# ilkyyldz95/3DmedicalImageSegmentation

Measured on AMD Instinct MI355X. Metric: training volumes/sec (96^3, 4-class), higher is better.
Workload: dtype bf16; 1 GPU; UNETR(img=96^3,patch=16,hidden=768,layers=12,heads=12,classes=4) fwd+DiceCE+bwd+AdamW, batch 2/GPU, configs[1]; global_batch=2

## Files before the change

### 3dmedicalimagesegmentation_amd/_capi.py

```python
import ctypes
import os
from ctypes import c_double, c_float, c_int, c_long, c_size_t, c_void_p

_HERE = os.path.dirname(os.path.abspath(__file__))
LIB_PATH = os.environ.get("UNETR_AMD_LIB") or os.path.join(_HERE, "libunetr_hip.so")

PREC_F32 = 0
PREC_BF16 = 1
PREC_BF16X3 = 2
ABI_VERSION = 21

_ERR = {1: "invalid argument", 2: "kernel launch failed", 3: "unsupported shape/configuration",
        4: "workspace too small"}


class GemmDesc(ctypes.Structure):
    _fields_ = [
        ("M", c_int), ("N", c_int), ("K", c_int), ("batch", c_int),
        ("a_trans", c_int), ("b_trans", c_int),
        ("lda", c_long), ("ldb", c_long), ("ldc", c_long),
        ("strideA", c_long), ("strideB", c_long), ("strideC", c_long),
        ("bias", c_void_p), ("res", c_void_p),
        ("ldr", c_long), ("strideR", c_long), ("res_mod", c_int),
        ("pre", c_void_p), ("aux", c_void_p), ("ldaux", c_long),
        ("act", c_int), ("accumulate", c_int), ("alpha", c_float), ("prec", c_int), ("b_x3words", c_int),
    ]


class GemmBf16Desc(ctypes.Structure):
    _fields_ = [
        ("M", c_int), ("N", c_int), ("K", c_int), ("b_kn", c_int),
        ("lda", c_long), ("ldb", c_long), ("ldc", c_long), ("ldcb", c_long),
        ("bias", c_void_p), ("res", c_void_p), ("ldr", c_long), ("res_mod", c_int),
        ("pre", c_void_p), ("aux", c_void_p), ("ldaux", c_long),
        ("act", c_int), ("accumulate", c_int), ("alpha", c_float),
        ("tc_d", c_int), ("tc_h", c_int), ("tc_w", c_int), ("tc_cout", c_int), ("x3", c_int),
    ]


class GroupedProblem(ctypes.Structure):
    _fields_ = [("dy", c_void_p), ("x", c_void_p), ("dw", c_void_p), ("M", c_int), ("N", c_int), ("K", c_int)]


class AdamWArena(ctypes.Structure):
    _fields_ = [("param", c_void_p), ("grad", c_void_p), ("m", c_void_p), ("v", c_void_p), ("shadow_bf16", c_void_p), ("steps", c_void_p),
                ("total", c_long), ("lr", c_float), ("beta1", c_float), ("beta2", c_float), ("eps", c_float), ("weight_decay", c_float),
                ("shadow_x3", c_void_p)]


class PackProblem(ctypes.Structure):
    _fields_ = [("w", c_void_p), ("out", c_void_p), ("Cin", c_int), ("Cout", c_int), ("kind", c_int)]


class ReduceProblem(ctypes.Structure):
    _fields_ = [("part", c_void_p), ("dst", c_void_p), ("n", c_long), ("rows", c_int)]


class SplitProblem(ctypes.Structure):
    _fields_ = [("src", c_void_p), ("dst", c_void_p), ("rows", c_long), ("cols", c_long), ("second", c_int)]


class ColsumProblem(ctypes.Structure):
    _fields_ = [("x", c_void_p), ("out", c_void_p), ("ld", c_long), ("M", c_int), ("N", c_int), ("x_bf16", c_int)]


class AugDesc(ctypes.Structure):
    _fields_ = [("B", c_int), ("num_samples", c_int), ("C", c_int), ("L", c_int), ("S0", c_int), ("S1", c_int), ("S2", c_int),
                ("sampling", c_int), ("ax0", c_int), ("ax1", c_int), ("max_k", c_int), ("normalize", c_int),
                ("pos_ratio", c_double), ("flip_prob", c_double * 3), ("rot90_prob", c_double), ("shift_prob", c_double),
                ("shift_lo", c_double), ("shift_hi", c_double), ("seed", ctypes.c_uint64)]


P = c_void_p
_SIGNATURES = {
    "unetr_abi_version": [],
    "unetr_gemm": [ctypes.POINTER(GemmDesc), P, P, P, P, c_size_t, P],
    "unetr_gemm_bf16": [ctypes.POINTER(GemmBf16Desc), P, P, P, P, P, c_size_t, P],
    "unetr_gemm_bf16_ln_bwd": [ctypes.POINTER(GemmBf16Desc), P, P, P, P, P, P, P, P, P, P, P, P, P, c_size_t, P, c_size_t, P],
    "unetr_gemm_bf16_ln_fwd": [ctypes.POINTER(GemmBf16Desc), P, P, P, P, P, c_float, P, P, P, P, P, c_size_t, P],
    "unetr_cast_bf16": [P, P, c_long, P],
    "unetr_split_words": [P, P, c_long, P],
    "unetr_split_stack_bf16": [P, P, c_long, c_long, c_int, P],
    "unetr_split_stack_bf16_grouped": [ctypes.POINTER(SplitProblem), c_int, P],
    "unetr_attention_bf16_fwd": [P, P, P, P, c_int, c_int, c_int, c_int, c_float, P],
    "unetr_attention_bf16_bwd": [P, P, P, P, P, P, P, c_int, c_int, c_int, c_int, c_float, P],
    "unetr_gemm_grouped_wgrad": [ctypes.POINTER(GroupedProblem), c_int, c_int, P],
    "unetr_gemm_bf16_grouped_wgrad": [ctypes.POINTER(GroupedProblem), c_int, P],
    "unetr_gemm_bf16_grouped_wgrad_adamw": [ctypes.POINTER(GroupedProblem), c_int, ctypes.POINTER(AdamWArena), ctypes.POINTER(c_int), P],
    "unetr_adamw_ranges": [ctypes.POINTER(AdamWArena), P, c_int, c_long, P],
    "unetr_gemm_bf16_grouped_wgrad_bf16out": [ctypes.POINTER(GroupedProblem), c_int, P, P, c_long, P],
    "unetr_cast_bf16_ranges": [P, P, P, c_int, c_long, P],
    "unetr_colsum_grouped": [ctypes.POINTER(ColsumProblem), c_int, P],
    "unetr_tconv_fwd": [P, c_long, P, P, c_long, c_int, c_int, c_int, c_int, c_int, c_int, c_int, P, c_size_t, P],
    "unetr_tconv_dgrad": [P, c_long, P, P, c_long, c_int, c_int, c_int, c_int, c_int, c_int, c_int, c_int, P, c_size_t, P],
    "unetr_tconv_wgrad": [P, c_long, P, c_long, P, c_int, c_int, c_int, c_int, c_int, c_int, c_int, P, c_size_t, P],
    "unetr_tconv2_fwd": [P, c_long, P, P, c_long, c_int, c_int, c_int, c_int, c_int, c_int, c_int, P, c_size_t, P],
    "unetr_tconv2_wgrad": [P, c_long, P, c_long, P, c_int, c_int, c_int, c_int, c_int, c_int, c_int, P, c_size_t, P],
    "unetr_tconv2_dgrad": [P, c_long, P, P, c_long, c_int, c_int, c_int, c_int, c_int, c_int, c_int, c_int, P, c_size_t, P],
    "unetr_tconv2_fwd_supported": [c_long, c_int, c_int, c_long, c_long],
    "unetr_tconv2_wgrad_supported": [c_long, c_int, c_int, c_long, c_long],
    "unetr_pixel_shuffle2": [P, P, c_long, c_int, c_int, c_int, c_int, c_int, c_int, P],
    "unetr_pixel_unshuffle2_bf16": [P, c_long, P, c_int, c_int, c_int, c_int, c_int, c_int, P],
    "unetr_colsum": [P, c_long, c_int, c_int, P, c_int, P, c_size_t, P],
    "unetr_layernorm_fwd": [P, P, P, P, P, P, P, c_int, c_int, c_float, P],
    "unetr_layernorm_bwd": [P, P, P, P, P, P, P, P, P, P, c_int, c_int, P, c_size_t, P],
    "unetr_attention_fwd": [P, P, P, P, c_int, c_int, c_int, c_int, c_float, c_int, P],
    "unetr_attention_bwd": [P, P, P, P, P, P, P, c_int, c_int, c_int, c_int, c_float, c_int, P],
    "unetr_conv_pack_weight": [P, P, c_int, c_int, c_int, c_int, P],
    "unetr_conv_gemm_fwd": [P, c_long, P, P, c_long, c_int, c_int, c_int, c_int, c_int, c_int, c_int, c_int, c_int, P, c_size_t, P],
    "unetr_conv_gemm_wgrad": [P, c_long, P, c_long, P, c_int, c_int, c_int, c_int, c_int, c_int, c_int, c_int, P, c_size_t, P],
    "unetr_conv3_pack_weight": [P, P, c_int, c_int, c_int, c_int, P],
    "unetr_conv3_fwd": [P, c_long, P, P, c_long, c_int, c_int, c_int, c_int, c_int, c_int, c_int, c_int, P],
    "unetr_conv3_fwd_fused": [P, c_long, P, P, c_long, P, P, P, c_long, P, c_float, c_int, c_int, c_int, c_int, c_int, c_int, c_int, c_int, P, c_size_t, P],
    "unetr_conv3_fwd_parts": [P, c_long, P, P, c_long, P, P, P, c_long, P, ctypes.POINTER(c_int), c_int, c_int, c_int, c_int, c_int, c_int, c_int, c_int, P],
    "unetr_conv3_dgrad_stats": [P, c_long, P, P, c_long, P, c_long, P, P, ctypes.POINTER(c_int), c_int, c_int, c_int, c_int, c_int, c_int, c_int, P],
    "unetr_instnorm_apply_fin": [P, c_long, P, c_int, P, c_long, P, c_int, P, P, c_float, P, c_long, c_int, c_long, c_int, c_int, c_int, P],
    "unetr_instnorm_apply_fin_img": [P, c_long, P, c_int, P, c_int, P, P, c_int, P, P, c_float, P, c_long, c_int, c_long, c_int, c_int, c_int, P],
    "unetr_instnorm_bwd_img": [P, c_long, P, c_long, P, P, c_int, P, P, P, c_long, P, ctypes.POINTER(c_int), c_int, c_long, c_int, c_int, P, c_size_t, c_int, P],
    "unetr_instnorm_bwd_apply_fin": [P, c_long, P, c_long, P, P, c_long, P, P, c_int, c_int, P, c_long, P, c_long, c_int, c_long, c_int, c_int, c_int, P],
    "unetr_conv3_wgrad_parts": [P, c_long, P, c_long, P, c_long, P, c_size_t, ctypes.POINTER(c_long), c_int, c_int, c_int, c_int, c_int, c_int, c_int, c_int, P],
    "unetr_tconv2_wgrad_parts": [P, c_long, P, c_long, P, c_size_t, ctypes.POINTER(c_long), c_int, c_int, c_int, c_int, c_int, c_int, c_int, P],
    "unetr_reduce_rows_grouped": [ctypes.POINTER(ReduceProblem), c_int, P],
    "unetr_conv3_dgrad_fused": [P, c_long, P, P, c_long, P, P, P, c_long, c_int, c_int, c_int, c_int, c_int, c_int, c_int, P, c_size_t, P],
    "unetr_conv3_pack_grouped": [ctypes.POINTER(PackProblem), c_int, c_int, P],
    "unetr_conv3_pack_1x1": [P, P, c_int, c_int, c_int, P],
    "unetr_instnorm_stats_finalize": [P, c_int, c_int, c_long, c_int, c_float, P, P],
    "unetr_conv3_wgrad": [P, c_long, P, c_long, P, P, c_long, P, c_int, c_int, c_int, c_int, c_int, c_int, c_int, c_int, P, c_size_t, P],
    "unetr_debug_tr16": [P, P, P],
    "unetr_instnorm_stats": [P, c_long, c_int, c_long, c_int, c_float, P, P, c_size_t, c_int, P],
    "unetr_instnorm_apply": [P, c_long, P, P, c_long, P, P, c_long, c_int, c_long, c_int, c_int, c_int, P],
    "unetr_instnorm_bwd": [P, c_long, P, c_long, P, P, c_long, P, P, c_long, P, c_long, c_int, c_long, c_int, c_int, P, c_size_t, c_int, P],
    "unetr_nchw_to_nhwc": [P, P, c_long, c_int, c_int, c_long, c_int, P],
    "unetr_nhwc_to_nchw": [P, c_long, P, c_int, c_int, c_long, c_int, c_int, P],
    "unetr_patch_gather": [P, P, P, c_int, c_int, c_int, c_int, c_int, c_int, P],
    "unetr_counter_add": [P, P, c_int, P],
    "unetr_add_cast_bf16": [P, P, P, P, c_long, P],
    "unetr_copy_rows": [P, c_long, P, c_long, c_long, c_int, c_int, c_int, P],
    "unetr_outconv_fwd": [P, c_long, P, P, P, c_int, c_long, c_int, c_int, c_int, P],
    "unetr_outconv_bwd": [P, P, c_long, P, P, c_long, P, P, c_int, c_long, c_int, c_int, P, c_size_t, c_int, P],
    "unetr_outconv_in_fwd": [P, c_long, P, c_int, P, c_long, P, c_int, P, P, c_float, P, P, P, c_int, c_long, c_int, c_int, c_int, P],
    "unetr_outconv_in_bwd": [P, P, c_long, P, P, c_long, P, P, P, c_long, P, P, P, c_int, c_long, c_int, c_int, P, c_size_t, c_int, P],
    "unetr_dicece_fwd": [P, P, c_int, c_int, c_long, c_int, c_float, c_float, P, P, P, c_size_t, P],
    "unetr_dicece_bwd": [P, P, P, P, P, c_int, c_int, c_long, c_int, P],
    "unetr_sw_accumulate": [P, P, P, P, c_int, c_int, c_int, c_int, c_int, c_int, c_int, c_int, c_int, c_int, P],
    "unetr_sw_finalize": [P, P, c_int, c_int, c_long, P],
    "unetr_dice_counts": [P, P, c_int, c_int, c_long, c_int, P, P, c_size_t, P],
    "unetr_hausdorff": [P, P, c_int, c_int, c_int, c_int, c_int, c_int, c_int, c_int, c_double, c_int, P, P, c_size_t, c_int, P],
    "unetr_aug_prep": [P, P, c_int, c_int, c_int, c_int, c_int, c_int, c_float, c_float, c_float, c_float, c_float, c_int, P, P, P],
    "unetr_aug_crop": [P, P, c_int, c_int, c_int, c_int, c_int, c_int, c_int, c_int, c_int, c_int, c_int, P, P, P],
    "unetr_aug_index_count": [P, P, c_int, c_int, c_long, c_float, P, c_size_t, P],
    "unetr_aug_index_scatter": [P, P, c_int, c_int, c_long, c_float, P, c_size_t, P, P, P],
    "unetr_aug_sample": [ctypes.POINTER(AugDesc), P, c_int, P, P, P, P],
    "unetr_aug_gather": [ctypes.POINTER(AugDesc), P, c_int, P, P, P, P, c_size_t, P],
    "unetr_resample_orient": [P, c_int, P, c_int, c_int, c_int, c_int, c_int, c_int, ctypes.POINTER(c_double), c_int, c_int, c_int, P, P, P],
    "unetr_ranking_loss_fwd": [P, c_int, c_int, c_int, c_int, c_int, c_int, c_float, c_int, P, P, P, c_size_t, P],
    "unetr_ranking_loss_bwd": [P, c_int, c_int, c_int, c_int, c_int, c_int, P, P, P, P],
    "unetr_adamw": [P, P, P, P, c_long, c_float, c_float, c_float, c_float, c_float, P, P, P],
    "unetr_adamw_reduced": [P, P, c_int, c_float, P, P, c_long, c_float, c_float, c_float, c_float, c_float, P, P, P, P],
}

EXPORTED_SYMBOLS = tuple(_SIGNATURES) + ("unetr_conv3_packed_bytes", "unetr_conv3_packed_1x1_bytes", "unetr_ranking_workspace_floats",
                                            "unetr_conv3_wgrad_rows", "unetr_tconv2_wgrad_rows", "unetr_outconv_in_bwd_rows", "unetr_hausdorff_workspace_bytes",
                                            "unetr_aug_index_ws_ints", "unetr_aug_gather_ws_bytes")

_lib = None


def load():
    global _lib
    if _lib is not None:
        return _lib
    if not os.path.exists(LIB_PATH):
        raise RuntimeError(
            f"{LIB_PATH} is missing: the HIP extension is not built. Run `python -c 'import __graft_entry__ as g; "
            f"g.build()'` or `make -C {os.path.join(_HERE, 'csrc')}`. There is no CPU/PyTorch fallback.")
    lib = ctypes.CDLL(LIB_PATH)
    lib.unetr_abi_version.restype = c_int
    got = lib.unetr_abi_version()
    if got != ABI_VERSION:
        raise RuntimeError(f"{LIB_PATH} reports C-ABI version {got}, this binding was written against {ABI_VERSION}: the "
                           f"library is stale -- rebuild the extension (`make -C {os.path.join(_HERE, 'csrc')}`).")
    for name, argtypes in _SIGNATURES.items():
        fn = getattr(lib, name)
        fn.argtypes = argtypes
        fn.restype = c_int
    lib.unetr_conv3_packed_bytes.argtypes = [c_int, c_int, c_int, c_int]
    lib.unetr_conv3_packed_bytes.restype = c_size_t
    lib.unetr_conv3_packed_1x1_bytes.argtypes = [c_int, c_int, c_int]
# ... 31 lines not shown
```

### 3dmedicalimagesegmentation_amd/csrc/attention_b16.hip

```cpp
#include <cstdlib>
#include "common.hpp"
#include "../../include/unetr_hip.h"

namespace {

typedef __attribute__((address_space(3))) void lds_void_t;
typedef const __attribute__((address_space(1))) void gbl_void_t;
typedef short s16x4 __attribute__((ext_vector_type(4)));
typedef short s16x8 __attribute__((ext_vector_type(8)));
#define LDS_AS_ __attribute__((address_space(3)))

constexpr int DH = 64, ROWB = 128;
constexpr int CKEYS = 224, CT = CKEYS / 16;
constexpr int IMG = CKEYS * ROWB;
constexpr float NEG_BIG = -1.0e30f;

__device__ __forceinline__ int img_off(int row, int chunk) { return row * ROWB + ((chunk ^ (((row >> 1) & 3) << 1)) << 4); }

template <int NT>
__device__ __forceinline__ void stage_img(const uint16_t* __restrict__ src, long rs, int row0, int nrows, int rows, char* img) {
    const int tid = threadIdx.x, wave = __builtin_amdgcn_readfirstlane(tid >> 6);
    const int pieces = rows * 8;
    for (int base = 0; base < pieces; base += NT) {
        const int id = base + tid;
// ... 18 lines not shown

__device__ __forceinline__ void prod_T(f32x4 (&out)[4], f32x4 x0, f32x4 x1, const char* img, int R0) {
    const int lane = threadIdx.x & 63, c = lane & 15, g = lane >> 4, q = c >> 2, p = c & 3;
    float xv[8] = {x0[0], x0[1], x0[2], x0[3], x1[0], x1[1], x1[2], x1[3]};
    const u32x4 b = PrecBF16::pack(xv);
    const int r0 = R0 + 4 * g + q, r1 = r0 + 16;
#pragma unroll
    for (int dt = 0; dt < 4; ++dt) {
        const int ch = dt * 2 + (p >> 1);
        s16x4 lo = __builtin_amdgcn_ds_read_tr16_b64_v4i16((LDS_AS_ s16x4*)(img + img_off(r0, ch) + (p & 1) * 8));
        s16x4 hi = __builtin_amdgcn_ds_read_tr16_b64_v4i16((LDS_AS_ s16x4*)(img + img_off(r1, ch) + (p & 1) * 8));
        s16x8 t = {lo[0], lo[1], lo[2], lo[3], hi[0], hi[1], hi[2], hi[3]};
        PrecBF16::mma(out[dt], __builtin_bit_cast(u32x4, t), b);
    }
}

template <class F>
__device__ __forceinline__ void prod_rows_full(const char* img, const u32x4 (&vec)[2], F&& each) {
    const int lane = threadIdx.x & 63, c = lane & 15, g = lane >> 4;
    constexpr int DPT = 5;
    const char* p0 = img + img_off(c, g);
    const char* p1 = img + img_off(c, 4 + g);
    u32x4 r0[DPT], r1[DPT];
#pragma unroll
    for (int t = 0; t < DPT; ++t) { r0[t] = *(const u32x4*)(p0 + t * 16 * ROWB); r1[t] = *(const u32x4*)(p1 + t * 16 * ROWB); }
    __builtin_amdgcn_sched_barrier(0);
#pragma unroll
    for (int t = 0; t < CT; ++t) {
        f32x4 acc = {0.f, 0.f, 0.f, 0.f};
        PrecBF16::mma(acc, r0[t % DPT], vec[0]);
        PrecBF16::mma(acc, r1[t % DPT], vec[1]);
        if (t + DPT < CT) { r0[t % DPT] = *(const u32x4*)(p0 + (t + DPT) * 16 * ROWB); r1[t % DPT] = *(const u32x4*)(p1 + (t + DPT) * 16 * ROWB); }
        each(t, acc);
        __builtin_amdgcn_sched_barrier(0);
    }
}
template <class F>
__device__ __forceinline__ void prod_T_full(f32x4 (&out)[4], const char* img, F&& x) {
    const int lane = threadIdx.x & 63, c = lane & 15, g = lane >> 4, q = c >> 2, p = c & 3;
    constexpr int NS = (CT / 2) * 4, DPT = 6;
    const char* b0[2];
    const int r0 = 4 * g + q;
    auto addr = [&](int st, int hi) { const int t2 = st >> 2, dt = st & 3; return img + img_off(32 * t2 + r0 + 16 * hi, dt * 2 + (p >> 1)) + (p & 1) * 8; };
    (void)b0;
    s16x4 lo[DPT], hi[DPT];
#pragma unroll
    for (int st = 0; st < DPT; ++st) {
        lo[st] = __builtin_amdgcn_ds_read_tr16_b64_v4i16((LDS_AS_ s16x4*)addr(st, 0));
        hi[st] = __builtin_amdgcn_ds_read_tr16_b64_v4i16((LDS_AS_ s16x4*)addr(st, 1));
    }
    __builtin_amdgcn_sched_barrier(0);
    u32x4 b = {0u, 0u, 0u, 0u};
#pragma unroll
    for (int st = 0; st < NS; ++st) {
        const int t2 = st >> 2, dt = st & 3;
        if (dt == 0) {
            f32x4 x0, x1;
            x(t2, x0, x1);
            float xv[8] = {x0[0], x0[1], x0[2], x0[3], x1[0], x1[1], x1[2], x1[3]};
            b = PrecBF16::pack(xv);
        }
        s16x8 t = {lo[st % DPT][0], lo[st % DPT][1], lo[st % DPT][2], lo[st % DPT][3], hi[st % DPT][0], hi[st % DPT][1], hi[st % DPT][2], hi[st % DPT][3]};
        PrecBF16::mma(out[dt], __builtin_bit_cast(u32x4, t), b);
        if (st + DPT < NS) {
            lo[st % DPT] = __builtin_amdgcn_ds_read_tr16_b64_v4i16((LDS_AS_ s16x4*)addr(st + DPT, 0));
            hi[st % DPT] = __builtin_amdgcn_ds_read_tr16_b64_v4i16((LDS_AS_ s16x4*)addr(st + DPT, 1));
        }
        __builtin_amdgcn_sched_barrier(0);
    }
}

__device__ __forceinline__ void load_vec(const uint16_t* __restrict__ row, u32x4 (&f)[2]) {
    const int g = (threadIdx.x & 63) >> 4;
    f[0] = *(const u32x4*)(row + g * 8);
    f[1] = *(const u32x4*)(row + (4 + g) * 8);
}

__device__ __forceinline__ float grp_max(float v) { v = fmaxf(v, __shfl_xor(v, 16, 64)); return fmaxf(v, __shfl_xor(v, 32, 64)); }
__device__ __forceinline__ float grp_sum(float v) { v += __shfl_xor(v, 16, 64); return v + __shfl_xor(v, 32, 64); }

template <int NW>
__global__ void __launch_bounds__(64 * NW)
attn16_fwd_kernel(const uint16_t* __restrict__ qkv, float* __restrict__ out, uint16_t* __restrict__ outb, float* __restrict__ lse,
                  int L, int heads, float scale) {
    constexpr int NT = 64 * NW;
    extern __shared__ __attribute__((aligned(1024))) char lds[];
    char* kimg = lds;
    char* vimg = lds + IMG;
    const int lane = threadIdx.x & 63, wave = __builtin_amdgcn_readfirstlane(threadIdx.x >> 6), c = lane & 15, g = lane >> 4;
    const int head = blockIdx.y, b = blockIdx.z, Hd = heads * DH;
    const long rs = 3L * Hd;
    const uint16_t* qb = qkv + (long)b * L * rs + head * DH;
    const uint16_t* kb_ = qb + Hd;
    const uint16_t* vb = qb + 2 * Hd;
    const int q = blockIdx.x * (16 * NW) + wave * 16 + c, qc = min(q, L - 1);
    u32x4 qf[2];
    load_vec(qb + (long)qc * rs, qf);
    f32x4 o[4];
#pragma unroll
    for (int dt = 0; dt < 4; ++dt) o[dt] = (f32x4){0.f, 0.f, 0.f, 0.f};
    float m = NEG_BIG, l = 0.f;
    for (int k0 = 0; k0 < L; k0 += CKEYS) {
        const int nkeys = min(CKEYS, L - k0), rows = (nkeys + 31) & ~31, nt = rows >> 4;
        if (k0) __syncthreads();
        stage_img<NT>(kb_, rs, k0, L, rows, kimg);
        stage_img<NT>(vb, rs, k0, L, rows, vimg);
        asm volatile("s_waitcnt vmcnt(0)" ::: "memory");
        __syncthreads();
        f32x4 s[CT];
        float tmax = NEG_BIG;
        const bool full = nt == CT;
        if (full) {
            prod_rows_full(kimg, qf, [&](int t, f32x4 acc) {
#pragma unroll
                for (int r = 0; r < 4; ++r) {
                    const int key = t * 16 + 4 * g + r;
                    acc[r] = key < nkeys ? acc[r] * scale : NEG_BIG;
                    tmax = fmaxf(tmax, acc[r]);
                }
                s[t] = acc;
            });
        } else
#pragma unroll
        for (int t = 0; t < CT; ++t) {
            if (t < nt) {
                s[t] = prod_rows(kimg, t, qf);
#pragma unroll
                for (int r = 0; r < 4; ++r) {
                    const int key = t * 16 + 4 * g + r;
                    s[t][r] = key < nkeys ? s[t][r] * scale : NEG_BIG;
                    tmax = fmaxf(tmax, s[t][r]);
                }
            } else {
                s[t] = (f32x4){NEG_BIG, NEG_BIG, NEG_BIG, NEG_BIG};
            }
        }
        tmax = grp_max(tmax);
        const float mn = fmaxf(m, tmax), alpha = __expf(m - mn);
        float ps = 0.f;
#pragma unroll
        for (int t = 0; t < CT; ++t)
#pragma unroll
            for (int r = 0; r < 4; ++r) { s[t][r] = __expf(s[t][r] - mn); ps += s[t][r]; }
        ps = grp_sum(ps);
        l = l * alpha + ps;
        m = mn;
#pragma unroll
        for (int dt = 0; dt < 4; ++dt) o[dt] *= alpha;
        if (full) {
            prod_T_full(o, vimg, [&](int t2, f32x4& x0, f32x4& x1) { x0 = s[2 * t2]; x1 = s[2 * t2 + 1]; });
        } else {
#pragma unroll
            for (int t2 = 0; t2 < CT / 2; ++t2)
                if (2 * t2 < nt) prod_T(o, s[2 * t2], s[2 * t2 + 1], vimg, 32 * t2);
        }
    }
    if (q < L) {
        const float inv = 1.f / l;
        if (out) {
            float* op = out + ((long)b * L + q) * Hd + head * DH + 4 * g;
#pragma unroll
            for (int dt = 0; dt < 4; ++dt) *(f32x4*)(op + dt * 16) = o[dt] * inv;
        }
        if (outb) {
            uint16_t* ob = outb + ((long)b * L + q) * Hd + head * DH + 4 * g;
#pragma unroll
            for (int dt = 0; dt < 4; ++dt) *(bf16x4*)(ob + dt * 16) = __builtin_convertvector(o[dt] * inv, bf16x4);
        }
// ... 117 lines not shown
        stage_img<NT>(qb, rs, q0, L, rows, qimg);
        stage_img<NT>(dob, (long)Hd, q0, L, rows, doimg);
        for (int i = threadIdx.x; i < rows; i += NT) {
            const int qq = q0 + i;
            lse_t[i] = qq < L ? lse[((long)b * heads + head) * L + qq] : 1.0e30f;
        }
        for (int i = threadIdx.x; i < rows; i += NT) {
            const int qq = min(q0 + i, L - 1);
            float part[4];
#pragma unroll
            for (int gg = 0; gg < 4; ++gg) {
                part[gg] = 0.f;
#pragma unroll
                for (int kb = 0; kb < 2; ++kb) {
                    const bf16x8 a = __builtin_bit_cast(bf16x8, *(const u32x4*)(ob_ + (long)qq * Hd + (kb * 4 + gg) * 8));
                    const bf16x8 d = __builtin_bit_cast(bf16x8, *(const u32x4*)(dob + (long)qq * Hd + (kb * 4 + gg) * 8));
#pragma unroll
                    for (int e = 0; e < 8; ++e) part[gg] += (float)a[e] * (float)d[e];
                }
            }
            del_t[i] = q0 + i < L ? (part[0] + part[1]) + (part[2] + part[3]) : 0.f;
        }
        asm volatile("s_waitcnt vmcnt(0)" ::: "memory");
        __syncthreads();
        if (nt == CT) {
            f32x4 pf[CT], dsf[CT];
            prod_rows_full(qimg, kf, [&](int t, f32x4 acc) {
                const f32x4 l4 = *(const f32x4*)(lse_t + t * 16 + 4 * g);
#pragma unroll
                for (int r = 0; r < 4; ++r) acc[r] = __expf(acc[r] * scale - l4[r]);
                pf[t] = acc;
            });
            prod_rows_full(doimg, vf, [&](int t, f32x4 dp) {
                const f32x4 d4 = *(const f32x4*)(del_t + t * 16 + 4 * g);
#pragma unroll
                for (int r = 0; r < 4; ++r) dsf[t][r] = pf[t][r] * (dp[r] - d4[r]);
            });
            prod_T_full(dv, doimg, [&](int t2, f32x4& x0, f32x4& x1) { x0 = pf[2 * t2]; x1 = pf[2 * t2 + 1]; });
            prod_T_full(dk, qimg, [&](int t2, f32x4& x0, f32x4& x1) { x0 = dsf[2 * t2]; x1 = dsf[2 * t2 + 1]; });
        } else
#pragma unroll
        for (int t2 = 0; t2 < CT / 2; ++t2) {
            if (2 * t2 >= nt) break;
            f32x4 p[2], ds[2];
#pragma unroll
            for (int h = 0; h < 2; ++h) {
                const int t = 2 * t2 + h;
                const f32x4 s = prod_rows(qimg, t, kf);
                const f32x4 dp = prod_rows(doimg, t, vf);
                const f32x4 l4 = *(const f32x4*)(lse_t + t * 16 + 4 * g), d4 = *(const f32x4*)(del_t + t * 16 + 4 * g);
#pragma unroll
                for (int r = 0; r < 4; ++r) {
                    const float pv = __expf(s[r] * scale - l4[r]);
                    p[h][r] = pv;
                    ds[h][r] = pv * (dp[r] - d4[r]);
                }
            }
            prod_T(dv, p[0], p[1], doimg, 32 * t2);
            prod_T(dk, ds[0], ds[1], qimg, 32 * t2);
        }
    }
    if (key < L) {
        if (dqkv) {
            float* kp = dqkv + ((long)b * L + key) * rs + Hd + head * DH + 4 * g;
#pragma unroll
            for (int dt = 0; dt < 4; ++dt) {
                *(f32x4*)(kp + dt * 16) = dk[dt] * scale;
                *(f32x4*)(kp + Hd + dt * 16) = dv[dt];
            }
        }
        uint16_t* kb2 = dqkvb + ((long)b * L + key) * rs + Hd + head * DH + 4 * g;
#pragma unroll
        for (int dt = 0; dt < 4; ++dt) {
            *(bf16x4*)(kb2 + dt * 16) = __builtin_convertvector(dk[dt] * scale, bf16x4);
            *(bf16x4*)(kb2 + Hd + dt * 16) = __builtin_convertvector(dv[dt], bf16x4);
        }
    }
}

template <int NW>
__global__ void __launch_bounds__(64 * NW)
attn16_bwd_kernel(const uint16_t* __restrict__ qkv, const uint16_t* __restrict__ outb, const uint16_t* __restrict__ doutb,
                  const float* __restrict__ lse, float* __restrict__ delta, float* __restrict__ dqkv, uint16_t* __restrict__ dqkvb,
                  int L, int heads, float scale, int nqb) {
    extern __shared__ __attribute__((aligned(1024))) char lds[];
    const int xb = __builtin_amdgcn_readfirstlane(blockIdx.x);
    if (xb < nqb) attn16_bwd_dq_body<NW>(lds, xb, qkv, outb, doutb, lse, delta, dqkv, dqkvb, L, heads, scale);
    else attn16_bwd_dkv_body<NW>(lds, xb - nqb, qkv, outb, doutb, lse, dqkv, dqkvb, L, heads, scale);
}

template <class K, class... A>
void launch_dyn(K kern, dim3 grid, int nt, size_t lds, hipStream_t st, A... args) {
    if (lds > 64 * 1024) (void)hipFuncSetAttribute((const void*)kern, hipFuncAttributeMaxDynamicSharedMemorySize, (int)lds);
    hipLaunchKernelGGL(kern, grid, dim3(nt), lds, st, args...);
}

inline int pick_nw(int B, int L, int heads) { return ((long)cdiv(L, 32) * heads * B <= 512) ? 2 : 4; }
inline int pick_nw_fwd(int B, int L, int heads) {
    if (const char* e = getenv("UNETR_ATTN_NW")) { const int v = atoi(e); if (v == 2 || v == 4 || v == 8) return v; }
    const int nw = pick_nw(B, L, heads);
    return (nw == 4 && (long)cdiv(L, 64) * heads * B > 1024) ? 8 : nw;
}

}

extern "C" int unetr_attention_bf16_fwd(const void* qkv, float* out, void* out_bf16, float* lse, int B, int L, int heads, int dh,
                                        float scale, void* stream) {
    if (!qkv || (!out && !out_bf16) || !lse || B <= 0 || L <= 0 || heads <= 0 || B > 65535 || heads > 65535) return UNETR_ERR_ARG;
    if (dh != DH || ((uintptr_t)qkv & 15) || (out && ((uintptr_t)out & 15)) || (out_bf16 && ((uintptr_t)out_bf16 & 7))) return UNETR_ERR_UNSUPPORTED;
    hipStream_t st = (hipStream_t)stream;
    const size_t lds = 2 * IMG;
    const int nw = pick_nw_fwd(B, L, heads);
    if (nw == 2)
        launch_dyn(attn16_fwd_kernel<2>, dim3(cdiv(L, 32), heads, B), 128, lds, st, (const uint16_t*)qkv, out, (uint16_t*)out_bf16, lse, L, heads, scale);
    else if (nw == 4)
        launch_dyn(attn16_fwd_kernel<4>, dim3(cdiv(L, 64), heads, B), 256, lds, st, (const uint16_t*)qkv, out, (uint16_t*)out_bf16, lse, L, heads, scale);
    else
        launch_dyn(attn16_fwd_kernel<8>, dim3(cdiv(L, 128), heads, B), 512, lds, st, (const uint16_t*)qkv, out, (uint16_t*)out_bf16, lse, L, heads, scale);
    return unetr_check_launch();
}

extern "C" int unetr_attention_bf16_bwd(const void* qkv, const void* out_bf16, const void* dout_bf16, const float* lse, float* dqkv,
                                        void* dqkv_bf16, float* delta, int B, int L, int heads, int dh, float scale, void* stream) {
    if (!qkv || !out_bf16 || !dout_bf16 || !lse || !dqkv_bf16 || !delta || B <= 0 || L <= 0 || heads <= 0 || B > 65535 || heads > 65535)
        return UNETR_ERR_ARG;
    if (dh != DH || ((uintptr_t)qkv & 15) || ((uintptr_t)out_bf16 & 15) || ((uintptr_t)dout_bf16 & 15) || ((uintptr_t)dqkv_bf16 & 7) ||
        (dqkv && ((uintptr_t)dqkv & 15)))
        return UNETR_ERR_UNSUPPORTED;
    hipStream_t st = (hipStream_t)stream;
    const uint16_t* q = (const uint16_t*)qkv;
    const uint16_t* o = (const uint16_t*)out_bf16;
    const uint16_t* d = (const uint16_t*)dout_bf16;
    uint16_t* gq = (uint16_t*)dqkv_bf16;
    const size_t lk = 2 * IMG + 2 * CKEYS * sizeof(float);
    if (pick_nw(B, L, heads) == 2) {
        const int nqb = cdiv(L, 32);
        launch_dyn(attn16_bwd_kernel<2>, dim3(2 * nqb, heads, B), 128, lk, st, q, o, d, lse, delta, dqkv, gq, L, heads, scale, nqb);
    } else {
        const int nqb = cdiv(L, 64);
        launch_dyn(attn16_bwd_kernel<4>, dim3(2 * nqb, heads, B), 256, lk, st, q, o, d, lse, delta, dqkv, gq, L, heads, scale, nqb);
    }
    return unetr_check_launch();
}
```

### 3dmedicalimagesegmentation_amd/csrc/common.hpp

```cpp
#pragma once
#include "../../include/unetr_hip.h"
#include <hip/hip_runtime.h>
#include <stdint.h>

typedef float f32x2 __attribute__((ext_vector_type(2)));
typedef float f32x4 __attribute__((ext_vector_type(4)));
typedef float f32x8 __attribute__((ext_vector_type(8)));
typedef __bf16 bf16x8 __attribute__((ext_vector_type(8)));
typedef __bf16 bf16x4 __attribute__((ext_vector_type(4)));
typedef uint32_t u32x4 __attribute__((ext_vector_type(4)));

#define UNETR_OK 0
#define UNETR_ERR_ARG 1
#define UNETR_ERR_LAUNCH 2
#define UNETR_ERR_UNSUPPORTED 3
#define UNETR_ERR_WORKSPACE 4

#define UNETR_PREC_F32 0
#define UNETR_PREC_BF16 1
#define UNETR_PREC_BF16X3 2

static inline int unetr_check_launch() {
    hipError_t e = hipGetLastError();
    return e == hipSuccess ? UNETR_OK : UNETR_ERR_LAUNCH;
}

struct PrecF32 {
    static constexpr int CH = 4;
    static __device__ __forceinline__ u32x4 pack(const float* v) {
        f32x4 t = {v[0], v[1], v[2], v[3]};
        return __builtin_bit_cast(u32x4, t);
    }
    static __device__ __forceinline__ u32x4 from_raw(u32x4 r) { return r; }
    static __device__ __forceinline__ void mma(f32x4& acc, u32x4 a, u32x4 b) {
        f32x4 af = __builtin_bit_cast(f32x4, a), bf = __builtin_bit_cast(f32x4, b);
        acc = __builtin_amdgcn_mfma_f32_16x16x4f32(af[0], bf[0], acc, 0, 0, 0);
        acc = __builtin_amdgcn_mfma_f32_16x16x4f32(af[1], bf[1], acc, 0, 0, 0);
        acc = __builtin_amdgcn_mfma_f32_16x16x4f32(af[2], bf[2], acc, 0, 0, 0);
        acc = __builtin_amdgcn_mfma_f32_16x16x4f32(af[3], bf[3], acc, 0, 0, 0);
    }
};

struct PrecBF16 {
    static constexpr int CH = 8;
    static __device__ __forceinline__ u32x4 pack(const float* v) {
        f32x8 t = {v[0], v[1], v[2], v[3], v[4], v[5], v[6], v[7]};
        bf16x8 b = __builtin_convertvector(t, bf16x8);
        return __builtin_bit_cast(u32x4, b);
    }
    static __device__ __forceinline__ u32x4 from_raw(u32x4 r) { return r; }
    static __device__ __forceinline__ void mma(f32x4& acc, u32x4 a, u32x4 b) {
        acc = __builtin_amdgcn_mfma_f32_16x16x32_bf16(__builtin_bit_cast(bf16x8, a), __builtin_bit_cast(bf16x8, b),
                                                      acc, 0, 0, 0);
    }
};

struct PrecBF16x3 {
    static constexpr int CH = 4;
    static __device__ __forceinline__ uint32_t split(float a) {
        const __bf16 h = (__bf16)a;
#ifdef UNETR_X3_DROP_LO
        return (uint32_t)__builtin_bit_cast(uint16_t, h);
#endif
        const __bf16 l = (__bf16)(a - (float)h);
        return (uint32_t)__builtin_bit_cast(uint16_t, h) | ((uint32_t)__builtin_bit_cast(uint16_t, l) << 16);
    }
    static __device__ __forceinline__ u32x4 pack(const float* v) { return (u32x4){split(v[0]), split(v[1]), split(v[2]), split(v[3])}; }
    static __device__ __forceinline__ u32x4 from_raw(u32x4 r) {
        const f32x4 f = __builtin_bit_cast(f32x4, r);
        return (u32x4){split(f[0]), split(f[1]), split(f[2]), split(f[3])};
    }
    static __device__ __forceinline__ void mma(f32x4& acc, u32x4 a, u32x4 b) {
        u32x4 ah, al;
#pragma unroll
        for (int e = 0; e < 4; ++e) {
            ah[e] = __builtin_amdgcn_perm(a[e], a[e], 0x01000100u);
            al[e] = __builtin_amdgcn_perm(a[e], a[e], 0x03020302u);
        }
        acc = __builtin_amdgcn_mfma_f32_16x16x32_bf16(__builtin_bit_cast(bf16x8, ah), __builtin_bit_cast(bf16x8, b), acc, 0, 0, 0);
        acc = __builtin_amdgcn_mfma_f32_16x16x32_bf16(__builtin_bit_cast(bf16x8, al), __builtin_bit_cast(bf16x8, b), acc, 0, 0, 0);
    }
};
typedef float f32x2_ __attribute__((ext_vector_type(2)));
typedef __bf16 bf16x2_ __attribute__((ext_vector_type(2)));
__device__ __forceinline__ float x3_rem(uint32_t r) {
#ifdef UNETR_X3_DROP_LO
// ... 66 lines not shown
    const float pe = p * c.decay;
    const float me = fmaf(c.b1, m, (1.f - c.b1) * g);
    const float ve = fmaf(c.b2, v, ((1.f - c.b2) * g) * g);
    const float denom = fmaf(sqrtf(ve), c.inv_sqrt_bc2, c.eps);
    p = fmaf(-c.step_size, me / denom, pe);
    m = me;
    v = ve;
}

__device__ __forceinline__ float gelu_exact(float x) { return 0.5f * x * (1.0f + erff(x * 0.70710678118654752440f)); }
__device__ __forceinline__ float gelu_grad(float x) {
    return 0.5f * (1.0f + erff(x * 0.70710678118654752440f)) + x * 0.39894228040143267794f * expf(-0.5f * x * x);
}

__device__ __forceinline__ float erf_poly_tail(float t , float e ) {
    const float k = __builtin_amdgcn_rcpf(1.0f + 0.3275911f * t);
    float p = 1.061405429f;
    p = fmaf(p, k, -1.453152027f); p = fmaf(p, k, 1.421413741f); p = fmaf(p, k, -0.284496736f); p = fmaf(p, k, 0.254829592f);
    return 1.0f - p * k * e;
}
__device__ __forceinline__ float gelu_fast(float x) {
    const float t = fabsf(x) * 0.70710678118654752440f;
    const float e = __expf(-t * t);
    const float er = copysignf(erf_poly_tail(t, e), x);
    return 0.5f * x * (1.0f + er);
}
__device__ __forceinline__ float gelu_grad_fast(float x) {
    const float t = fabsf(x) * 0.70710678118654752440f;
    const float e = __expf(-t * t);
    const float er = copysignf(erf_poly_tail(t, e), x);
    return 0.5f * (1.0f + er) + x * 0.39894228040143267794f * e;
}

static inline int cdiv(long a, long b) { return (int)((a + b - 1) / b); }

template <class T> struct Io;
template <> struct Io<float> {
    static constexpr int B16 = 0;
    static constexpr int W = 4;
    static __device__ __forceinline__ void ldw(const float* p, float (&v)[4]) { const f32x4 t = *(const f32x4*)p; v[0] = t[0]; v[1] = t[1]; v[2] = t[2]; v[3] = t[3]; }
    static __device__ __forceinline__ void stw(float* p, const float (&v)[4]) { *(f32x4*)p = (f32x4){v[0], v[1], v[2], v[3]}; }
    static __device__ __forceinline__ u32x4 ldraw(const float* p) { return *(const u32x4*)p; }
    static __device__ __forceinline__ void unpack(u32x4 r, float (&v)[4]) {
#pragma unroll
        for (int e = 0; e < 4; ++e) { const uint32_t t = r[e]; v[e] = __builtin_bit_cast(float, t); }
    }
    static __device__ __forceinline__ f32x4 ld4(const float* p) { return *(const f32x4*)p; }
    static __device__ __forceinline__ void st4(float* p, f32x4 v) { *(f32x4*)p = v; }
    static __device__ __forceinline__ float ld1(const float* p) { return *p; }
    static __device__ __forceinline__ void st1(float* p, float v) { *p = v; }
};
template <> struct Io<uint16_t> {
    static constexpr int B16 = 1;
    static constexpr int W = 8;
    static __device__ __forceinline__ void ldw(const uint16_t* p, float (&v)[8]) {
        const f32x8 t = __builtin_convertvector(*(const bf16x8*)p, f32x8);
#pragma unroll
        for (int e = 0; e < 8; ++e) v[e] = t[e];
    }
    static __device__ __forceinline__ void stw(uint16_t* p, const float (&v)[8]) {
        const f32x8 t = {v[0], v[1], v[2], v[3], v[4], v[5], v[6], v[7]};
        *(bf16x8*)p = __builtin_convertvector(t, bf16x8);
    }
    static __device__ __forceinline__ u32x4 ldraw(const uint16_t* p) { return *(const u32x4*)p; }
    static __device__ __forceinline__ void unpack(u32x4 r, float (&v)[8]) {
#pragma unroll
        for (int e = 0; e < 4; ++e) {
            v[2 * e] = __builtin_bit_cast(float, r[e] << 16);
            v[2 * e + 1] = __builtin_bit_cast(float, r[e] & 0xffff0000u);
        }
    }
    static __device__ __forceinline__ f32x4 ld4(const uint16_t* p) { return __builtin_convertvector(*(const bf16x4*)p, f32x4); }
    static __device__ __forceinline__ void st4(uint16_t* p, f32x4 v) { *(bf16x4*)p = __builtin_convertvector(v, bf16x4); }
    static __device__ __forceinline__ float ld1(const uint16_t* p) { return __builtin_bit_cast(float, (uint32_t)*p << 16); }
    static __device__ __forceinline__ void st1(uint16_t* p, float v) { __bf16 h = (__bf16)v; *p = __builtin_bit_cast(uint16_t, h); }
};
template <class P> struct ActOf { typedef float type; };
template <> struct ActOf<PrecBF16> { typedef uint16_t type; };
template <class P>
__device__ __forceinline__ u32x4 act_chunk(const typename ActOf<P>::type* p, bool ok) {
    const u32x4 w = *(const u32x4*)p;
    return ok ? P::from_raw(w) : (u32x4){0u, 0u, 0u, 0u};
}
int unetr_layernorm_bwd_partials(const float* dy, int splits, long slab, const float* x, const float* gamma, const float* mean,
                                 const float* rstd, float* dx, void* dx_bf16, const float* dres, float* dgamma,
                                 float* dbeta, int M, int H, float* ws, size_t ws_bytes, void* stream);

int unetr_layernorm_fwd_partials(const float* partials, int splits, long slab, const float* bias, const float* res, long ldr, int res_mod,
                                 float* xout, const float* gamma, const float* beta, float* y, void* y_bf16, float* mean, float* rstd,
                                 int M, int H, float eps, void* stream);

int unetr_gemm_x3_dma(const unetr_gemm_bf16_desc* d, const float* A, const float* B, int b_words, float* C, float* ws, size_t ws_bytes, void* stream,
                      int* psp = nullptr);

int unetr_instnorm_stats_finalize2(const float* part, const float* part_b, int nchunk, int B, long V, int C, float eps,
                                   float* stats, float* stats_b, void* stream);

#define ACT_DISPATCH(act16, ...) do { if (act16) { typedef uint16_t AT; __VA_ARGS__; } else { typedef float AT; __VA_ARGS__; } } while (0)
```

### 3dmedicalimagesegmentation_amd/csrc/gemm_bf16.hip

```cpp
#include <type_traits>
#include "gemm_kernel.hpp"

namespace {

typedef __attribute__((address_space(3))) void lds_void_t;
typedef const __attribute__((address_space(1))) void gbl_void_t;
typedef short s16x4 __attribute__((ext_vector_type(4)));
typedef short s16x8 __attribute__((ext_vector_type(8)));
#define LDS_AS_ __attribute__((address_space(3)))

struct EpBf {
    int vec_ok;
    float* C; long ldc;
    uint16_t* Cb; long ldcb;
    const float* bias;
    const float* res; long ldr; int res_mod;
    float* pre;
    const float* aux; long ldaux;
    int act, accumulate; float alpha;
    int tc_d, tc_h, tc_w, tc_cout;
    __device__ __forceinline__ long tc_off(int m, int n) const {
        const int tap = n / tc_cout, co = n - tap * tc_cout;
        const int x = m % tc_w; int t = m / tc_w; const int y = t % tc_h; t /= tc_h; const int z = t % tc_d; const int b = t / tc_d;
        const long ov = (((long)b * 2 * tc_d + 2 * z + (tap >> 2)) * 2 * tc_h + 2 * y + ((tap >> 1) & 1)) * 2 * tc_w + 2 * x + (tap & 1);
// ... 760 lines not shown
    if (M <= 0 || N <= 0 || K <= 0) return UNETR_ERR_ARG;
    if (K % 64 || d->lda % 8 || d->ldb % 8 || ((uintptr_t)A & 15) || ((uintptr_t)B & 15)) return UNETR_ERR_UNSUPPORTED;
    if (d->b_kn && (N % 8 || N < 8)) return UNETR_ERR_UNSUPPORTED;
    if (d->act == 2 && !d->aux) return UNETR_ERR_ARG;
    if (d->accumulate && !C) return UNETR_ERR_ARG;
    hipStream_t st = (hipStream_t)stream;
    auto al16 = [](const void* p) { return ((uintptr_t)p & 15) == 0; };
    const int vec_ok = (N % 4 == 0) && (!C || (d->ldc % 4 == 0 && al16(C))) && (!Cb || (d->ldcb % 4 == 0 && ((uintptr_t)Cb & 7) == 0)) &&
                       (!d->bias || al16(d->bias)) && (!d->res || (d->ldr % 4 == 0 && al16(d->res))) && (!d->pre || al16(d->pre)) &&
                       (!d->aux || (d->ldaux % 4 == 0 && al16(d->aux))) && al16(ws);
    if (d->tc_cout > 0 && (C || !Cb || d->pre || d->accumulate || d->tc_cout % 4 || N != 8 * d->tc_cout || d->tc_d <= 0 || d->tc_h <= 0 ||
                           d->tc_w <= 0 || M % (d->tc_d * d->tc_h * d->tc_w))) return UNETR_ERR_UNSUPPORTED;
    EpBf ep{vec_ok, C, d->ldc, (uint16_t*)Cb, d->ldcb, d->bias, d->res, d->ldr, d->res_mod > 0 ? d->res_mod : M,
            d->pre, d->aux, d->ldaux, d->act, d->accumulate, d->alpha, d->tc_d, d->tc_h, d->tc_w, d->tc_cout > 0 ? d->tc_cout : 0};
    const uint16_t* a = (const uint16_t*)A;
    const uint16_t* b = (const uint16_t*)B;
    const int env_cfg = getenv("UNETR_GEMM_CFG") ? atoi(getenv("UNETR_GEMM_CFG")) : 0;
    const bool few128 = K <= 512 && (long)cdiv(M, 128) * cdiv(N, 128) < 128;
    const bool big = env_cfg == 128 || (env_cfg == 0 && M >= 1024 && N >= 128 && !few128);
    if (!d->b_kn && d->tc_cout <= 0 && (env_cfg == 256 || (env_cfg == 0 && M >= 1024))) {
        const int wn = env_cfg == 256 ? (getenv("UNETR_GEMM_BIG_WN") ? big_tile_width(M, N, K) : 4) : big_tile_width(M, N, K);
        if (wn) return launch_bf16_big(M, N, K, a, d->lda, b, d->ldb, ep, st, wn);
    }
#define BF16_GO(WM_, WN_, BKN_, NS_) return launch_bf16<WM_, WN_, 2, 2, BKN_, NS_>(M, N, K, a, d->lda, b, d->ldb, ep, ws, ws_bytes, st, psp)
    int cfg = env_cfg;
    if (!big && (cfg == 0 || cfg == 64)) {
        cfg = 6464;
        if (env_cfg == 0 && K <= 1024 && N <= 1024) cfg = d->b_kn ? 3264 : 6432;
        if (env_cfg == 0 && K <= 1024 && d->b_kn && N > 1024 && N % 64 == 0) cfg = 3264;
        if (env_cfg == 0 && M > 512) {
            if (!d->b_kn) {
                if (N >= 3072 || (N >= 2304 && M >= 960)) cfg = 6496;
                else if (K >= 2048 && N <= 1024) cfg = 6432;
            } else if (N % 128 == 0) {
                if ((K >= 2048 && N <= 1024) || (K <= 1024 && N > 1024)) cfg = 64128;
            }
        }
    }
    if (!d->b_kn) {
        if (big) BF16_GO(4, 4, false, 2);
        if (cfg == 6432) BF16_GO(2, 1, false, 4);
        if (cfg == 3264) BF16_GO(1, 2, false, 4);
        if (cfg == 64128) BF16_GO(2, 4, false, 3);
        if (cfg == 6496) BF16_GO(2, 3, false, 3);
        BF16_GO(2, 2, false, 4);
    }
    if (big) BF16_GO(4, 4, true, 2);
    if (cfg == 3264) BF16_GO(1, 2, true, 4);
    if (cfg == 64128) BF16_GO(2, 4, true, 3);
    BF16_GO(2, 2, true, 4);
#undef BF16_GO
}

int unetr_gemm_x3_dma(const unetr_gemm_bf16_desc* d, const float* A, const float* B, int b_words, float* C, float* ws, size_t ws_bytes, void* stream,
                      int* psp) {
    const int M = d->M, N = d->N, K = d->K;
    if (M <= 0 || N <= 0 || K <= 0) return UNETR_ERR_ARG;
    if (K % 32 || d->lda % 4 || d->ldb % 4 || ((uintptr_t)A & 15) || ((uintptr_t)B & 15) || N % 4) return UNETR_ERR_UNSUPPORTED;
    if (d->b_kn && N < 64) return UNETR_ERR_UNSUPPORTED;
    auto al16 = [](const void* p) { return ((uintptr_t)p & 15) == 0; };
    const int vec_ok = (d->ldc % 4 == 0 && al16(C)) && (!d->bias || al16(d->bias)) && (!d->res || (d->ldr % 4 == 0 && al16(d->res))) &&
                       (!d->pre || al16(d->pre)) && (!d->aux || (d->ldaux % 4 == 0 && al16(d->aux))) && al16(ws);
    if (!vec_ok) return UNETR_ERR_UNSUPPORTED;
    EpBf ep{1, C, d->ldc, nullptr, 0, d->bias, d->res, d->ldr, d->res_mod > 0 ? d->res_mod : M, d->pre, d->aux, d->ldaux, d->act,
            d->accumulate, d->alpha, 0, 0, 0, 0};
    hipStream_t st = (hipStream_t)stream;
#define X3_GO(WM_, WN_, BKN_, NS_) do { if (b_words) return launch_bf16<WM_, WN_, 2, 2, BKN_, NS_, 2>(M, N, K, A, d->lda, B, d->ldb, ep, ws, ws_bytes, st, psp); \
                                        return launch_bf16<WM_, WN_, 2, 2, BKN_, NS_, 1>(M, N, K, A, d->lda, B, d->ldb, ep, ws, ws_bytes, st, psp); } while (0)
    if (M >= 1024 && N >= 128) { if (d->b_kn) X3_GO(4, 4, true, 2); X3_GO(4, 4, false, 2); }
    if (!d->b_kn) {
        if (K <= 1024 && N <= 1024) X3_GO(2, 1, false, 4);
        X3_GO(2, 2, false, 4);
    }
    if (K <= 1024 && N % 64 == 0) X3_GO(1, 2, true, 4);
    X3_GO(2, 2, true, 4);
#undef X3_GO
}

extern "C" int unetr_gemm_bf16(const unetr_gemm_bf16_desc* d, const void* A, const void* B, float* C, void* Cb,
                               float* ws, size_t ws_bytes, void* stream) {
    return gemm_bf16_impl(d, A, B, C, Cb, ws, ws_bytes, stream, nullptr);
}

extern "C" int unetr_gemm_bf16_ln_bwd(const unetr_gemm_bf16_desc* d, const void* A, const void* B, float* C,
                                      const float* x, const float* gamma, const float* mean, const float* rstd,
                                      float* dx, void* dx_bf16, const float* dres, float* dgamma, float* dbeta,
                                      float* ln_ws, size_t ln_ws_bytes, float* ws, size_t ws_bytes, void* stream) {
    if (!d || !C) return UNETR_ERR_ARG;
    if (d->bias || d->res || d->pre || d->act || d->accumulate || d->alpha != 1.f || d->ldc != d->N) return UNETR_ERR_UNSUPPORTED;
    int splits = 1;
    if (int e = gemm_bf16_impl(d, A, B, C, nullptr, ws, ws_bytes, stream, &splits)) return e;
    const float* dy = splits > 1 ? ws : C;
    return unetr_layernorm_bwd_partials(dy, splits, (long)d->M * d->N, x, gamma, mean, rstd, dx, dx_bf16, dres, dgamma, dbeta,
                                        d->M, d->N, ln_ws, ln_ws_bytes, stream);
}

extern "C" int unetr_gemm_bf16_ln_fwd(const unetr_gemm_bf16_desc* d, const void* A, const void* B, float* C,
                                      const float* gamma, const float* beta, float eps, float* y, void* y_bf16, float* mean, float* rstd,
                                      float* ws, size_t ws_bytes, void* stream) {
    if (!d || !C) return UNETR_ERR_ARG;
    if (d->pre || d->act || d->accumulate || d->alpha != 1.f || d->ldc != d->N) return UNETR_ERR_UNSUPPORTED;
    int splits = 1;
    if (int e = gemm_bf16_impl(d, A, B, C, nullptr, ws, ws_bytes, stream, &splits)) return e;
    if (splits > 1)
        return unetr_layernorm_fwd_partials(ws, splits, (long)d->M * d->N, d->bias, d->res, d->ldr, d->res_mod > 0 ? d->res_mod : d->M,
                                            C, gamma, beta, y, y_bf16, mean, rstd, d->M, d->N, eps, stream);
    return unetr_layernorm_fwd(C, gamma, beta, y, y_bf16, mean, rstd, d->M, d->N, eps, stream);
}

extern "C" int unetr_cast_bf16(const float* src, void* dst, long n, void* stream) {
    if (!src || !dst || n < 0) return UNETR_ERR_ARG;
    if (n == 0) return UNETR_OK;
    hipStream_t st = (hipStream_t)stream;
    const bool al = (((uintptr_t)src & 15) | ((uintptr_t)dst & 15)) == 0;
    const long n8 = al ? n / 8 : 0;
    if (n8) hipLaunchKernelGGL(cast_bf16_kernel, dim3((unsigned)std::min<long>(cdiv(n8, 256), 4096)), dim3(256), 0, st, src, (uint16_t*)dst, n8);
    if (n8 * 8 < n) hipLaunchKernelGGL(cast_bf16_tail_kernel, dim3(cdiv(n - n8 * 8, 256)), dim3(256), 0, st, src, (uint16_t*)dst, n8 * 8, n);
    return unetr_check_launch();
}

__global__ void __launch_bounds__(256) split_words_kernel(const float* __restrict__ src, uint32_t* __restrict__ dst, long n4) {
    for (long i = blockIdx.x * 256L + threadIdx.x; i < n4; i += (long)gridDim.x * 256) ((u32x4*)dst)[i] = x3_words(((const u32x4*)src)[i]);
}

extern "C" int unetr_split_words(const float* src, void* dst, long n, void* stream) {
    if (!src || !dst || n <= 0) return UNETR_ERR_ARG;
    if ((n & 3) || (((uintptr_t)src | (uintptr_t)dst) & 15)) return UNETR_ERR_UNSUPPORTED;
    hipLaunchKernelGGL(split_words_kernel, dim3((unsigned)std::min<long>(cdiv(n / 4, 256), 8192)), dim3(256), 0, (hipStream_t)stream, src, (uint32_t*)dst, n / 4);
    return unetr_check_launch();
}

extern "C" int unetr_split_stack_bf16(const float* src, void* dst, long rows, long cols, int second, void* stream) {
    if (!src || !dst || rows <= 0 || cols <= 0) return UNETR_ERR_ARG;
    const long n = rows * cols;
    if ((n & 7) || (((uintptr_t)src | (uintptr_t)dst) & 15)) return UNETR_ERR_UNSUPPORTED;
    hipLaunchKernelGGL(split_stack_kernel, dim3((unsigned)std::min<long>(cdiv(n / 8, 256), 4096)), dim3(256), 0, (hipStream_t)stream, src, (uint16_t*)dst,
                       n / 8, n, second);
    return unetr_check_launch();
}

extern "C" int unetr_split_stack_bf16_grouped(const unetr_split_problem* probs, int n, void* stream) {
    if (!probs || n <= 0) return UNETR_ERR_ARG;
    for (int base = 0; base < n; base += SS_MAX) {
        SsArgs a;
        a.n = std::min(SS_MAX, n - base);
        int blocks = 0;
        for (int i = 0; i < a.n; ++i) {
            const unetr_split_problem& q = probs[base + i];
            const long ne = q.rows * q.cols;
            if (!q.src || !q.dst || q.rows <= 0 || q.cols <= 0) return UNETR_ERR_ARG;
            if ((ne & 7) || (((uintptr_t)q.src | (uintptr_t)q.dst) & 15)) return UNETR_ERR_UNSUPPORTED;
            const int nb = (int)std::min<long>(cdiv(ne / 8, 256), 1024);
            a.p[i] = SsProblem{q.src, (uint16_t*)q.dst, ne / 8, q.second, blocks, nb};
            blocks += nb;
        }
        hipLaunchKernelGGL(split_stack_grouped_kernel, dim3(blocks), dim3(256), 0, (hipStream_t)stream, a);
    }
    return unetr_check_launch();
}

__global__ void __launch_bounds__(256) cast_bf16_ranges_kernel(const float* __restrict__ src, uint16_t* __restrict__ dst,
                                                               const long* __restrict__ table, int nr) {
    int lo_r = 0, hi_r = nr - 1;
    const long blk = blockIdx.x;
    while (lo_r < hi_r) {
        const int mid = (lo_r + hi_r + 1) >> 1;
        if (table[3 * mid + 2] <= blk) lo_r = mid; else hi_r = mid - 1;
    }
    const long beg = table[3 * lo_r] + (blk - table[3 * lo_r + 2]) * 8192, end = min(table[3 * lo_r + 1], beg + 8192);
    for (long i = beg / 8 + threadIdx.x; i < end / 8; i += 256) {
        const f32x4 a = ((const f32x4*)src)[2 * i], b = ((const f32x4*)src)[2 * i + 1];
        float v[8] = {a[0], a[1], a[2], a[3], b[0], b[1], b[2], b[3]};
        ((u32x4*)dst)[i] = PrecBF16::pack(v);
    }
}

extern "C" int unetr_cast_bf16_ranges(const float* src_arena, void* dst_arena, const long* table_dev, int n_ranges, long n_blocks, void* stream) {
    if (!src_arena || !dst_arena || !table_dev || n_ranges <= 0 || n_blocks <= 0 || n_blocks > 0x7fffffffL) return UNETR_ERR_ARG;
    if (((uintptr_t)src_arena & 31) || ((uintptr_t)dst_arena & 15)) return UNETR_ERR_UNSUPPORTED;
    hipLaunchKernelGGL(cast_bf16_ranges_kernel, dim3((unsigned)n_blocks), dim3(256), 0, (hipStream_t)stream, src_arena, (uint16_t*)dst_arena,
                       table_dev, n_ranges);
    return unetr_check_launch();
}

extern "C" int unetr_add_cast_bf16(const float* a, const float* b, float* out, void* out_bf16, long n, void* stream) {
    if (!a || !b || !out || n <= 0) return UNETR_ERR_ARG;
    if ((n & 3) || (((uintptr_t)a | (uintptr_t)b | (uintptr_t)out) & 15) || ((uintptr_t)out_bf16 & 7)) return UNETR_ERR_UNSUPPORTED;
    hipLaunchKernelGGL(add_cast_bf16_kernel, dim3((unsigned)std::min<long>(cdiv(n / 4, 256), 2048)), dim3(256), 0, (hipStream_t)stream, a, b, out,
                       (uint16_t*)out_bf16, n / 4);
    return unetr_check_launch();
// ... 54 lines not shown
```

### 3dmedicalimagesegmentation_amd/csrc/norm_misc.hip

```cpp
#include <algorithm>
#include <cstdlib>
#include "common.hpp"
#include "../../include/unetr_hip.h"

namespace {

constexpr int LN_MAXV_MAX = 8;

struct LnFwdSrc { int splits; long slab; const float* bias; const float* res; long ldr; int res_mod; float* xout; };

template <int LN_MAXV>
__global__ void __launch_bounds__(256)
layernorm_fwd_kernel(const float* __restrict__ x, const float* __restrict__ gamma, const float* __restrict__ beta,
                     float* __restrict__ y, uint16_t* __restrict__ yb, float* __restrict__ mean, float* __restrict__ rstd,
                     int M, int H, float eps, LnFwdSrc src) {
    const int lane = threadIdx.x & 63, row = blockIdx.x * 4 + (threadIdx.x >> 6);
    if (row >= M) return;
    const int nv = H >> 2;
    const f32x4* xr = (const f32x4*)(x + (long)row * H);
    f32x4 v[LN_MAXV], gam[LN_MAXV], bet[LN_MAXV];
    float s = 0.f;
#pragma unroll
    for (int j = 0; j < LN_MAXV; ++j) {
        const int i = min(lane + 64 * j, nv - 1);
        gam[j] = ((const f32x4*)gamma)[i];
        bet[j] = ((const f32x4*)beta)[i];
    }
    if (src.splits > 1) {
        f32x4 sl[LN_MAXV][4], bi[LN_MAXV], re[LN_MAXV];
#pragma unroll
        for (int j = 0; j < LN_MAXV; ++j) {
            const int i = min(lane + 64 * j, nv - 1);
#pragma unroll
            for (int sp = 0; sp < 4; ++sp) sl[j][sp] = ((const f32x4*)(x + (sp < src.splits ? sp : 0) * src.slab + (long)row * H))[i];
            bi[j] = src.bias ? ((const f32x4*)src.bias)[i] : (f32x4){0.f, 0.f, 0.f, 0.f};
            re[j] = src.res ? ((const f32x4*)(src.res + (long)(row % src.res_mod) * src.ldr))[i] : (f32x4){0.f, 0.f, 0.f, 0.f};
        }
#pragma unroll
        for (int j = 0; j < LN_MAXV; ++j) {
            const int i = lane + 64 * j;
            f32x4 t = {0.f, 0.f, 0.f, 0.f};
            if (i < nv) {
#pragma unroll
                for (int sp = 0; sp < 4; ++sp)
                    if (sp < src.splits) t += sl[j][sp];
                for (int sp = 4; sp < src.splits; ++sp) t += ((const f32x4*)(x + sp * src.slab + (long)row * H))[i];
                if (src.bias) t += bi[j];
                if (src.res) t += re[j];
                ((f32x4*)(src.xout + (long)row * H))[i] = t;
            }
            v[j] = t;
        }
    } else {
#pragma unroll
        for (int j = 0; j < LN_MAXV; ++j) {
            const int i = lane + 64 * j;
            v[j] = i < nv ? xr[i] : (f32x4){0.f, 0.f, 0.f, 0.f};
        }
    }
#pragma unroll
    for (int j = 0; j < LN_MAXV; ++j) s += v[j][0] + v[j][1] + v[j][2] + v[j][3];
    const float mu = wave_sum(s) / (float)H;
    float q = 0.f;
#pragma unroll
    for (int j = 0; j < LN_MAXV; ++j) {
        int i = lane + 64 * j;
        if (i < nv) {
#pragma unroll
            for (int e = 0; e < 4; ++e) { float d = v[j][e] - mu; q += d * d; }
        }
    }
    const float rs = rsqrtf(wave_sum(q) / (float)H + eps);
    if (lane == 0) { mean[row] = mu; rstd[row] = rs; }
    f32x4* yr = (f32x4*)(y + (long)row * H);
#pragma unroll
    for (int j = 0; j < LN_MAXV; ++j) {
        int i = lane + 64 * j;
        if (i < nv) {
            const f32x4 g = gam[j], b = bet[j];
            f32x4 o;
#pragma unroll
            for (int e = 0; e < 4; ++e) o[e] = (v[j][e] - mu) * rs * g[e] + b[e];
            if (y) yr[i] = o;
            if (yb) ((bf16x4*)(yb + (long)row * H))[i] = __builtin_convertvector(o, bf16x4);
        }
    }
}

constexpr int LN_RPB = 4;
template <int LN_MAXV>
__global__ void __launch_bounds__(256)
layernorm_bwd_kernel(const float* __restrict__ dy, int splits, long slab, const float* __restrict__ x, const float* __restrict__ gamma,
                     const float* __restrict__ mean, const float* __restrict__ rstd, float* __restrict__ dx,
                     uint16_t* __restrict__ dxb, const float* __restrict__ dres, float* __restrict__ part, int M, int H) {
    extern __shared__ __attribute__((aligned(16))) float lds[];
    const int lane = threadIdx.x & 63, wave = threadIdx.x >> 6;
    const int nv = H >> 2;
    f32x4 dg[LN_MAXV], db[LN_MAXV];
#pragma unroll
    for (int j = 0; j < LN_MAXV; ++j) { dg[j] = (f32x4){0.f, 0.f, 0.f, 0.f}; db[j] = dg[j]; }
    for (int rr = wave; rr < LN_RPB; rr += 4) {
        const int row = blockIdx.x * LN_RPB + rr;
        if (row >= M) break;
        const float mu = mean[row], rs = rstd[row];
        const f32x4* xr = (const f32x4*)(x + (long)row * H);
        const f32x4* dyr = (const f32x4*)(dy + (long)row * H);
        f32x4 xh[LN_MAXV], g[LN_MAXV];
        float s1 = 0.f, s2 = 0.f;
        f32x4 xv_[LN_MAXV], gm_[LN_MAXV], sl_[LN_MAXV][4], rs_[LN_MAXV];
#pragma unroll
        for (int j = 0; j < LN_MAXV; ++j) {
            const int i = min(lane + 64 * j, nv - 1);
            xv_[j] = xr[i];
            gm_[j] = ((const f32x4*)gamma)[i];
#pragma unroll
            for (int sp = 0; sp < 4; ++sp) sl_[j][sp] = ((const f32x4*)(dy + (sp < splits ? sp : 0) * slab + (long)row * H))[i];
            rs_[j] = dres ? ((const f32x4*)(dres + (long)row * H))[i] : (f32x4){0.f, 0.f, 0.f, 0.f};
        }
#pragma unroll
        for (int j = 0; j < LN_MAXV; ++j) {
            int i = lane + 64 * j;
            if (i < nv) {
                f32x4 xv = xv_[j], dv = {0.f, 0.f, 0.f, 0.f}, gm = gm_[j];
                if (splits <= 1) dv = sl_[j][0];
                else {
#pragma unroll
                    for (int sp = 0; sp < 4; ++sp)
                        if (sp < splits) dv += sl_[j][sp];
                    for (int sp = 4; sp < splits; ++sp) dv += ((const f32x4*)(dy + sp * slab + (long)row * H))[i];
                }
#pragma unroll
                for (int e = 0; e < 4; ++e) {
                    float h = (xv[e] - mu) * rs;
                    xh[j][e] = h;
                    g[j][e] = dv[e] * gm[e];
                    s1 += g[j][e];
                    s2 += g[j][e] * h;
                    dg[j][e] += dv[e] * h;
                    db[j][e] += dv[e];
                }
            } else { xh[j] = (f32x4){0.f, 0.f, 0.f, 0.f}; g[j] = xh[j]; }
        }
        const float c1 = wave_sum(s1) / (float)H, c2 = wave_sum(s2) / (float)H;
        f32x4* dxr = (f32x4*)(dx + (long)row * H);
#pragma unroll
        for (int j = 0; j < LN_MAXV; ++j) {
            int i = lane + 64 * j;
            if (i < nv) {
                f32x4 o;
#pragma unroll
                for (int e = 0; e < 4; ++e) o[e] = rs * (g[j][e] - c1 - xh[j][e] * c2);
                if (dres) o += rs_[j];
                dxr[i] = o;
                if (dxb) ((bf16x4*)(dxb + (long)row * H))[i] = __builtin_convertvector(o, bf16x4);
            }
        }
    }
    f32x4* l4 = (f32x4*)lds;
#pragma unroll
    for (int j = 0; j < LN_MAXV; ++j) {
        int i = lane + 64 * j;
        if (i < nv) { l4[(wave * 2 + 0) * nv + i] = dg[j]; l4[(wave * 2 + 1) * nv + i] = db[j]; }
    }
    __syncthreads();
    for (int i = threadIdx.x; i < 2 * nv; i += 256) {
        int which = i / nv, c = i - which * nv;
        f32x4 s = l4[(0 * 2 + which) * nv + c];
        s += l4[(1 * 2 + which) * nv + c];
        s += l4[(2 * 2 + which) * nv + c];
        s += l4[(3 * 2 + which) * nv + c];
        ((f32x4*)part)[((long)blockIdx.x * 2 + which) * nv + c] = s;
    }
}

__global__ void __launch_bounds__(256)
ln_finalize_kernel(const float* __restrict__ part, int nblk, int H, float* __restrict__ dgamma, float* __restrict__ dbeta) {
    __shared__ float sm[4][64];
// ... 1307 lines not shown
__global__ void outconv_final_kernel(const float* __restrict__ part, int R, int N, int n0, float* __restrict__ out0, float* __restrict__ out1) {
    const int n = blockIdx.x * blockDim.x + threadIdx.x;
    if (n >= N) return;
    float s = 0.f;
    for (int r = 0; r < R; ++r) s += part[(long)r * N + n];
    if (n < n0) out0[n] = s; else out1[n - n0] = s;
}

template <bool GB16>
__global__ void __launch_bounds__(256)
adamw_kernel(float* __restrict__ p, const void* __restrict__ gsrc, float gscale, float* __restrict__ m, float* __restrict__ v,
             long n4, long n, float lr, float b1, float b2, float eps, float wd, const float* __restrict__ step_dev,
             uint16_t* __restrict__ shadow, uint32_t* __restrict__ words) {
    const AdamWCoef c = adamw_coef(lr, b1, b2, eps, wd, *step_dev);
    auto grad1 = [&](long i) -> float {
        if (GB16) { uint32_t u = (uint32_t)((const uint16_t*)gsrc)[i] << 16; return __builtin_bit_cast(float, u) * gscale; }
        return ((const float*)gsrc)[i] * gscale;
    };
    for (long i = (long)blockIdx.x * blockDim.x + threadIdx.x; i < n4; i += (long)gridDim.x * blockDim.x) {
        f32x4 pv = __builtin_nontemporal_load((f32x4*)p + i), mv = __builtin_nontemporal_load((f32x4*)m + i), vv = __builtin_nontemporal_load((f32x4*)v + i), gv;
        if (GB16) gv = __builtin_convertvector(__builtin_nontemporal_load((const bf16x4*)gsrc + i), f32x4) * gscale;
        else gv = __builtin_nontemporal_load((const f32x4*)gsrc + i) * gscale;
#pragma unroll
        for (int e = 0; e < 4; ++e) {
            float pe = pv[e], me = mv[e], ve = vv[e];
            adamw_elem(pe, me, ve, gv[e], c);
            pv[e] = pe; mv[e] = me; vv[e] = ve;
        }
        __builtin_nontemporal_store(pv, (f32x4*)p + i); __builtin_nontemporal_store(mv, (f32x4*)m + i); __builtin_nontemporal_store(vv, (f32x4*)v + i);
        if (shadow) ((bf16x4*)shadow)[i] = __builtin_convertvector(pv, bf16x4);
        if (words) ((u32x4*)words)[i] = x3_words(__builtin_bit_cast(u32x4, pv));
    }
    if (blockIdx.x == 0 && threadIdx.x < (n - n4 * 4)) {
        long i = n4 * 4 + threadIdx.x;
        float pe = p[i], me = m[i], ve = v[i];
        adamw_elem(pe, me, ve, grad1(i), c);
        p[i] = pe; m[i] = me; v[i] = ve;
        if (shadow) { __bf16 h = (__bf16)p[i]; shadow[i] = __builtin_bit_cast(uint16_t, h); }
        if (words) { const u32x4 w4 = x3_words((u32x4){__builtin_bit_cast(uint32_t, p[i]), 0u, 0u, 0u}); words[i] = w4[0]; }
    }
}

constexpr int AR_BLOCK = 4096;
__global__ void __launch_bounds__(256)
adamw_ranges_kernel(float* __restrict__ p, const float* __restrict__ g, float* __restrict__ m, float* __restrict__ v,
                    uint16_t* __restrict__ shadow, const float* __restrict__ steps, const long* __restrict__ table, int nr,
                    float lr, float b1, float b2, float eps, float wd, uint32_t* __restrict__ words) {
    int lo_r = 0, hi_r = nr - 1;
    const long blk = blockIdx.x;
    while (lo_r < hi_r) {
        const int mid = (lo_r + hi_r + 1) >> 1;
        if (table[4 * mid + 3] <= blk) lo_r = mid; else hi_r = mid - 1;
    }
    const long lo = table[4 * lo_r], hi = table[4 * lo_r + 1];
    const AdamWCoef c = adamw_coef(lr, b1, b2, eps, wd, steps[table[4 * lo_r + 2]]);
    const long beg = lo + (blk - table[4 * lo_r + 3]) * AR_BLOCK, end = min(hi, beg + AR_BLOCK);
    for (long i = beg / 4 + threadIdx.x; i < end / 4; i += 256) {
        f32x4 pv = __builtin_nontemporal_load((f32x4*)p + i), mv = __builtin_nontemporal_load((f32x4*)m + i), vv = __builtin_nontemporal_load((f32x4*)v + i);
        const f32x4 gv = __builtin_nontemporal_load((const f32x4*)g + i);
#pragma unroll
        for (int e = 0; e < 4; ++e) {
            float pe = pv[e], me = mv[e], ve = vv[e];
            adamw_elem(pe, me, ve, gv[e], c);
            pv[e] = pe; mv[e] = me; vv[e] = ve;
        }
        __builtin_nontemporal_store(pv, (f32x4*)p + i); __builtin_nontemporal_store(mv, (f32x4*)m + i); __builtin_nontemporal_store(vv, (f32x4*)v + i);
        if (shadow) ((bf16x4*)shadow)[i] = __builtin_convertvector(pv, bf16x4);
        if (words) ((u32x4*)words)[i] = x3_words(__builtin_bit_cast(u32x4, pv));
    }
}

inline void in_chunks(long V, int B, long step, long blocks, long& vpb, int& nchunk) {
    vpb = std::max<long>(step, ((V * B + blocks - 1) / blocks + step - 1) / step * step);
    nchunk = (int)((V + vpb - 1) / vpb);
}

inline int grid_for(long total, int per_block = 256, int cap = 8192) {
    long b = (total + per_block - 1) / per_block;
    return (int)std::max<long>(1, std::min<long>(b, cap));
}

}

extern "C" int unetr_layernorm_fwd(const float* x, const float* gamma, const float* beta, float* y, void* y_bf16,
                                   float* mean, float* rstd, int M, int H, float eps, void* stream) {
    if (!x || !gamma || !beta || (!y && !y_bf16) || !mean || !rstd || M <= 0) return UNETR_ERR_ARG;
    if ((H & 3) || H > LN_MAXV_MAX * 256) return UNETR_ERR_UNSUPPORTED;
    const LnFwdSrc src{1, 0, nullptr, nullptr, 0, 1, nullptr};
#define LN_FWD(V_) hipLaunchKernelGGL(layernorm_fwd_kernel<V_>, dim3(cdiv(M, 4)), dim3(256), 0, (hipStream_t)stream, x, gamma, beta, y, \
                                      (uint16_t*)y_bf16, mean, rstd, M, H, eps, src)
    if (H <= 768) LN_FWD(3); else if (H <= 1024) LN_FWD(4); else LN_FWD(8);
#undef LN_FWD
    return unetr_check_launch();
}

int unetr_layernorm_fwd_partials(const float* partials, int splits, long slab, const float* bias, const float* res, long ldr, int res_mod,
                                 float* xout, const float* gamma, const float* beta, float* y, void* y_bf16, float* mean, float* rstd,
                                 int M, int H, float eps, void* stream) {
    if (!partials || splits < 2 || !xout || !gamma || !beta || (!y && !y_bf16) || !mean || !rstd || M <= 0) return UNETR_ERR_ARG;
    if ((H & 3) || H > LN_MAXV_MAX * 256 || (res && (ldr & 3))) return UNETR_ERR_UNSUPPORTED;
    const LnFwdSrc src{splits, slab, bias, res, ldr, res_mod > 0 ? res_mod : M, xout};
    const float* x = partials;
#define LN_FWD(V_) hipLaunchKernelGGL(layernorm_fwd_kernel<V_>, dim3(cdiv(M, 4)), dim3(256), 0, (hipStream_t)stream, x, gamma, beta, y, \
                                      (uint16_t*)y_bf16, mean, rstd, M, H, eps, src)
    if (H <= 768) LN_FWD(3); else if (H <= 1024) LN_FWD(4); else LN_FWD(8);
#undef LN_FWD
    return unetr_check_launch();
}

int unetr_layernorm_bwd_partials(const float* dy, int splits, long slab, const float* x, const float* gamma, const float* mean,
                                 const float* rstd, float* dx, void* dx_bf16, const float* dres, float* dgamma,
                                 float* dbeta, int M, int H, float* ws, size_t ws_bytes, void* stream) {
    if (!dy || !x || !gamma || !mean || !rstd || !dx || ((dgamma == nullptr) != (dbeta == nullptr)) || M <= 0) return UNETR_ERR_ARG;
    if ((H & 3) || H > LN_MAXV_MAX * 256) return UNETR_ERR_UNSUPPORTED;
    int nblk = cdiv(M, LN_RPB);
    if ((size_t)nblk * 2 * H * sizeof(float) > ws_bytes || !ws) return UNETR_ERR_WORKSPACE;
    hipStream_t st = (hipStream_t)stream;
#define LN_BWD(V_) hipLaunchKernelGGL(layernorm_bwd_kernel<V_>, dim3(nblk), dim3(256), 4 * 2 * H * sizeof(float), st, dy, splits, slab, x, gamma, mean, \
                                      rstd, dx, (uint16_t*)dx_bf16, dres, ws, M, H)
    if (H <= 768) LN_BWD(3); else if (H <= 1024) LN_BWD(4); else LN_BWD(8);
    if (dgamma) hipLaunchKernelGGL(ln_finalize_kernel, dim3(cdiv(2 * H, 64)), dim3(256), 0, st, ws, nblk, H, dgamma, dbeta);
    return unetr_check_launch();
}

extern "C" int unetr_layernorm_bwd(const float* dy, const float* x, const float* gamma, const float* mean,
                                   const float* rstd, float* dx, void* dx_bf16, const float* dres, float* dgamma,
                                   float* dbeta, int M, int H, float* ws, size_t ws_bytes, void* stream) {
    return unetr_layernorm_bwd_partials(dy, 1, 0, x, gamma, mean, rstd, dx, dx_bf16, dres, dgamma, dbeta, M, H, ws, ws_bytes, stream);
}

extern "C" int unetr_colsum(const float* x, long ld, int M, int N, float* out, int accumulate,
                            float* ws, size_t ws_bytes, void* stream) {
    if (!x || !out || M <= 0 || N <= 0) return UNETR_ERR_ARG;
    int RB = std::max(1, std::min(cdiv(M, 64), 256));
    if (!ws || (size_t)RB * N * sizeof(float) > ws_bytes) return UNETR_ERR_WORKSPACE;
    hipStream_t st = (hipStream_t)stream;
    hipLaunchKernelGGL(colsum_kernel, dim3(cdiv(N, 64), RB), dim3(256), 0, st, x, ld, M, N, ws, RB);
    hipLaunchKernelGGL(colsum_final_kernel, dim3(cdiv(N, 256)), dim3(256), 0, st, ws, RB, N, out, accumulate);
    return unetr_check_launch();
}

extern "C" int unetr_colsum_grouped(const unetr_colsum_problem* probs, int n, void* stream) {
    if (!probs || n <= 0) return UNETR_ERR_ARG;
    for (int base = 0; base < n; base += CS_MAX) {
        ColsumArgs a;
        a.n = std::min(CS_MAX, n - base);
        int blocks = 0;
        for (int i = 0; i < a.n; ++i) {
            const unetr_colsum_problem& q = probs[base + i];
            if (!q.x || !q.out || q.M <= 0 || q.N <= 0) return UNETR_ERR_ARG;
            int vec = q.N % 4 == 0 && q.ld % 4 == 0 && (((uintptr_t)q.x | (uintptr_t)q.out) & 15) == 0;
            if (q.x_bf16) {
                if (q.N % 8 || q.ld % 8 || ((uintptr_t)q.x & 15)) return UNETR_ERR_UNSUPPORTED;
                vec = 2;
            }
            a.p[i] = ColsumProblem{(const float*)q.x, q.out, q.ld, q.M, q.N, blocks, vec};
            blocks += cdiv(q.N, 64);
        }
        hipLaunchKernelGGL(colsum_grouped_kernel, dim3(blocks), dim3(256), 0, (hipStream_t)stream, a);
    }
    return unetr_check_launch();
}

static int in_check(int C, long ld, int act16 = 0) {
    const int W = act16 ? 8 : 4;
    if ((C % W) || C > 1024 || (ld % W) || (256 % (C / W)) != 0) return UNETR_ERR_UNSUPPORTED;
    return UNETR_OK;
}

extern "C" int unetr_reduce_rows_grouped(const unetr_reduce_problem* probs, int n, void* stream) {
    if (!probs || n <= 0) return UNETR_ERR_ARG;
    hipStream_t st = (hipStream_t)stream;
    for (int base = 0; base < n; base += RR_MAX) {
        RrArgs a;
        a.n = std::min(RR_MAX, n - base);
        int blocks = 0;
        for (int i = 0; i < a.n; ++i) {
            const unetr_reduce_problem& q = probs[base + i];
            if (!q.part || !q.dst || q.rows <= 0 || q.n <= 0) return UNETR_ERR_ARG;
            const int vec = (q.n % 4 == 0 && (((uintptr_t)q.part | (uintptr_t)q.dst) & 15) == 0) ? 1 : 0;
            const int nb = (int)std::min<long>(vec ? (q.n + 127) / 128 : (q.n + 31) / 32, 8192);
            a.p[i] = RrProblem{q.part, q.dst, q.n, q.rows, blocks, nb, vec};
            blocks += nb;
        }
        hipLaunchKernelGGL(reduce_rows_grouped_kernel, dim3(blocks), dim3(256), 0, st, a);
    }
    return unetr_check_launch();
}

extern "C" int unetr_instnorm_stats(const void* x, long ld, int B, long V, int C, float eps, float* stats,
                                    float* ws, size_t ws_bytes, int act16, void* stream) {
    if (!x || !stats || B <= 0 || V <= 0) return UNETR_ERR_ARG;
    if (int e = in_check(C, ld, act16)) return e;
    int nchunk = cdiv(V, IN_VPB);
    if (!ws || (size_t)B * nchunk * 2 * C * sizeof(float) > ws_bytes) return UNETR_ERR_WORKSPACE;
    hipStream_t st = (hipStream_t)stream;
    const int cvn = C / (act16 ? 8 : 4), nphase = 256 / cvn;
    ACT_DISPATCH(act16, hipLaunchKernelGGL(in_stats_kernel<AT>, dim3(nchunk, B), dim3(256), (size_t)2 * nphase * C * 4, st, (const AT*)x, ld, V, C, ws));
    hipLaunchKernelGGL(in_stats_final_kernel, dim3(B * C), dim3(64), 0, st, ws, nchunk, V, C, eps, stats, B);
    return unetr_check_launch();
}

__global__ void __launch_bounds__(256)
in_stats_final_block_kernel(const float* __restrict__ part, int nchunk, long V, int C, float eps, float* __restrict__ stats,
                            const float* __restrict__ part_b, float* __restrict__ stats_b) {
    if (blockIdx.y) { part = part_b; stats = stats_b; }
    __shared__ double sm[2][4];
    const int i = blockIdx.x, b = i / C, c = i - b * C, lane = threadIdx.x & 63, wave = threadIdx.x >> 6;
    double s = 0.0, q = 0.0;
    int k = threadIdx.x;
    for (; k + 3 * 256 < nchunk; k += 4 * 256) {
// ... 370 lines not shown
```

### 3dmedicalimagesegmentation_amd/functional.py

```python
import ctypes
import os
import weakref

import torch

from . import _capi
from ._capi import GemmDesc, GemmBf16Desc, call, call_rc

LN_EPS = 1e-5
IN_EPS = 1e-5

_WS = {}
_WS_BYTES = int(os.environ.get("UNETR_AMD_WS_MB", "256")) << 20
_WS_SHARED = {}


def share_workspace(stream):
    _WS_SHARED.setdefault(stream.device.index, set()).add(stream.cuda_stream)


def workspace(device):
    sid = torch.cuda.current_stream(device).cuda_stream
    idx = device.index if device.index is not None else torch.cuda.current_device()
    if sid == 0 or sid in _WS_SHARED.get(idx, ()):
# ... 228 lines not shown
        raise RuntimeError("3dmedicalimagesegmentation_amd: the HIP backend needs tensors on a ROCm device "
                           "(got a CPU tensor); there is no CPU fallback.")
    if t.dtype != torch.float32 and not (act and t.dtype == torch.bfloat16):
        raise RuntimeError(f"3dmedicalimagesegmentation_amd: fp32 storage expected, got {t.dtype}")
    if t.device.index != torch.cuda.current_device():
        raise RuntimeError(f"3dmedicalimagesegmentation_amd: tensor lives on {t.device} but the current device is "
                           f"cuda:{torch.cuda.current_device()}; call torch.cuda.set_device({t.device.index}) (one process per GPU)")


def _rows(t):
    c = t.shape[-1]
    if t.stride(-1) == 1 and t.dim() >= 2:
        ld = t.stride(-2)
        al = 16 // t.element_size()
        ok = ld >= c and (ld % al == 0 or (ld == c and t.dtype == torch.float32)) and t.data_ptr() % 16 == 0
        exp = ld
        for d in range(t.dim() - 2, -1, -1):
            if t.shape[d] != 1 and t.stride(d) != exp:
                ok = False
                break
            exp *= t.shape[d]
        if ok:
            return t, ld
    t = t.contiguous()
    return t, c


def gemm(A, B, C, M, N, K, *, lda, ldb, ldc, prec, a_trans=False, b_trans=False, bias=None, res=None, ldr=0,
         res_mod=0, pre=None, aux=None, ldaux=0, act=0, accumulate=False, alpha=1.0, b_words=None):
    d = GemmDesc()
    d.b_x3words = 0
    if (b_words is not None and prec == _capi.PREC_BF16X3 and not a_trans and M >= 32 and K % 32 == 0 and N % 4 == 0 and lda % 4 == 0
            and ldb % 4 == 0 and ldc % 4 == 0 and (not b_trans or N >= 64)):
        B = b_words
        d.b_x3words = 1
    d.M, d.N, d.K, d.batch = M, N, K, 1
    d.a_trans, d.b_trans = int(a_trans), int(b_trans)
    d.lda, d.ldb, d.ldc = lda, ldb, ldc
    d.strideA = d.strideB = d.strideC = d.strideR = 0
    d.bias = bias.data_ptr() if bias is not None else None
    d.res = res.data_ptr() if res is not None else None
    d.ldr, d.res_mod = ldr, res_mod
    d.pre = pre.data_ptr() if pre is not None else None
    d.aux = aux.data_ptr() if aux is not None else None
    d.ldaux = ldaux
    d.act, d.accumulate, d.alpha, d.prec = act, int(accumulate), alpha, prec
    ws = workspace(C.device)
    call("unetr_gemm", ctypes.byref(d), A.data_ptr(), B.data_ptr(), C.data_ptr(), ws.data_ptr(), ws.numel() * 4, _stream())


def cast_bf16(src, out=None):
    src = src.contiguous()
    if out is None:
        out = torch.empty(src.shape, dtype=torch.bfloat16, device=src.device)
    call("unetr_cast_bf16", src.data_ptr(), out.data_ptr(), src.numel(), _stream())
    return out


def gemm_bf16(A, B, M, N, K, *, b_kn=False, C=None, Cb=None, lda=None, ldb=None, bias=None, res=None, ldr=0, res_mod=0,
              pre=None, aux=None, ldaux=0, act=0, accumulate=False, alpha=1.0, ldcb=None, tc=None):
    assert A.dtype == torch.bfloat16 and B.dtype == torch.bfloat16
    d = GemmBf16Desc()
    d.M, d.N, d.K, d.b_kn = M, N, K, int(b_kn)
    d.lda = lda if lda is not None else K
    d.ldb = ldb if ldb is not None else (N if b_kn else K)
    d.ldc = d.ldcb = N
    if ldcb is not None:
        d.ldcb = ldcb
    if tc is not None:
        d.tc_d, d.tc_h, d.tc_w, d.tc_cout = tc
    d.bias = bias.data_ptr() if bias is not None else None
    d.res = res.data_ptr() if res is not None else None
    d.ldr, d.res_mod = ldr, res_mod
    d.pre = pre.data_ptr() if pre is not None else None
    d.aux = aux.data_ptr() if aux is not None else None
    d.ldaux = ldaux
    d.act, d.accumulate, d.alpha = act, int(accumulate), alpha
    ws = workspace(A.device)
    call("unetr_gemm_bf16", ctypes.byref(d), A.data_ptr(), B.data_ptr(), C.data_ptr() if C is not None else None,
         Cb.data_ptr() if Cb is not None else None, ws.data_ptr(), ws.numel() * 4, _stream())


_SHADOW = {}
_WEIGHT_EPOCH = [0]


def mark_flat_maintained(params, state=None):
    if state is None and params:
        state = _GRAD_SINK.get(params[0].data_ptr())
    if state is not None and not state.unmaintained:
        return
    for w in params:
        ent = _SHADOW.get(id(w))
        if ent is not None and ent[4]() is w and ent[5] == w.data_ptr():
            ent[1], ent[3] = w._version, True
    if state is not None:
        state.unmaintained = 0


def invalidate_weight_shadows():
    _WEIGHT_EPOCH[0] += 1
    for ent in _SHADOW.values():
        ent[1] = -1
    for ent in _SHADOW_X3.values():
        ent[1] = -1
    for ent in _PACKS.values():
        ent[1] = -1


def begin_forward(state=None):
    if not torch.cuda.is_current_stream_capturing():
        _WEIGHT_EPOCH[0] += 1
    if state is not None:
        state.reset_deferred()
        state.fuse = None


_SHADOW_X3 = {}


def x3_words_enabled():
    return os.environ.get("UNETR_AMD_X3_WORDS", "1") != "0"


def _split_words(src, dst, n):
    call("unetr_split_words", src.data_ptr(), dst.data_ptr(), n, _stream())


def weight_x3(w):
    if not x3_words_enabled():
        return None
    st = _GRAD_SINK.get(w.data_ptr())
    flat = getattr(st, "flat", None) if st is not None else None
    if flat is None:
        return None
    if flat.get("shadow_x3") is None:
        if torch.cuda.is_current_stream_capturing():
            return None
        arena = torch.empty(flat["total"], dtype=torch.int32, device=w.device)
        _split_words(flat["param"], arena, flat["total"])
        flat["shadow_x3"] = arena
        for p, o in zip(flat["params"], flat["offsets"]):
            _SHADOW_X3[id(p)] = [arena[o:o + p.numel()].view_as(p), p._version, weakref.ref(p), p.data_ptr(), (p.numel() + 7) // 8 * 8]
    ent = _SHADOW_X3.get(id(w))
    if ent is None or ent[2]() is not w or ent[3] != w.data_ptr() or ent[0].device != w.device:
        return None
    if ent[1] != w._version:
        _split_words(w, ent[0], ent[4])
        ent[1] = w._version
    return ent[0]


def refresh_x3_shadow(flat, written=False):
    arena = flat.get("shadow_x3") if flat is not None else None
    if arena is None:
        return
    if not written:
        _split_words(flat["param"], arena, flat["total"])
    for p in flat["params"]:
        ent = _SHADOW_X3.get(id(p))
        if ent is not None and ent[2]() is p and ent[3] == p.data_ptr():
            ent[1] = p._version


def register_weight_shadow(w, shadow):
    _SHADOW[id(w)] = [shadow, w._version, _WEIGHT_EPOCH[0], True, weakref.ref(w), w.data_ptr()]


def weight_bf16(w):
    ent = _SHADOW.get(id(w))
    if ent is None or ent[4]() is not w or ent[0].shape != w.shape or ent[0].device != w.device:
        ent = [torch.empty(w.shape, dtype=torch.bfloat16, device=w.device), -1, -1, False, weakref.ref(w), 0]
        _SHADOW[id(w)] = ent
    fresh = ent[1] == w._version and ent[5] == w.data_ptr() and (
        ent[3] or (ent[2] == _WEIGHT_EPOCH[0] and not torch.cuda.is_current_stream_capturing()))
    if not fresh:
        cast_bf16(w.detach(), out=ent[0])
        ent[1], ent[2], ent[5], ent[3] = w._version, _WEIGHT_EPOCH[0], w.data_ptr(), False
        st = _GRAD_SINK.get(w.data_ptr())
        if st is not None:
            st.unmaintained += 1
    return ent[0]


_PACKS = {}


def conv_pack_get(w, kind, prec):
    key = (id(w), kind, prec)
    ent = _PACKS.get(key)
    cout, cin = w.shape[0], w.shape[1]
    if ent is None or ent[4]() is not w or ent[0].device != w.device:
        lib = _capi.load()
        if kind == 4:
            nbytes = w.numel() * 2
        else:
            nbytes = lib.unetr_conv3_packed_bytes(cin, cout, kind, prec) if kind <= 1 else (
                lib.unetr_conv3_packed_1x1_bytes(cin, cout, prec) if kind == 2 else lib.unetr_conv3_packed_1x1_bytes(cout, cin, prec))
        ent = [torch.empty(nbytes, dtype=torch.uint8, device=w.device), -1, -1, False, weakref.ref(w), 0]
        _PACKS[key] = ent
    fresh = ent[1] == w._version and ent[5] == w.data_ptr() and (
        ent[3] or (ent[2] == _WEIGHT_EPOCH[0] and not torch.cuda.is_current_stream_capturing()))
    if not fresh:
        _pack_launch([(w, ent[0], cin, cout, kind)], prec)
        ent[1], ent[2], ent[5], ent[3] = w._version, _WEIGHT_EPOCH[0], w.data_ptr(), False
    return ent[0]


def _pack_launch(items, prec):
    arr = (_capi.PackProblem * len(items))()
    for i, (w, buf, cin, cout, kind) in enumerate(items):
        arr[i].w, arr[i].out, arr[i].Cin, arr[i].Cout, arr[i].kind = w.data_ptr(), buf.data_ptr(), cin, cout, kind
    call("unetr_conv3_pack_grouped", arr, len(items), prec, _stream())


def refresh_conv_packs():
    by_prec = {}
    for key, ent in list(_PACKS.items()):
        w = ent[4]()
        if w is None:
            del _PACKS[key]
            continue
        if not w.is_cuda or ent[1] != w._version or ent[5] != w.data_ptr():
            continue
        by_prec.setdefault(key[2], []).append((w, ent[0], w.shape[1], w.shape[0], key[1]))
        ent[3] = True
    for prec, items in by_prec.items():
        _pack_launch(items, prec)


def shadow_ptr_for_update(w):
    ent = _SHADOW.get(id(w))
    if ent is None or ent[4]() is not w or ent[1] != w._version or ent[5] != w.data_ptr():
        return None
    ent[3] = True
    return ent[0].data_ptr()


def _bf16_path(prec, *kdims):
    return prec == _capi.PREC_BF16 and all(k % 64 == 0 for k in kdims)


def _twin(t):
    if t.dtype == torch.bfloat16:
        return t
    tw = getattr(t, "_unetr_bf16", None)
    if tw is not None and tw[0].numel() == t.numel() and tw[1] == t._version and t.is_contiguous():
        return tw[0].view(t.shape)
    return cast_bf16(t)


def _attach_twin(t, tb):
    t._unetr_bf16 = (tb, t._version)


def carry_twin(src, dst):
    tw = getattr(src, "_unetr_bf16", None)
    if tw is not None and tw[1] == src._version:
        dst._unetr_bf16 = (tw[0], dst._version)
    if hasattr(src, "_unetr_ln"):
        dst._unetr_ln = src._unetr_ln
    return dst


def add_cast(a, b, want_bf16=True):
    a, b = a.contiguous(), b.contiguous()
    out = torch.empty_like(a)
    ok16 = want_bf16 and a.numel() % 4 == 0
    ob = torch.empty(a.shape, dtype=torch.bfloat16, device=a.device) if ok16 else None
    if a.numel() % 4 or a.dtype != torch.float32 or b.dtype != torch.float32:
        raise RuntimeError("add_cast needs fp32 tensors with a multiple of 4 elements")
    call("unetr_add_cast_bf16", a.data_ptr(), b.data_ptr(), out.data_ptr(), _p(ob), a.numel(), _stream())
    if ob is not None:
        _attach_twin(out, ob)
    return out


class TapFn(torch.autograd.Function):

    @staticmethod
    def forward(ctx, x, want_bf16):
        ctx.want_bf16 = bool(want_bf16)
        a, b = x.view_as(x), x.view_as(x)
        carry_twin(x, a)
        carry_twin(x, b)
        return a, b

    @staticmethod
    def backward(ctx, ga, gb):
        if ga is None or gb is None:
            return (ga if gb is None else gb), None
        _require_gpu(ga)
        return add_cast(ga, gb, ctx.want_bf16), None


def linear_fwd(x, w, bias, prec, res=None, res_mod=0, act=0, pre=None):
    M, K = x.shape
    N = w.shape[0]
    y = torch.empty(M, N, dtype=torch.float32, device=x.device)
    gemm(x, w, y, M, N, K, lda=K, ldb=K, ldc=N, prec=prec, bias=bias, res=res, ldr=N, res_mod=res_mod, act=act, pre=pre,
         b_words=weight_x3(w) if prec == _capi.PREC_BF16X3 else None)
    return y


def linear_dgrad(dy, w, prec, aux=None):
    M, N = dy.shape
    K = w.shape[1]
    dx = torch.empty(M, K, dtype=torch.float32, device=dy.device)
    gemm(dy, w, dx, M, K, N, lda=N, ldb=K, ldc=K, prec=prec, b_trans=True, aux=aux, ldaux=K, act=2 if aux is not None else 0,
         b_words=weight_x3(w) if prec == _capi.PREC_BF16X3 else None)
    return dx


def linear_wgrad(dy, x, prec, out=None):
    M, N = dy.shape
    K = x.shape[1]
    dw = out if out is not None else torch.empty(N, K, dtype=torch.float32, device=dy.device)
    gemm(dy, x, dw, N, K, M, lda=N, ldb=K, ldc=K, prec=prec, a_trans=True, b_trans=True)
    return dw


def colsum(x, M, N, ld, out=None):
    if out is None:
        out = torch.empty(N, dtype=torch.float32, device=x.device)
    ws = workspace(x.device)
    call("unetr_colsum", x.data_ptr(), ld, M, N, out.data_ptr(), 0, ws.data_ptr(), ws.numel() * 4, _stream())
    return out


def _p(t):
    return t.data_ptr() if t is not None else None


def bf16_like(t):
    return torch.empty(t.shape, dtype=torch.bfloat16, device=t.device)


def layernorm_fwd(x, w, b, bf16_out=None, want_fp32=True):
    M, H = x.shape
    y = torch.empty_like(x) if want_fp32 else None
    mean = torch.empty(M, dtype=torch.float32, device=x.device)
    rstd = torch.empty(M, dtype=torch.float32, device=x.device)
    call("unetr_layernorm_fwd", x.data_ptr(), w.data_ptr(), b.data_ptr(), _p(y), _p(bf16_out), mean.data_ptr(),
         rstd.data_ptr(), M, H, LN_EPS, _stream())
    return y, mean, rstd


def layernorm_bwd(dy, x, w, mean, rstd, dres=None, out_w=None, out_b=None, dx_bf16=None):
    M, H = x.shape
    dx = torch.empty_like(x)
    dw = out_w if out_w is not None else torch.empty(H, dtype=torch.float32, device=x.device)
    db = out_b if out_b is not None else torch.empty(H, dtype=torch.float32, device=x.device)
    ws = workspace(x.device)
    call("unetr_layernorm_bwd", dy.data_ptr(), x.data_ptr(), w.data_ptr(), mean.data_ptr(), rstd.data_ptr(), dx.data_ptr(),
         _p(dx_bf16), dres.data_ptr() if dres is not None else None, dw.data_ptr(), db.data_ptr(), M, H, ws.data_ptr(), ws.numel() * 4, _stream())
    return dx, dw, db


def layernorm_bwd_params(dy, x, w, b, mean, rstd, dres=None, dx_bf16=None):
    ow, ob = _gout(w), _gout(b)
    if ow is None or ob is None:
        dx, dw, db = layernorm_bwd(dy, x, w, mean, rstd, dres=dres, out_w=ow, out_b=ob, dx_bf16=dx_bf16)
        return dx, _ret(w, dw), _ret(b, db)
    M, H = x.shape
    nblk = (M + 3) // 4
    part = torch.empty(nblk * 2 * H, dtype=torch.float32, device=x.device)
    dx = torch.empty_like(x)
    call("unetr_layernorm_bwd", dy.data_ptr(), x.data_ptr(), w.data_ptr(), mean.data_ptr(), rstd.data_ptr(), dx.data_ptr(),
         _p(dx_bf16), _p(dres), None, None, M, H, part.data_ptr(), part.numel() * 4, _stream())
    st = _GRAD_SINK[w.data_ptr()]
    st.defer["colsum"].append((part, ow, nblk, H, 2 * H))
    st.defer["colsum"].append((part[H:], ob, nblk, H, 2 * H))
    _arm_flush(st)
    return dx, _ret(w, ow, deferred=True), _ret(b, ob, deferred=True)


def x3_ride_ok(M, N, K):
    return M >= 32 and K % 32 == 0 and N % 4 == 0 and N >= 64 and os.environ.get("UNETR_X3_GEMM_DMA", "1") != "0"


def gemm_bf16_ln_fwd(A, B, M, N, K, C, gamma, beta, y_bf16, bias=None, res=None, ldr=0, y=None, b_words=None):
    x3 = A.dtype == torch.float32
    assert x3 or (A.dtype == torch.bfloat16 and B.dtype == torch.bfloat16)
    d = GemmBf16Desc()
    d.x3 = (2 if b_words is not None else 1) if x3 else 0
    if b_words is not None:
        B = b_words
    d.M, d.N, d.K, d.b_kn = M, N, K, 0
    d.lda, d.ldb, d.ldc, d.ldcb = K, K, N, N
    d.bias = bias.data_ptr() if bias is not None else None
    d.res = res.data_ptr() if res is not None else None
    d.ldr, d.alpha = ldr, 1.0
    mean = torch.empty(M, dtype=torch.float32, device=C.device)
    rstd = torch.empty(M, dtype=torch.float32, device=C.device)
    ws = workspace(C.device)
    call("unetr_gemm_bf16_ln_fwd", ctypes.byref(d), A.data_ptr(), B.data_ptr(), C.data_ptr(), gamma.data_ptr(), beta.data_ptr(), LN_EPS,
         _p(y), _p(y_bf16), mean.data_ptr(), rstd.data_ptr(), ws.data_ptr(), ws.numel() * 4, _stream())
    return mean, rstd


def ln_ride_enabled():
    return os.environ.get("UNETR_AMD_LN_RIDE", "1") == "1"


def _stash_ln(x, gamma, beta, xn, mean, rstd):
    x._unetr_ln = (xn, mean, rstd, gamma.data_ptr(), gamma._version, beta.data_ptr(), beta._version, x._version)


def _stashed_ln(x, gamma, beta):
    st = getattr(x, "_unetr_ln", None)
    if st is None or st[3:] != (gamma.data_ptr(), gamma._version, beta.data_ptr(), beta._version, x._version) or st[0].shape != x.shape:
        return None
    return st[0], st[1], st[2]


def gemm_ln_bwd_params(A, Bw, M, N, K, x, w, b, mean, rstd, dres=None, dx_bf16=None, b_words=None):
    x3 = A.dtype == torch.float32
    assert x3 or (A.dtype == torch.bfloat16 and Bw.dtype == torch.bfloat16)
    d = GemmBf16Desc()
    d.x3 = (2 if b_words is not None else 1) if x3 else 0
    if b_words is not None:
        Bw = b_words
    d.M, d.N, d.K, d.b_kn = M, N, K, 1
    d.lda, d.ldb, d.ldc, d.ldcb = K, N, N, N
    d.alpha = 1.0
    scratch = torch.empty(M, N, dtype=torch.float32, device=x.device)
    dx = torch.empty_like(x)
    ws = workspace(x.device)
    ow, ob = _gout(w), _gout(b)
    nblk = (M + 3) // 4
    if ow is None or ob is None:
        dw = ow if ow is not None else torch.empty(N, dtype=torch.float32, device=x.device)
        db = ob if ob is not None else torch.empty(N, dtype=torch.float32, device=x.device)
        lnws = torch.empty(nblk * 2 * N, dtype=torch.float32, device=x.device)
        call("unetr_gemm_bf16_ln_bwd", ctypes.byref(d), A.data_ptr(), Bw.data_ptr(), scratch.data_ptr(), x.data_ptr(), w.data_ptr(),
             mean.data_ptr(), rstd.data_ptr(), dx.data_ptr(), _p(dx_bf16), _p(dres), dw.data_ptr(), db.data_ptr(),
             lnws.data_ptr(), lnws.numel() * 4, ws.data_ptr(), ws.numel() * 4, _stream())
        return dx, _ret(w, dw), _ret(b, db)
    part = torch.empty(nblk * 2 * N, dtype=torch.float32, device=x.device)
    call("unetr_gemm_bf16_ln_bwd", ctypes.byref(d), A.data_ptr(), Bw.data_ptr(), scratch.data_ptr(), x.data_ptr(), w.data_ptr(),
         mean.data_ptr(), rstd.data_ptr(), dx.data_ptr(), _p(dx_bf16), _p(dres), None, None,
         part.data_ptr(), part.numel() * 4, ws.data_ptr(), ws.numel() * 4, _stream())
    st = _GRAD_SINK[w.data_ptr()]
    st.defer["colsum"].append((part, ow, nblk, N, 2 * N))
    st.defer["colsum"].append((part[N:], ob, nblk, N, 2 * N))
    _arm_flush(st)
    return dx, _ret(w, ow, deferred=True), _ret(b, ob, deferred=True)


def attention_fwd(qkv, B, L, heads, dh, prec, out_bf16=None):
    out = torch.empty(B * L, heads * dh, dtype=torch.float32, device=qkv.device)
    lse = torch.empty(B, heads, L, dtype=torch.float32, device=qkv.device)
    call("unetr_attention_fwd", qkv.data_ptr(), out.data_ptr(), _p(out_bf16), lse.data_ptr(), B, L, heads, dh, float(dh) ** -0.5, prec, _stream())
    return out, lse


def attention_bwd(qkv, out, dout, lse, B, L, heads, dh, prec, dqkv_bf16=None):
    dqkv = torch.empty_like(qkv)
    delta = torch.empty_like(lse)
    call("unetr_attention_bwd", qkv.data_ptr(), out.data_ptr(), dout.data_ptr(), lse.data_ptr(), dqkv.data_ptr(), _p(dqkv_bf16),
         delta.data_ptr(),
         B, L, heads, dh, float(dh) ** -0.5, prec, _stream())
    return dqkv


def attention_bf16_fwd(qkvb, B, L, heads, dh, out_bf16, out=None):
    lse = torch.empty(B, heads, L, dtype=torch.float32, device=qkvb.device)
    call("unetr_attention_bf16_fwd", qkvb.data_ptr(), _p(out), out_bf16.data_ptr(), lse.data_ptr(), B, L, heads, dh, float(dh) ** -0.5, _stream())
    return lse


def attention_bf16_bwd(qkvb, outb, doutb, lse, B, L, heads, dh, dqkv=None):
    dqkvb = torch.empty_like(qkvb)
    delta = torch.empty_like(lse)
    call("unetr_attention_bf16_bwd", qkvb.data_ptr(), outb.data_ptr(), doutb.data_ptr(), lse.data_ptr(), _p(dqkv), dqkvb.data_ptr(),
         delta.data_ptr(), B, L, heads, dh, float(dh) ** -0.5, _stream())
    return dqkvb


def conv3(x, ldx, w, dims, prec, mode=0, out=None, ldo=None, accumulate=False):
    B, D, H, W = dims
    cout_w, cin_w = w.shape[0], w.shape[1]
    cin, cout = (cin_w, cout_w) if mode == 0 else (cout_w, cin_w)
    if cout % 16 != 0:
        return conv_fwd(x, ldx, conv_pack(w, mode), dims, cin, cout, 3, prec, out=out, ldo=ldo, accumulate=accumulate)
    wp = conv_pack_get(w, mode, prec)
    if out is None:
        out = torch.empty(B, D, H, W, cout, dtype=act_dtype(prec), device=x.device)
        ldo = cout
    call("unetr_conv3_fwd", x.data_ptr(), ldx, wp.data_ptr(), out.data_ptr(), ldo, int(accumulate), B, D, H, W, cin, cout, prec, _stream())
    return out


def conv3_fused(x, ldx, w, w3, dims, prec):
    B, D, H, W = dims
    cout, cin = w.shape[0], w.shape[1]
    if cout % 16 != 0:
        return None
    dev = x.device
    wp = conv_pack_get(w, 0, prec)
    adt = act_dtype(prec)
    x_f32 = int(prec == _capi.PREC_BF16 and x.dtype == torch.float32)
    c = torch.empty(B, D, H, W, cout, dtype=adt, device=dev)
    st = torch.empty(B, cout, 2, dtype=torch.float32, device=dev)
    wp3 = c3 = st3 = None
    if w3 is not None:
        wp3 = conv_pack_get(w3, 2, prec)
        c3 = torch.empty(B, D, H, W, cout, dtype=adt, device=dev)
        st3 = torch.empty(B, cout, 2, dtype=torch.float32, device=dev)
    ws = workspace(dev)
    rc = call_rc("unetr_conv3_fwd_fused", x.data_ptr(), ldx, wp.data_ptr(), c.data_ptr(), cout, st.data_ptr(), _p(wp3), _p(c3), cout,
                 _p(st3), IN_EPS, B, D, H, W, cin, cout, prec, x_f32, ws.data_ptr(), ws.numel() * 4, _stream())
    if rc != 0:
        return None
    return c, st, c3, st3


CONV3_MAX_ROWS = 1024


def in_fuse_level():
    return int(os.environ.get("UNETR_AMD_IN_FUSE", "3"))


def conv3_parts(x, ldx, w, w3, dims, prec, store3=True):
    B, D, H, W = dims
    cout, cin = w.shape[0], w.shape[1]
    if cout % 16 != 0 or cout > 128:
        return None
    dev = x.device
    wp = conv_pack_get(w, 0, prec)
    adt = act_dtype(prec)
    x_f32 = int(prec == _capi.PREC_BF16 and x.dtype == torch.float32)
    c = torch.empty(B, D, H, W, cout, dtype=adt, device=dev)
    part = torch.empty(B, CONV3_MAX_ROWS, 2, cout, dtype=torch.float32, device=dev)
    wp3 = c3 = part3 = None
    if w3 is not None:
        wp3 = conv_pack_get(w3, 2, prec)
        c3 = torch.empty(B, D, H, W, cout, dtype=adt, device=dev) if store3 else None
        part3 = torch.empty(B, CONV3_MAX_ROWS, 2, cout, dtype=torch.float32, device=dev)
    rows = ctypes.c_int(0)
    rc = call_rc("unetr_conv3_fwd_parts", x.data_ptr(), ldx, wp.data_ptr(), c.data_ptr(), cout, part.data_ptr(), _p(wp3), _p(c3), cout,
                 _p(part3), ctypes.byref(rows), B, D, H, W, cin, cout, prec, x_f32, _stream())
    if rc != 0:
        return None
    return c, part, c3, part3, rows.value


def instnorm_apply_fin(x, part, rows, B, V, C, lrelu, x2=None, part_b=None, rows_b=0, out=None, ldo=None):
    y = torch.empty_like(x) if out is None else out
    sa = torch.empty(B, C, 2, dtype=torch.float32, device=x.device)
    sb = torch.empty(B, C, 2, dtype=torch.float32, device=x.device) if x2 is not None else None
    rc = call_rc("unetr_instnorm_apply_fin", x.data_ptr(), C, part.data_ptr(), rows, _p(x2), C, _p(part_b), rows_b, sa.data_ptr(), _p(sb),
                 IN_EPS, y.data_ptr(), C if out is None else ldo, B, V, C, int(lrelu), _a16(x), _stream())
    if rc != 0:
        return None
    return y, sa, sb


# ... 261 lines not shown
        rows = _capi.load().unetr_tconv2_wgrad_rows(B, D, H, W, cin, cout)
        n = cin * cout * 8
        if rows > 0:
            part = torch.empty(rows * n, dtype=torch.float32, device=x.device)
            got = ctypes.c_long(0)
            if call_rc("unetr_tconv2_wgrad_parts", x.data_ptr(), ldx, dy.data_ptr(), lddy, part.data_ptr(), part.numel() * 4, ctypes.byref(got),
                       B, D, H, W, cin, cout, prec, _stream()) == 0:
                st.defer["reduce"].append((part, gw, n, got.value))
                _arm_flush(st)
                return dx, _ret(w, gw, deferred=True)
    dw = tconv_wgrad(x, ldx, dy, lddy, dims, cin, cout, prec, out=gw)
    return dx, _ret(w, dw)


def tconv_dgrad(dy, lddy, w, dims, cin, cout, prec):
    B, D, H, W = dims
    dx = torch.empty(B, D, H, W, cin, dtype=act_dtype(prec), device=dy.device)
    ws = workspace(dy.device)
    args = (dy.data_ptr(), lddy, w.data_ptr(), dx.data_ptr(), cin, 0, B, D, H, W, cin, cout, prec, ws.data_ptr(), ws.numel() * 4, _stream())
    if call_rc("unetr_tconv2_dgrad", *args) != 0:
        if prec == _capi.PREC_BF16:
            d32 = dy.float().contiguous() if lddy == cout else dy[..., :cout].float().contiguous()
            x32 = torch.empty(B, D, H, W, cin, dtype=torch.float32, device=dy.device)
            call("unetr_tconv_dgrad", d32.data_ptr(), cout, w.data_ptr(), x32.data_ptr(), cin, 0, B, D, H, W, cin, cout, prec,
                 ws.data_ptr(), ws.numel() * 4, _stream())
            dx.copy_(x32)
        else:
            call("unetr_tconv_dgrad", *args)
    return dx


def tconv_wgrad(x, ldx, dy, lddy, dims, cin, cout, prec, out=None):
    B, D, H, W = dims
    dw = out if out is not None else torch.empty(cin, cout, 2, 2, 2, dtype=torch.float32, device=x.device)
    ws = workspace(x.device)
    args = (x.data_ptr(), ldx, dy.data_ptr(), lddy, dw.data_ptr(), B, D, H, W, cin, cout, prec, ws.data_ptr(), ws.numel() * 4, _stream())
    if call_rc("unetr_tconv2_wgrad", *args) != 0:
        if prec == _capi.PREC_BF16:
            x32 = x.float().contiguous() if ldx == cin else x[..., :cin].float().contiguous()
            d32 = dy.float().contiguous() if lddy == cout else dy[..., :cout].float().contiguous()
            call("unetr_tconv_wgrad", x32.data_ptr(), cin, d32.data_ptr(), cout, dw.data_ptr(), B, D, H, W, cin, cout, prec,
                 ws.data_ptr(), ws.numel() * 4, _stream())
        else:
            call("unetr_tconv_wgrad", *args)
    return dw


class PatchEmbedFn(torch.autograd.Function):

    @staticmethod
    def forward(ctx, x_in, w, b, pos, patch, prec):
        _require_gpu(x_in)
        x_in = x_in.contiguous()
        B, C, D, H, W = x_in.shape
        L = (D // patch) * (H // patch) * (W // patch)
        pd = C * patch ** 3
        hid = w.shape[0]
        ctx.pb = None
        if _bf16_path(prec, pd) and (B * L) % 8 == 0 and hid % 8 == 0:
            z = torch.empty(B * L, hid, dtype=torch.float32, device=x_in.device)
            ctx.pb = torch.empty(B * L, pd, dtype=torch.bfloat16, device=x_in.device)
            patches = x_in.new_empty(0)
            call("unetr_patch_gather", x_in.data_ptr(), None, ctx.pb.data_ptr(), B, C, D, H, W, patch, _stream())
            gemm_bf16(ctx.pb, weight_bf16(w), B * L, hid, pd, C=z, bias=b, res=pos, ldr=hid, res_mod=L)
        else:
            patches = torch.empty(B * L, pd, dtype=torch.float32, device=x_in.device)
            call("unetr_patch_gather", x_in.data_ptr(), patches.data_ptr(), None, B, C, D, H, W, patch, _stream())
            z = linear_fwd(patches, w, b, prec, res=pos, res_mod=L)
        ctx.save_for_backward(patches, w, b, pos)
        ctx.meta = (B, L, hid, prec)
        return z

    @staticmethod
    def backward(ctx, dz):
        patches, w, b, pos = ctx.saved_tensors
        B, L, hid, prec = ctx.meta
        dz = dz.contiguous()
        dw = wgrad_or_defer(dz, patches, prec, w, _twin(dz) if ctx.pb is not None else None, ctx.pb)
        db = colsum_or_defer(dz, B * L, hid, hid, b)
        dpos = colsum_or_defer(dz, B, L * hid, L * hid, pos, view_shape=(1, L, hid))
        return None, dw, db, dpos, None, None


def _tblock_forward(x, n1w, n1b, wqkv, wp, bp, n2w, n2b, w1, b1, w2, b2, B, L, heads, prec, train, next_ln=None, emit_twin=False):
    hid = x.shape[1]
    dh = hid // heads
    M, mlp = x.shape[0], w1.shape[0]
    if _bf16_path(prec, hid, mlp) and M % 8 == 0:
        f32 = dict(dtype=torch.float32, device=x.device)
        y1 = y2 = a = x.new_empty(0)
        b16att = dh == 64
        qkv = torch.empty(M, 3 * hid, dtype=torch.bfloat16 if b16att else torch.float32, device=x.device)
        pre = _stashed_ln(x, n1w, n1b)
        if pre is not None:
            y1b, m1, r1 = pre
        else:
            y1b = bf16_like(x)
            _, m1, r1 = layernorm_fwd(x, n1w, n1b, bf16_out=y1b, want_fp32=False)
        gemm_bf16(y1b, weight_bf16(wqkv), M, 3 * hid, hid, C=None if b16att else qkv, Cb=qkv if b16att else None)
        attb = bf16_like(x)
        if b16att:
            att = x.new_empty(0)
            lse = attention_bf16_fwd(qkv, B, L, heads, dh, attb)
        else:
            att, lse = attention_fwd(qkv, B, L, heads, dh, prec, out_bf16=attb)
        x1 = torch.empty(M, hid, **f32)
        gemm_bf16(attb, weight_bf16(wp), M, hid, hid, C=x1, bias=bp, res=x, ldr=hid)
        u = torch.empty(M, mlp, **f32) if train else None
        ab = torch.empty(M, mlp, dtype=torch.bfloat16, device=x.device)
        y2b = bf16_like(x)
        _, m2, r2 = layernorm_fwd(x1, n2w, n2b, bf16_out=y2b, want_fp32=False)
        gemm_bf16(y2b, weight_bf16(w1), M, mlp, hid, Cb=ab, bias=b1, act=1, pre=u)
        if not train:
            u = m1 = r1 = m2 = r2 = y1b = y2b = x.new_empty(0)
        x2 = torch.empty(M, hid, **f32)
        if next_ln is not None and not emit_twin:
            xn = bf16_like(x)
            mn, rn = gemm_bf16_ln_fwd(ab, weight_bf16(w2), M, hid, mlp, x2, next_ln[0], next_ln[1], xn, bias=b2, res=x1, ldr=hid)
            _stash_ln(x2, next_ln[0], next_ln[1], xn, mn, rn)
        else:
            x2b = bf16_like(x) if emit_twin else None
            gemm_bf16(ab, weight_bf16(w2), M, hid, mlp, C=x2, Cb=x2b, bias=b2, res=x1, ldr=hid)
            if x2b is not None:
                _attach_twin(x2, x2b)
        twins = (y1b, attb, y2b, ab)
    else:
        twins = None
        x3ride = prec == _capi.PREC_BF16X3 and ln_ride_enabled() and x3_ride_ok(M, hid, mlp)
        pre = _stashed_ln(x, n1w, n1b) if x3ride else None
        y1, m1, r1 = pre if pre is not None else layernorm_fwd(x, n1w, n1b)
        qkv = linear_fwd(y1, wqkv, None, prec)
        att, lse = attention_fwd(qkv, B, L, heads, dh, prec)
        x1 = linear_fwd(att, wp, bp, prec, res=x)
        y2, m2, r2 = layernorm_fwd(x1, n2w, n2b)
        u = torch.empty(M, mlp, dtype=torch.float32, device=x.device)
        a = linear_fwd(y2, w1, b1, prec, act=1, pre=u)
        if x3ride and next_ln is not None:
            x2 = torch.empty(M, hid, dtype=torch.float32, device=x.device)
            xn = torch.empty_like(x2)
            mn, rn = gemm_bf16_ln_fwd(a, w2, M, hid, mlp, x2, next_ln[0], next_ln[1], None, bias=b2, res=x1, ldr=hid, y=xn, b_words=weight_x3(w2))
            _stash_ln(x2, next_ln[0], next_ln[1], xn, mn, rn)
        else:
            x2 = linear_fwd(a, w2, b2, prec, res=x1)
    return x2, (y1, m1, r1, qkv, att, lse, x1, y2, m2, r2, u, a), twins


class TransformerBlockFn(torch.autograd.Function):

    @staticmethod
    def forward(ctx, x, n1w, n1b, wqkv, wp, bp, n2w, n2b, w1, b1, w2, b2, B, L, heads, prec, ckpt=False, next_n1w=None, next_n1b=None,
                emit_twin=False):
        _require_gpu(x)
        xc = x.contiguous()
        if xc is not x and hasattr(x, "_unetr_ln"):
            xc._unetr_ln = x._unetr_ln
        x = xc
        train = any(ctx.needs_input_grad[:12])
        x2, acts, twins = _tblock_forward(x, n1w, n1b, wqkv, wp, bp, n2w, n2b, w1, b1, w2, b2, B, L, heads, prec,
                                          train and not ckpt, None if next_n1w is None else (next_n1w, next_n1b), bool(emit_twin))
        ctx.ckpt = bool(ckpt) and train
        if ctx.ckpt:
            acts, twins = (), None
        ctx.twins = twins
        ctx.save_for_backward(x, n1w, wqkv, wp, n2w, w1, w2, n1b, bp, n2b, b1, b2, *acts)
        ctx.meta = (B, L, heads, x.shape[1] // heads, prec)
        return x2

    @staticmethod
    def backward(ctx, dx2):
        x, n1w, wqkv, wp, n2w, w1, w2, n1b, bp, n2b, b1, b2, *acts = ctx.saved_tensors
        B, L, heads, dh, prec = ctx.meta
        twins = ctx.twins
        if ctx.ckpt:
            _, acts, twins = _tblock_forward(x, n1w, n1b, wqkv, wp, bp, n2w, n2b, w1, b1, w2, b2, B, L, heads, prec, True)
        y1, m1, r1, qkv, att, lse, x1, y2, m2, r2, u, a = acts
        M, hid = x.shape
        dx2 = dx2.contiguous()
        mlp = w1.shape[0]
        fast = _bf16_path(prec, hid, mlp) and M % 8 == 0
        f32 = dict(dtype=torch.float32, device=x.device)
        y1b = attb = y2b = ab = dx2b = dub = None
        if fast:
            if twins is not None:
                y1b, attb, y2b, ab = twins
            dx2b = _twin(dx2)
            du, dub = None, torch.empty(M, mlp, dtype=torch.bfloat16, device=x.device)
            gemm_bf16(dx2b, weight_bf16(w2), M, mlp, hid, b_kn=True, Cb=dub, act=2, aux=u, ldaux=mlp)
        else:
            du = linear_dgrad(dx2, w2, prec, aux=u)
        dw2 = wgrad_or_defer(dx2, a, prec, w2, dx2b, ab)
        db2 = colsum_or_defer(dx2, M, hid, hid, b2)
        dw1 = wgrad_or_defer(du, y2, prec, w1, dub, y2b)
        db1 = colsum_or_defer(dub if fast else du, M, mlp, mlp, b1)
        if fast:
            dx1b = bf16_like(x)
            dx1, dn2w, dn2b = gemm_ln_bwd_params(dub, weight_bf16(w1), M, hid, mlp, x1, n2w, n2b, m2, r2, dres=dx2, dx_bf16=dx1b)
        else:
            dx1b = None
            if prec == _capi.PREC_BF16X3 and ln_ride_enabled() and x3_ride_ok(M, hid, mlp):
                dx1, dn2w, dn2b = gemm_ln_bwd_params(du, w1, M, hid, mlp, x1, n2w, n2b, m2, r2, dres=dx2, b_words=weight_x3(w1))
            else:
                dy2 = linear_dgrad(du, w1, prec)
                dx1, dn2w, dn2b = layernorm_bwd_params(dy2, x1, n2w, n2b, m2, r2, dres=dx2, dx_bf16=dx1b)
        b16att = fast and qkv.dtype == torch.bfloat16
        if b16att:
            dattb = bf16_like(x)
            gemm_bf16(dx1b, weight_bf16(wp), M, hid, hid, b_kn=True, Cb=dattb)
        elif fast:
            datt = torch.empty(M, hid, **f32)
            gemm_bf16(dx1b, weight_bf16(wp), M, hid, hid, b_kn=True, C=datt)
        else:
            datt = linear_dgrad(dx1, wp, prec)
        dwp = wgrad_or_defer(dx1, att, prec, wp, dx1b, attb)
        dbp = colsum_or_defer(dx1, M, hid, hid, bp)
        if b16att:
            dqkv = None
            dqkvb = attention_bf16_bwd(qkv, attb, dattb, lse, B, L, heads, dh)
        else:
            dqkvb = torch.empty(M, 3 * hid, dtype=torch.bfloat16, device=x.device) if fast else None
            dqkv = attention_bwd(qkv, att, datt, lse, B, L, heads, dh, prec, dqkv_bf16=dqkvb)
        dwqkv = wgrad_or_defer(dqkv, y1, prec, wqkv, dqkvb, y1b)
        if fast:
            dxb = bf16_like(x)
            dx, dn1w, dn1b = gemm_ln_bwd_params(dqkvb, weight_bf16(wqkv), M, hid, 3 * hid, x, n1w, n1b, m1, r1, dres=dx1, dx_bf16=dxb)
        else:
            dxb = None
            if prec == _capi.PREC_BF16X3 and ln_ride_enabled() and x3_ride_ok(M, hid, 3 * hid):
                dx, dn1w, dn1b = gemm_ln_bwd_params(dqkv, wqkv, M, hid, 3 * hid, x, n1w, n1b, m1, r1, dres=dx1, b_words=weight_x3(wqkv))
            else:
                dy1 = linear_dgrad(dqkv, wqkv, prec)
                dx, dn1w, dn1b = layernorm_bwd_params(dy1, x, n1w, n1b, m1, r1, dres=dx1, dx_bf16=dxb)
        if fast:
            _attach_twin(dx, dxb)
        return (dx, dn1w, dn1b, dwqkv, dwp, dbp, dn2w, dn2b, dw1, db1, dw2, db2, None, None, None, None, None, None, None, None)


class LayerNormFn(torch.autograd.Function):
    @staticmethod
    def forward(ctx, x, w, b, twin=False):
        _require_gpu(x)
        x = x.contiguous()
        yb = bf16_like(x) if twin else None
        y, mean, rstd = layernorm_fwd(x, w, b, bf16_out=yb)
        if yb is not None:
            _attach_twin(y, yb)
        ctx.save_for_backward(x, w, mean, rstd, b)
        ctx.twin = bool(twin)
        return y

    @staticmethod
    def backward(ctx, dy):
        x, w, mean, rstd, b = ctx.saved_tensors
        dxb = bf16_like(x) if ctx.twin else None
        dx, dw, db = layernorm_bwd_params(dy.contiguous(), x, w, b, mean, rstd, dx_bf16=dxb)
        if dxb is not None:
            _attach_twin(dx, dxb)
        return dx, dw, db, None


def skip_half(dims, C, prec, device):
    cat = torch.empty(*dims, 2 * C, dtype=act_dtype(prec), device=device)
    return cat, cat[..., C:]


def cat_of_skip(skip, C):
    B, D, H, W, c = skip.shape
    want = (D * H * W * 2 * C, H * W * 2 * C, W * 2 * C, 2 * C, 1)
    if c != C or tuple(skip.stride()) != want or skip.storage_offset() != C or skip.untyped_storage().nbytes() != B * want[0] * skip.element_size():
        raise RuntimeError("skip_in_cat=True needs the second half of a buffer made by functional.skip_half")
    return skip.as_strided((B, D, H, W, 2 * C), want, 0)


def _resblock_fwd(x, ldx, dims, cin, cout, w1, w2, w3, prec, to_cat=False, head=None):
    B, D, H, W = dims
    V = D * H * W
    if in_fuse_level() & 1:
        r = _resblock_fwd_fin(x, ldx, dims, cout, w1, w2, w3, prec, to_cat, head if out_fuse_enabled() else None)
        if r is not None:
            return r if head is not None else r[:2]
    f1 = conv3_fused(x, ldx, w1, w3, dims, prec)
    if f1 is not None:
        c1, s1, c3, s3 = f1
    else:
        f1 = conv3_fused(x, ldx, w1, None, dims, prec)
        if f1 is not None:
            c1, s1 = f1[0], f1[1]
        else:
            c1 = conv3(x, ldx, w1, dims, prec)
            s1 = instnorm_stats(c1, cout, B, V, cout)
        x32 = x if x.dtype == torch.float32 else x.float()
        c3 = torch.empty(B, D, H, W, cout, dtype=torch.float32, device=x.device)
        gemm(x32, w3, c3, B * V, cout, cin, lda=x32.stride(-2), ldb=cin, ldc=cout, prec=prec)
        c3 = _as_act(c3, prec)
        s3 = instnorm_stats(c3, cout, B, V, cout)
    a1 = instnorm_apply(c1, s1, B, V, cout, True)
    f2 = conv3_fused(a1, cout, w2, None, dims, prec)
    if f2 is not None:
        c2, s2 = f2[0], f2[1]
    else:
        c2 = conv3(a1, cout, w2, dims, prec)
        s2 = instnorm_stats(c2, cout, B, V, cout)
    if to_cat:
        _, half = skip_half(dims, cout, prec, x.device)
        out = instnorm_apply(c2, s2, B, V, cout, True, x2=c3, sb=s3, out=half, ldo=2 * cout)
    else:
        out = instnorm_apply(c2, s2, B, V, cout, True, x2=c3, sb=s3)
    if head is not None:
        return out, (c1, s1, a1, c2, s2, c3, s3), False
    return out, (c1, s1, a1, c2, s2, c3, s3)


def _materialize_c3(x, w3, dims, cin, cout, prec):
    B, D, H, W = dims
    V = D * H * W
    c3f = torch.empty(B * V, cout, dtype=torch.float32, device=x.device)
    gemm(x.reshape(B * V, cin), w3, c3f, B * V, cout, cin, lda=cin, ldb=cin, ldc=cout, prec=prec)
    return _as_act(c3f.view(B, D, H, W, cout), prec)


def _resblock_fwd_fin(x, ldx, dims, cout, w1, w2, w3, prec, to_cat, head=None):
    B, D, H, W = dims
    V = D * H * W
    cin = w1.shape[1]
    img = (x.dtype == torch.float32 and cin <= 4 and ldx == cin and not x.requires_grad and w3.is_contiguous()
           and cout % 8 == 0 and 64 % max(1, cout // 8) == 0)
    f1 = conv3_parts(x, ldx, w1, w3, dims, prec, store3=not img)
    if f1 is None and img:
        img = False
        f1 = conv3_parts(x, ldx, w1, w3, dims, prec)
    if f1 is None:
        return None
    c1, p1, c3, p3, rows1 = f1
    r1 = instnorm_apply_fin(c1, p1, rows1, B, V, cout, True)
    if r1 is None:
        return None
    a1, s1, _ = r1
    f2 = conv3_parts(a1, cout, w2, None, dims, prec)
    if f2 is None:
        return None
    c2, p2, _, _, rows2 = f2
# ... 294 lines not shown
```

### 3dmedicalimagesegmentation_amd/unetr.py

```python
import os
from typing import Tuple, Union

import torch
import torch.nn as nn

try:
    from . import _capi
    from . import functional as Fn
except ImportError:
    import importlib
    import sys
    _here = os.path.dirname(os.path.abspath(__file__))
    if os.path.dirname(_here) not in sys.path:
        sys.path.insert(0, os.path.dirname(_here))
    _pkg = importlib.import_module(os.path.basename(_here))
    _capi, Fn = _pkg._capi, _pkg.functional

_PRECISIONS = {"fp32": _capi.PREC_F32, "bf16": _capi.PREC_BF16, "bf16x3": _capi.PREC_BF16X3}


def default_precision() -> str:
    return os.environ.get("UNETR_AMD_PRECISION", "fp32")


# ... 194 lines not shown
        with torch.no_grad():
            for p, o in zip(params, offs):
                v = flat_p[o:o + p.numel()].view_as(p)
                v.copy_(p)
                p.data = v
                p.grad = None
                views.append((p, flat_g[o:o + p.numel()].view_as(p)))
        old = getattr(self, "_arena_state", None)
        if old is not None:
            old.clear()
        self._arena_state = Fn.register_grad_sinks(views, Fn.ArenaState())
        shadow = Fn.cast_bf16(flat_p)
        for p, o in zip(params, offs):
            Fn.register_weight_shadow(p, shadow[o:o + p.numel()].view_as(p))
        self._flat = dict(param=flat_p, grad=flat_g, offsets=offs, params=params, total=n, shadow=shadow,
                          state=self._arena_state)
        self._arena_state.flat = self._flat
        return self._flat

    backward_stage_starts = (8, 4, 1)

    def _pass_of_block(self, j):
        return 1 + sum(1 for s in self.backward_stage_starts if s > j)

    def stage_ranges(self):
        flat = getattr(self, "_flat", None)
        if flat is None:
            raise RuntimeError("stage_ranges() needs use_flat_buffers()")
        index = {id(p): i for i, p in enumerate(flat["params"])}
        offs = flat["offsets"]
        first = lambda m: offs[index[id(next(m.parameters()))]]
        conv = first(self.encoder1)
        bounds = [conv] + [first(self.vit.blocks[s]) for s in sorted(self.backward_stage_starts, reverse=True)] + [0]
        return [(conv, flat["total"])] + [(lo, hi) for hi, lo in zip(bounds[:-1], bounds[1:])]

    def _prec(self) -> int:
        try:
            return _PRECISIONS[self.precision]
        except KeyError:
            raise ValueError(f"precision must be one of {sorted(_PRECISIONS)}, got {self.precision!r}")

    def proj_feat(self, x, hidden_size, feat_size):
        x = x.view(x.size(0), feat_size[0], feat_size[1], feat_size[2], hidden_size)
        x = x.permute(0, 4, 1, 2, 3).contiguous()
        return x

    def _tokens_cl(self, tok, B):
        g = self.feat_size
        return Fn.carry_twin(tok, tok.view(B, g[0], g[1], g[2], self.hidden_size))

    def _res_w(self, blk):
        return blk.conv1.conv.weight, blk.conv2.conv.weight, blk.conv3.conv.weight

    def _encode(self, x_in, prec, stages=None):
        B = x_in.shape[0]
        if tuple(x_in.shape[1:]) != (self.in_channels, *self.img_size):
            raise ValueError(f"expected input [B,{self.in_channels},{self.img_size}], got {tuple(x_in.shape)}")
        pe = self.vit.patch_embedding
        lin = pe.patch_embeddings[1]
        L = pe.position_embeddings.shape[1]
        Fn._require_gpu(x_in)

        def cut(t, k):
            if stages is None:
                return t
            leaf = Fn.carry_twin(t, t.detach().requires_grad_(True))
            stages[k].append((t, leaf))
            return leaf

        ckpt = self.encoder_checkpointing and torch.is_grad_enabled()
        x = Fn.PatchEmbedFn.apply(x_in, lin.weight, lin.bias, pe.position_embeddings, self.patch_size[0], prec)
        hidden_states_out = []
        nblk = len(self.vit.blocks)
        starts = set(self.backward_stage_starts)
        b16 = Fn._bf16_path(prec, self.hidden_size, self.vit.blocks[0].mlp.linear1.weight.shape[0])
        taps = (3, 6, 9)
        for i, blk in enumerate(self.vit.blocks):
            nxt = self.vit.blocks[i + 1].norm1 if i + 1 < nblk and Fn.ln_ride_enabled() else None
            x = Fn.TransformerBlockFn.apply(
                x, blk.norm1.weight, blk.norm1.bias, blk.attn.qkv.weight, blk.attn.out_proj.weight, blk.attn.out_proj.bias,
                blk.norm2.weight, blk.norm2.bias, blk.mlp.linear1.weight, blk.mlp.linear1.bias, blk.mlp.linear2.weight,
                blk.mlp.linear2.bias, B, L, self.num_heads, prec, ckpt,
                None if nxt is None else nxt.weight.detach(), None if nxt is None else nxt.bias.detach(),
                i in taps)
            k = self._pass_of_block(i) - 1
            if i in taps:
                xa, xb = Fn.TapFn.apply(x, b16)
                hidden_states_out.append(cut(xb, k))
                x = cut(xa, k) if (i + 1) in starts else xa
            else:
                if (i + 1) in starts:
                    x = cut(x, k)
                hidden_states_out.append(x)
        x = Fn.LayerNormFn.apply(x, self.vit.norm.weight, self.vit.norm.bias,
                                 Fn._bf16_path(prec, self.hidden_size, self.vit.blocks[0].mlp.linear1.weight.shape[0]))
        x = cut(x, 0)
        enc1 = Fn.ResBlockFn.apply(Fn.to_channels_last(x_in), *self._res_w(self.encoder1.layer), prec, True)
        enc = []
        for tap, blk in ((3, self.encoder2), (6, self.encoder3), (9, self.encoder4)):
            t = Fn.TconvFn.apply(self._tokens_cl(hidden_states_out[tap], B), blk.transp_conv_init.conv.weight, prec, len(blk.blocks) == 0)
            for k, sub in enumerate(blk.blocks):
                t = Fn.TconvFn.apply(t, sub.conv.weight, prec, k == len(blk.blocks) - 1)
            enc.append(t)
        return x, enc1, enc[0], enc[1], enc[2]

    def _decode(self, x_in, x, enc1, enc2, enc3, enc4, prec):
        B = x_in.shape[0]
        dec4 = self._tokens_cl(x, B)
        d = self.decoder5
        dec3 = Fn.UpBlockFn.apply(dec4, enc4, d.transp_conv.conv.weight, *self._res_w(d.conv_block), prec, True)
        d = self.decoder4
        dec2 = Fn.UpBlockFn.apply(dec3, enc3, d.transp_conv.conv.weight, *self._res_w(d.conv_block), prec, True)
        d = self.decoder3
        dec1 = Fn.UpBlockFn.apply(dec2, enc2, d.transp_conv.conv.weight, *self._res_w(d.conv_block), prec, True)
        d = self.decoder2
        logits = Fn.UpBlockFn.apply(dec1, enc1, d.transp_conv.conv.weight, *self._res_w(d.conv_block), prec, True,
                                    self.out.conv.conv.weight, self.out.conv.conv.bias)
        return Fn.ToNCDHWFn.apply(enc4), logits

    def forward(self, x_in, freeze_encoder=False):
        prec = self._prec()
        Fn._require_gpu(x_in)
        Fn.begin_forward(getattr(self, "_arena_state", None))
        if freeze_encoder:
            with torch.no_grad():
                x, enc1, enc2, enc3, enc4 = self._encode(x_in, prec)
        else:
            x, enc1, enc2, enc3, enc4 = self._encode(x_in, prec)
        return self._decode(x_in, x, enc1, enc2, enc3, enc4, prec)

    def forward_staged(self, x_in):
        prec = self._prec()
        Fn._require_gpu(x_in)
        Fn.begin_forward(getattr(self, "_arena_state", None))
        stages = [[] for _ in range(len(self.backward_stage_starts) + 1)]
        x, enc1, enc2, enc3, enc4 = self._encode(x_in, prec, stages)
        enc4_out, logits = self._decode(x_in, x, enc1, enc2, enc3, enc4, prec)
        return enc4_out, logits, stages

    @staticmethod
    def backward_staged(loss, stages, after_stage=None):
        loss.backward()
        if after_stage is not None:
            after_stage(0)
        for k, st in enumerate(stages, 1):
            roots = [r for r, leaf in st if leaf.grad is not None]
            grads = [leaf.grad for r, leaf in st if leaf.grad is not None]
            if roots:
                torch.autograd.backward(roots, grads)
            if after_stage is not None:
                after_stage(k)


class UNETRLogits(UNETR):

    def forward(self, x_in):
        return super().forward(x_in)[1]
```

### include/unetr_hip.h

```cpp
#ifndef UNETR_HIP_H
#define UNETR_HIP_H
#include <stddef.h>
#ifdef __cplusplus
extern "C" {
#endif

#define UNETR_ABI_VERSION 21
int unetr_abi_version(void);

typedef struct {
    int M, N, K, batch;
    int a_trans, b_trans;
    long lda, ldb, ldc;
    long strideA, strideB, strideC;
    const float* bias;
    const float* res;
    long ldr, strideR;
    int res_mod;
    float* pre;
    const float* aux;
    long ldaux;
    int act;
    int accumulate;
    float alpha;
    int prec;
    int b_x3words;
} unetr_gemm_desc;
int unetr_gemm(const unetr_gemm_desc* d, const float* A, const float* B, float* C,
               float* ws, size_t ws_bytes, void* stream);
int unetr_split_words(const float* src, void* dst, long n, void* stream);

typedef struct {
    int M, N, K, b_kn;
    long lda, ldb, ldc, ldcb;
    const float* bias;
    const float* res;
    long ldr;
    int res_mod;
    float* pre;
    const float* aux;
    long ldaux;
    int act;
    int accumulate;
    float alpha;
    int tc_d, tc_h, tc_w, tc_cout;
    int x3;
} unetr_gemm_bf16_desc;
int unetr_gemm_bf16(const unetr_gemm_bf16_desc* d, const void* A, const void* B, float* C, void* Cb,
                    float* ws, size_t ws_bytes, void* stream);
int unetr_cast_bf16(const float* src, void* dst, long n, void* stream);
int unetr_split_stack_bf16(const float* src, void* dst, long rows, long cols, int second, void* stream);
typedef struct { const float* src; void* dst; long rows, cols; int second; } unetr_split_problem;
int unetr_split_stack_bf16_grouped(const unetr_split_problem* probs, int n, void* stream);
int unetr_add_cast_bf16(const float* a, const float* b, float* out, void* out_bf16, long n, void* stream);

typedef struct { const float* dy; const float* x; float* dw; int M, N, K; } unetr_grouped_problem;
int unetr_gemm_grouped_wgrad(const unetr_grouped_problem* probs, int n, int prec, void* stream);
int unetr_gemm_bf16_grouped_wgrad(const unetr_grouped_problem* probs, int n, void* stream);
typedef struct { const void* x; float* out; long ld; int M, N, x_bf16; } unetr_colsum_problem;
int unetr_colsum_grouped(const unetr_colsum_problem* probs, int n, void* stream);

int unetr_tconv_fwd(const float* x, long ldx, const float* w, float* y, long ldy,
                    int B, int D, int H, int W, int Cin, int Cout, int prec,
                    float* ws, size_t ws_bytes, void* stream);
int unetr_tconv_dgrad(const float* dy, long ldy, const float* w, float* dx, long ldx, int accumulate,
                      int B, int D, int H, int W, int Cin, int Cout, int prec,
                      float* ws, size_t ws_bytes, void* stream);
int unetr_tconv_wgrad(const float* x, long ldx, const float* dy, long ldy, float* dw,
                      int B, int D, int H, int W, int Cin, int Cout, int prec,
                      float* ws, size_t ws_bytes, void* stream);
int unetr_tconv2_fwd(const void* x, long ldx, const float* w, void* y, long ldy,
                     int B, int D, int H, int W, int Cin, int Cout, int prec,
                     float* ws, size_t ws_bytes, void* stream);
int unetr_tconv2_wgrad(const void* x, long ldx, const void* dy, long ldy, float* dw,
                       int B, int D, int H, int W, int Cin, int Cout, int prec,
                       float* ws, size_t ws_bytes, void* stream);
int unetr_tconv2_dgrad(const void* dy, long ldy, const float* w, void* dx, long ldx, int accumulate,
                       int B, int D, int H, int W, int Cin, int Cout, int prec,
                       float* ws, size_t ws_bytes, void* stream);
long unetr_tconv2_wgrad_rows(int B, int D, int H, int W, int Cin, int Cout);
int unetr_tconv2_wgrad_parts(const void* x, long ldx, const void* dy, long ldy, float* part, size_t part_bytes, long* rows_out,
                             int B, int D, int H, int W, int Cin, int Cout, int prec, void* stream);
int unetr_tconv2_fwd_supported(long M, int Cin, int Cout, long ldx, long ldy);
int unetr_tconv2_wgrad_supported(long M, int Cin, int Cout, long ldx, long lddy);


int unetr_attention_bf16_fwd(const void* qkv, float* out, void* out_bf16, float* lse, int B, int L, int heads, int dh,
                             float scale, void* stream);
int unetr_attention_bf16_bwd(const void* qkv, const void* out_bf16, const void* dout_bf16, const float* lse, float* dqkv,
                             void* dqkv_bf16, float* delta, int B, int L, int heads, int dh, float scale, void* stream);

int unetr_pixel_shuffle2(const float* t, void* y, long ldy, int B, int D, int H, int W, int Cout, int act16, void* stream);
int unetr_pixel_unshuffle2_bf16(const void* dy, long lddy, void* g_bf16, int B, int D, int H, int W, int Cout, int act16, void* stream);

int unetr_colsum(const float* x, long ld, int M, int N, float* out, int accumulate,
                 float* ws, size_t ws_bytes, void* stream);

int unetr_layernorm_fwd(const float* x, const float* gamma, const float* beta, float* y,
                        void* y_bf16 ,
                        float* mean, float* rstd, int M, int H, float eps, void* stream);
int unetr_layernorm_bwd(const float* dy, const float* x, const float* gamma, const float* mean,
                        const float* rstd, float* dx, void* dx_bf16 ,
                        const float* dres , float* dgamma, float* dbeta,
                        int M, int H, float* ws, size_t ws_bytes, void* stream);

int unetr_gemm_bf16_ln_bwd(const unetr_gemm_bf16_desc* d, const void* A, const void* B, float* C,
                           const float* x, const float* gamma, const float* mean, const float* rstd,
                           float* dx, void* dx_bf16, const float* dres, float* dgamma, float* dbeta,
                           float* ln_ws, size_t ln_ws_bytes, float* ws, size_t ws_bytes, void* stream);

int unetr_gemm_bf16_ln_fwd(const unetr_gemm_bf16_desc* d, const void* A, const void* B, float* C,
                           const float* gamma, const float* beta, float eps, float* y, void* y_bf16, float* mean, float* rstd,
                           float* ws, size_t ws_bytes, void* stream);

int unetr_attention_fwd(const float* qkv, float* out, void* out_bf16 , float* lse,
                        int B, int L, int heads, int dh, float scale, int prec, void* stream);
int unetr_attention_bwd(const float* qkv, const float* out, const float* dout, const float* lse,
                        float* dqkv, void* dqkv_bf16 , float* delta,
                        int B, int L, int heads, int dh, float scale, int prec, void* stream);

int unetr_conv_pack_weight(const float* w, float* wpack, int Cin, int Cout, int KS, int mode, void* stream);
int unetr_conv_gemm_fwd(const float* x, long ldx, const float* wpack, float* y, long ldy, int accumulate,
                        int B, int D, int H, int W, int Cin, int Cout, int KS, int prec,
                        float* ws, size_t ws_bytes, void* stream);
int unetr_conv_gemm_wgrad(const float* x, long ldx, const float* dy, long ldy, float* dw,
                          int B, int D, int H, int W, int Cin, int Cout, int KS, int prec,
                          float* ws, size_t ws_bytes, void* stream);

size_t unetr_conv3_packed_bytes(int Cin, int Cout, int mode, int prec);
int unetr_conv3_pack_weight(const float* w, void* wpack, int Cin, int Cout, int mode, int prec, void* stream);
int unetr_conv3_fwd(const void* x, long ldx, const void* wpack, void* y, long ldy, int accumulate,
                    int B, int D, int H, int W, int Cin, int Cout, int prec, void* stream);
int unetr_conv3_fwd_fused(const void* x, long ldx, const void* wpack, void* y, long ldy, float* stats,
                          const void* w3pack, void* y3, long ldy3, float* stats3, float eps,
                          int B, int D, int H, int W, int Cin, int Cout, int prec,
                          int x_f32 ,
                          float* ws, size_t ws_bytes, void* stream);
#define UNETR_CONV3_MAX_ROWS 1024
int unetr_conv3_fwd_parts(const void* x, long ldx, const void* wpack, void* y, long ldy, float* part,
                          const void* w3pack, void* y3, long ldy3, float* part3, int* rows_out,
                          int B, int D, int H, int W, int Cin, int Cout, int prec, int x_f32, void* stream);
int unetr_conv3_dgrad_stats(const void* dy, long lddy, const void* wpack_dgrad, void* dx, long lddx,
                            const void* xn, long ldxn, const float* stats, float* part, int* rows_out,
                            int B, int D, int H, int W, int Cin, int Cout, int prec, void* stream);
size_t unetr_conv3_packed_1x1_bytes(int Cin, int Cout, int prec);
int unetr_conv3_pack_1x1(const float* w3 , void* w3pack, int Cin, int Cout, int prec, void* stream);
int unetr_conv3_dgrad_fused(const void* dc1, long ld1, const void* wpack_dgrad, const void* dc3, long ld3, const float* w3,
                            const void* w3pack_t ,
                            void* dx, long lddx, int B, int D, int H, int W, int Cin, int Cout, int prec,
                            float* ws, size_t ws_bytes, void* stream);
typedef struct { const float* w; void* out; int Cin, Cout, kind; } unetr_pack_problem;
int unetr_conv3_pack_grouped(const unetr_pack_problem* probs, int n, int prec, void* stream);
int unetr_instnorm_stats_finalize(const float* part, int nchunk, int B, long V, int C, float eps, float* stats, void* stream);
int unetr_conv3_wgrad(const void* x, long ldx, const void* dy, long ldy, float* dw,
                      const void* dy3, long ldy3, float* dw3,
                      int B, int D, int H, int W, int Cin, int Cout, int prec, int x_f32 ,
                      float* ws, size_t ws_bytes, void* stream);
long unetr_conv3_wgrad_rows(int B, int D, int H, int W, int Cin, int Cout, int prec, int x_f32, int has3);
int unetr_conv3_wgrad_parts(const void* x, long ldx, const void* dy, long ldy, const void* dy3, long ldy3,
                            float* part, size_t part_bytes, long* rows_out, int B, int D, int H, int W, int Cin, int Cout, int prec,
                            int x_f32, void* stream);
typedef struct { const float* part; float* dst; long n; int rows; } unetr_reduce_problem;
int unetr_reduce_rows_grouped(const unetr_reduce_problem* probs, int n, void* stream);
int unetr_debug_tr16(const void* in_u16_64x64, void* out_u16_64x4, void* stream);

int unetr_instnorm_stats(const void* x, long ld, int B, long V, int C, float eps, float* stats,
                         float* ws, size_t ws_bytes, int act16, void* stream);
int unetr_instnorm_apply(const void* x, long ldx, const float* sa, const void* x2, long ldx2, const float* sb,
                         void* y, long ldy, int B, long V, int C, int lrelu, int act16, void* stream);
int unetr_instnorm_apply_fin(const void* x, long ldx, const float* part_a, int rows_a, const void* x2, long ldx2,
                             const float* part_b, int rows_b, float* stats_a, float* stats_b, float eps,
                             void* y, long ldy, int B, long V, int C, int lrelu, int act16, void* stream);
int unetr_instnorm_bwd_apply_fin(const void* dy, long lddy, const void* x, long ldx, const float* sa,
                                 const void* x2, long ldx2, const float* sb, const float* part, int nrows, int nsp,
                                 void* dx, long lddx, void* dx2, long lddx2, int B, long V, int C, int lrelu, int act16, void* stream);
#define UNETR_IN_IMG_MAX_ROWS 512
int unetr_instnorm_apply_fin_img(const void* x, long ldx, const float* part_a, int rows_a, const float* img, int Cin, const float* w3,
                                 const float* part_b, int rows_b, float* stats_a, float* stats_b, float eps,
                                 void* y, long ldy, int B, long V, int C, int lrelu, int act16, void* stream);
int unetr_instnorm_bwd_img(const void* dy, long lddy, const void* x, long ldx, const float* sa, const float* img, int Cin,
                           const float* w3, const float* sb, void* dx, long lddx, float* dw3_part, int* rows_out,
                           int B, long V, int C, int lrelu, float* ws, size_t ws_bytes, int act16, void* stream);
int unetr_instnorm_bwd(const void* dy, long lddy, const void* x, long ldx, const float* sa,
                       const void* x2, long ldx2, const float* sb, void* dx, long lddx, void* dx2, long lddx2,
                       int B, long V, int C, int lrelu, float* ws, size_t ws_bytes, int act16, void* stream);

int unetr_nchw_to_nhwc(const float* x , void* y , long ldy, int B, int C, long V, int act16, void* stream);
int unetr_nhwc_to_nchw(const void* x , long ldx, float* y , int B, int C, long V, int accumulate, int act16, void* stream);
int unetr_patch_gather(const float* x, float* patches, void* patches_bf16, int B, int C, int D, int H, int W, int P, void* stream);
int unetr_counter_add(float* y, const float* inc, int n, void* stream);
int unetr_copy_rows(void* y, long ldy, const void* a, long lda, long rows, int cols, int accumulate, int act16, void* stream);

int unetr_outconv_fwd(const void* x, long ldx, const float* w, const float* bias, float* logits,
                      int B, long V, int Cin, int Cout, int act16, void* stream);
int unetr_outconv_bwd(const float* dlogits, const void* x, long ldx, const float* w, void* dx, long lddx,
                      float* dw, float* dbias, int B, long V, int Cin, int Cout,
// ... 84 lines not shown
```

Before: 465.2 volumes/s.

## Add prefetch-rider blocks that warm upcoming layer weights into cache during memory-bound kernels

```diff
diff --git a/3dmedicalimagesegmentation_amd/_capi.py b/3dmedicalimagesegmentation_amd/_capi.py
--- a/3dmedicalimagesegmentation_amd/_capi.py
+++ b/3dmedicalimagesegmentation_amd/_capi.py
@@ -60,6 +60,10 @@
     _fields_ = [("src", c_void_p), ("dst", c_void_p), ("rows", c_long), ("cols", c_long), ("second", c_int)]
 
 
+class Prefetch(ctypes.Structure):
+    _fields_ = [("ptr", c_void_p * 2), ("bytes", c_size_t * 2)]
+
+
 class ColsumProblem(ctypes.Structure):
     _fields_ = [("x", c_void_p), ("out", c_void_p), ("ld", c_long), ("M", c_int), ("N", c_int), ("x_bf16", c_int)]
 
@@ -77,13 +81,17 @@
     "unetr_gemm": [ctypes.POINTER(GemmDesc), P, P, P, P, c_size_t, P],
     "unetr_gemm_bf16": [ctypes.POINTER(GemmBf16Desc), P, P, P, P, P, c_size_t, P],
     "unetr_gemm_bf16_ln_bwd": [ctypes.POINTER(GemmBf16Desc), P, P, P, P, P, P, P, P, P, P, P, P, P, c_size_t, P, c_size_t, P],
+    "unetr_gemm_bf16_ln_bwd_pf": [ctypes.POINTER(GemmBf16Desc), P, P, P, P, P, P, P, P, P, P, P, P, P, c_size_t, P, c_size_t, P, ctypes.POINTER(Prefetch)],
     "unetr_gemm_bf16_ln_fwd": [ctypes.POINTER(GemmBf16Desc), P, P, P, P, P, c_float, P, P, P, P, P, c_size_t, P],
+    "unetr_gemm_bf16_ln_fwd_pf": [ctypes.POINTER(GemmBf16Desc), P, P, P, P, P, c_float, P, P, P, P, P, c_size_t, P, ctypes.POINTER(Prefetch)],
     "unetr_cast_bf16": [P, P, c_long, P],
     "unetr_split_words": [P, P, c_long, P],
     "unetr_split_stack_bf16": [P, P, c_long, c_long, c_int, P],
     "unetr_split_stack_bf16_grouped": [ctypes.POINTER(SplitProblem), c_int, P],
     "unetr_attention_bf16_fwd": [P, P, P, P, c_int, c_int, c_int, c_int, c_float, P],
+    "unetr_attention_bf16_fwd_pf": [P, P, P, P, c_int, c_int, c_int, c_int, c_float, P, ctypes.POINTER(Prefetch)],
     "unetr_attention_bf16_bwd": [P, P, P, P, P, P, P, c_int, c_int, c_int, c_int, c_float, P],
+    "unetr_attention_bf16_bwd_pf": [P, P, P, P, P, P, P, c_int, c_int, c_int, c_int, c_float, P, ctypes.POINTER(Prefetch)],
     "unetr_gemm_grouped_wgrad": [ctypes.POINTER(GroupedProblem), c_int, c_int, P],
     "unetr_gemm_bf16_grouped_wgrad": [ctypes.POINTER(GroupedProblem), c_int, P],
     "unetr_gemm_bf16_grouped_wgrad_adamw": [ctypes.POINTER(GroupedProblem), c_int, ctypes.POINTER(AdamWArena), ctypes.POINTER(c_int), P],
@@ -103,7 +111,9 @@
     "unetr_pixel_unshuffle2_bf16": [P, c_long, P, c_int, c_int, c_int, c_int, c_int, c_int, P],
     "unetr_colsum": [P, c_long, c_int, c_int, P, c_int, P, c_size_t, P],
     "unetr_layernorm_fwd": [P, P, P, P, P, P, P, c_int, c_int, c_float, P],
+    "unetr_layernorm_fwd_pf": [P, P, P, P, P, P, P, c_int, c_int, c_float, P, ctypes.POINTER(Prefetch)],
     "unetr_layernorm_bwd": [P, P, P, P, P, P, P, P, P, P, c_int, c_int, P, c_size_t, P],
+    "unetr_layernorm_bwd_pf": [P, P, P, P, P, P, P, P, P, P, c_int, c_int, P, c_size_t, P, ctypes.POINTER(Prefetch)],
     "unetr_attention_fwd": [P, P, P, P, c_int, c_int, c_int, c_int, c_float, c_int, P],
     "unetr_attention_bwd": [P, P, P, P, P, P, P, c_int, c_int, c_int, c_int, c_float, c_int, P],
     "unetr_conv_pack_weight": [P, P, c_int, c_int, c_int, c_int, P],
diff --git a/3dmedicalimagesegmentation_amd/csrc/attention_b16.hip b/3dmedicalimagesegmentation_amd/csrc/attention_b16.hip
--- a/3dmedicalimagesegmentation_amd/csrc/attention_b16.hip
+++ b/3dmedicalimagesegmentation_amd/csrc/attention_b16.hip
@@ -124,8 +124,9 @@
 template <int NW>
 __global__ void __launch_bounds__(64 * NW)
 attn16_fwd_kernel(const uint16_t* __restrict__ qkv, float* __restrict__ out, uint16_t* __restrict__ outb, float* __restrict__ lse,
-                  int L, int heads, float scale) {
+                  int L, int heads, float scale, PrefetchRider pf) {
     constexpr int NT = 64 * NW;
+    if (pf.nblk && blockIdx.z == gridDim.z - 1) { prefetch_rider_block(pf, blockIdx.y * gridDim.x + blockIdx.x); return; }
     extern __shared__ __attribute__((aligned(1024))) char lds[];
     char* kimg = lds;
     char* vimg = lds + IMG;
@@ -409,7 +410,8 @@
 __global__ void __launch_bounds__(64 * NW)
 attn16_bwd_kernel(const uint16_t* __restrict__ qkv, const uint16_t* __restrict__ outb, const uint16_t* __restrict__ doutb,
                   const float* __restrict__ lse, float* __restrict__ delta, float* __restrict__ dqkv, uint16_t* __restrict__ dqkvb,
-                  int L, int heads, float scale, int nqb) {
+                  int L, int heads, float scale, int nqb, PrefetchRider pf) {
+    if (pf.nblk && blockIdx.z == gridDim.z - 1) { prefetch_rider_block(pf, blockIdx.y * gridDim.x + blockIdx.x); return; }
     extern __shared__ __attribute__((aligned(1024))) char lds[];
     const int xb = __builtin_amdgcn_readfirstlane(blockIdx.x);
     if (xb < nqb) attn16_bwd_dq_body<NW>(lds, xb, qkv, outb, doutb, lse, delta, dqkv, dqkvb, L, heads, scale);
@@ -429,26 +431,39 @@
     return (nw == 4 && (long)cdiv(L, 64) * heads * B > 1024) ? 8 : nw;
 }
 
-}
-
-extern "C" int unetr_attention_bf16_fwd(const void* qkv, float* out, void* out_bf16, float* lse, int B, int L, int heads, int dh,
-                                        float scale, void* stream) {
+inline PrefetchRider attn_rider(const unetr_prefetch* pf, int gx, int heads, int B) {
+    return B < 65535 ? prefetch_rider(pf, 0, gx * heads) : prefetch_rider(nullptr, 0);
+}
+
+}
+
+extern "C" int unetr_attention_bf16_fwd_pf(const void* qkv, float* out, void* out_bf16, float* lse, int B, int L, int heads, int dh,
+                                           float scale, void* stream, const unetr_prefetch* pf) {
     if (!qkv || (!out && !out_bf16) || !lse || B <= 0 || L <= 0 || heads <= 0 || B > 65535 || heads > 65535) return UNETR_ERR_ARG;
     if (dh != DH || ((uintptr_t)qkv & 15) || (out && ((uintptr_t)out & 15)) || (out_bf16 && ((uintptr_t)out_bf16 & 7))) return UNETR_ERR_UNSUPPORTED;
     hipStream_t st = (hipStream_t)stream;
     const size_t lds = 2 * IMG;
     const int nw = pick_nw_fwd(B, L, heads);
+    const int gx = cdiv(L, 16 * nw);
+    const PrefetchRider rd = attn_rider(pf, gx, heads, B);
+    const dim3 grid(gx, heads, B + (rd.nblk ? 1 : 0));
     if (nw == 2)
-        launch_dyn(attn16_fwd_kernel<2>, dim3(cdiv(L, 32), heads, B), 128, lds, st, (const uint16_t*)qkv, out, (uint16_t*)out_bf16, lse, L, heads, scale);
+        launch_dyn(attn16_fwd_kernel<2>, grid, 128, lds, st, (const uint16_t*)qkv, out, (uint16_t*)out_bf16, lse, L, heads, scale, rd);
     else if (nw == 4)
-        launch_dyn(attn16_fwd_kernel<4>, dim3(cdiv(L, 64), heads, B), 256, lds, st, (const uint16_t*)qkv, out, (uint16_t*)out_bf16, lse, L, heads, scale);
+        launch_dyn(attn16_fwd_kernel<4>, grid, 256, lds, st, (const uint16_t*)qkv, out, (uint16_t*)out_bf16, lse, L, heads, scale, rd);
     else
-        launch_dyn(attn16_fwd_kernel<8>, dim3(cdiv(L, 128), heads, B), 512, lds, st, (const uint16_t*)qkv, out, (uint16_t*)out_bf16, lse, L, heads, scale);
+        launch_dyn(attn16_fwd_kernel<8>, grid, 512, lds, st, (const uint16_t*)qkv, out, (uint16_t*)out_bf16, lse, L, heads, scale, rd);
     return unetr_check_launch();
 }
 
-extern "C" int unetr_attention_bf16_bwd(const void* qkv, const void* out_bf16, const void* dout_bf16, const float* lse, float* dqkv,
-                                        void* dqkv_bf16, float* delta, int B, int L, int heads, int dh, float scale, void* stream) {
+extern "C" int unetr_attention_bf16_fwd(const void* qkv, float* out, void* out_bf16, float* lse, int B, int L, int heads, int dh,
+                                        float scale, void* stream) {
+    return unetr_attention_bf16_fwd_pf(qkv, out, out_bf16, lse, B, L, heads, dh, scale, stream, nullptr);
+}
+
+extern "C" int unetr_attention_bf16_bwd_pf(const void* qkv, const void* out_bf16, const void* dout_bf16, const float* lse, float* dqkv,
+                                           void* dqkv_bf16, float* delta, int B, int L, int heads, int dh, float scale, void* stream,
+                                           const unetr_prefetch* pf) {
     if (!qkv || !out_bf16 || !dout_bf16 || !lse || !dqkv_bf16 || !delta || B <= 0 || L <= 0 || heads <= 0 || B > 65535 || heads > 65535)
         return UNETR_ERR_ARG;
     if (dh != DH || ((uintptr_t)qkv & 15) || ((uintptr_t)out_bf16 & 15) || ((uintptr_t)dout_bf16 & 15) || ((uintptr_t)dqkv_bf16 & 7) ||
@@ -462,10 +477,17 @@
     const size_t lk = 2 * IMG + 2 * CKEYS * sizeof(float);
     if (pick_nw(B, L, heads) == 2) {
         const int nqb = cdiv(L, 32);
-        launch_dyn(attn16_bwd_kernel<2>, dim3(2 * nqb, heads, B), 128, lk, st, q, o, d, lse, delta, dqkv, gq, L, heads, scale, nqb);
+        const PrefetchRider rd = attn_rider(pf, 2 * nqb, heads, B);
+        launch_dyn(attn16_bwd_kernel<2>, dim3(2 * nqb, heads, B + (rd.nblk ? 1 : 0)), 128, lk, st, q, o, d, lse, delta, dqkv, gq, L, heads, scale, nqb, rd);
     } else {
         const int nqb = cdiv(L, 64);
-        launch_dyn(attn16_bwd_kernel<4>, dim3(2 * nqb, heads, B), 256, lk, st, q, o, d, lse, delta, dqkv, gq, L, heads, scale, nqb);
+        const PrefetchRider rd = attn_rider(pf, 2 * nqb, heads, B);
+        launch_dyn(attn16_bwd_kernel<4>, dim3(2 * nqb, heads, B + (rd.nblk ? 1 : 0)), 256, lk, st, q, o, d, lse, delta, dqkv, gq, L, heads, scale, nqb, rd);
     }
     return unetr_check_launch();
 }
+
+extern "C" int unetr_attention_bf16_bwd(const void* qkv, const void* out_bf16, const void* dout_bf16, const float* lse, float* dqkv,
+                                        void* dqkv_bf16, float* delta, int B, int L, int heads, int dh, float scale, void* stream) {
+    return unetr_attention_bf16_bwd_pf(qkv, out_bf16, dout_bf16, lse, dqkv, dqkv_bf16, delta, B, L, heads, dh, scale, stream, nullptr);
+}
diff --git a/3dmedicalimagesegmentation_amd/csrc/common.hpp b/3dmedicalimagesegmentation_amd/csrc/common.hpp
--- a/3dmedicalimagesegmentation_amd/csrc/common.hpp
+++ b/3dmedicalimagesegmentation_amd/csrc/common.hpp
@@ -2,6 +2,7 @@
 #include "../../include/unetr_hip.h"
 #include <hip/hip_runtime.h>
 #include <stdint.h>
+#include <algorithm>
 
 typedef float f32x2 __attribute__((ext_vector_type(2)));
 typedef float f32x4 __attribute__((ext_vector_type(4)));
@@ -234,13 +235,56 @@
     const u32x4 w = *(const u32x4*)p;
     return ok ? P::from_raw(w) : (u32x4){0u, 0u, 0u, 0u};
 }
+struct PrefetchRider { const u32x4* p[2]; long u[2]; int upb, nblk; };
+
+static inline PrefetchRider prefetch_rider(const unetr_prefetch* pf, long block_bytes, int fixed_blocks = 0) {
+    PrefetchRider r{{nullptr, nullptr}, {0, 0}, 0, 0};
+    if (!pf) return r;
+    for (int i = 0; i < 2; ++i) {
+        if (!pf->ptr[i] || pf->bytes[i] < 16) continue;
+        const uintptr_t lo = ((uintptr_t)pf->ptr[i] + 15) & ~(uintptr_t)15, hi = ((uintptr_t)pf->ptr[i] + pf->bytes[i]) & ~(uintptr_t)15;
+        if (hi <= lo) continue;
+        r.p[i] = (const u32x4*)lo;
+        r.u[i] = (long)((hi - lo) >> 4);
+    }
+    const long total = r.u[0] + r.u[1];
+    if (total == 0) return r;
+    if (fixed_blocks > 0) {
+        r.nblk = fixed_blocks;
+        r.upb = (int)((total + fixed_blocks - 1) / fixed_blocks);
+    } else {
+        r.upb = (int)(block_bytes >> 4);
+        r.nblk = (int)std::min<long>((total + r.upb - 1) / r.upb, 4096);
+        r.upb = (int)((total + r.nblk - 1) / r.nblk);
+    }
+    return r;
+}
+
+constexpr int PF_FLIGHT = 8;
+__device__ __forceinline__ void prefetch_rider_block(const PrefetchRider& r, int rb) {
+    const long total = r.u[0] + r.u[1];
+    const long lo = (long)rb * r.upb, hi = min(lo + r.upb, total);
+    const int nt = blockDim.x;
+    for (long i = lo + threadIdx.x; i < hi; i += (long)nt * PF_FLIGHT) {
+        u32x4 v[PF_FLIGHT];
+#pragma unroll
+        for (int j = 0; j < PF_FLIGHT; ++j) {
+            const long k = min(i + (long)j * nt, hi - 1);
+            const u32x4* q = k < r.u[0] ? r.p[0] + k : r.p[1] + (k - r.u[0]);
+            v[j] = *q;
+        }
+#pragma unroll
+        for (int j = 0; j < PF_FLIGHT; ++j) asm volatile("" ::"v"(v[j]));
+    }
+}
+
 int unetr_layernorm_bwd_partials(const float* dy, int splits, long slab, const float* x, const float* gamma, const float* mean,
                                  const float* rstd, float* dx, void* dx_bf16, const float* dres, float* dgamma,
-                                 float* dbeta, int M, int H, float* ws, size_t ws_bytes, void* stream);
+                                 float* dbeta, int M, int H, float* ws, size_t ws_bytes, void* stream, const unetr_prefetch* pf = nullptr);
 
 int unetr_layernorm_fwd_partials(const float* partials, int splits, long slab, const float* bias, const float* res, long ldr, int res_mod,
                                  float* xout, const float* gamma, const float* beta, float* y, void* y_bf16, float* mean, float* rstd,
-                                 int M, int H, float eps, void* stream);
+                                 int M, int H, float eps, void* stream, const unetr_prefetch* pf = nullptr);
 
 int unetr_gemm_x3_dma(const unetr_gemm_bf16_desc* d, const float* A, const float* B, int b_words, float* C, float* ws, size_t ws_bytes, void* stream,
                       int* psp = nullptr);
diff --git a/3dmedicalimagesegmentation_amd/csrc/gemm_bf16.hip b/3dmedicalimagesegmentation_amd/csrc/gemm_bf16.hip
--- a/3dmedicalimagesegmentation_amd/csrc/gemm_bf16.hip
+++ b/3dmedicalimagesegmentation_amd/csrc/gemm_bf16.hip
@@ -866,30 +866,43 @@
     return gemm_bf16_impl(d, A, B, C, Cb, ws, ws_bytes, stream, nullptr);
 }
 
-extern "C" int unetr_gemm_bf16_ln_bwd(const unetr_gemm_bf16_desc* d, const void* A, const void* B, float* C,
-                                      const float* x, const float* gamma, const float* mean, const float* rstd,
-                                      float* dx, void* dx_bf16, const float* dres, float* dgamma, float* dbeta,
-                                      float* ln_ws, size_t ln_ws_bytes, float* ws, size_t ws_bytes, void* stream) {
+extern "C" int unetr_gemm_bf16_ln_bwd_pf(const unetr_gemm_bf16_desc* d, const void* A, const void* B, float* C,
+                                         const float* x, const float* gamma, const float* mean, const float* rstd,
+                                         float* dx, void* dx_bf16, const float* dres, float* dgamma, float* dbeta,
+                                         float* ln_ws, size_t ln_ws_bytes, float* ws, size_t ws_bytes, void* stream, const unetr_prefetch* pf) {
     if (!d || !C) return UNETR_ERR_ARG;
     if (d->bias || d->res || d->pre || d->act || d->accumulate || d->alpha != 1.f || d->ldc != d->N) return UNETR_ERR_UNSUPPORTED;
     int splits = 1;
     if (int e = gemm_bf16_impl(d, A, B, C, nullptr, ws, ws_bytes, stream, &splits)) return e;
     const float* dy = splits > 1 ? ws : C;
     return unetr_layernorm_bwd_partials(dy, splits, (long)d->M * d->N, x, gamma, mean, rstd, dx, dx_bf16, dres, dgamma, dbeta,
-                                        d->M, d->N, ln_ws, ln_ws_bytes, stream);
-}
-
-extern "C" int unetr_gemm_bf16_ln_fwd(const unetr_gemm_bf16_desc* d, const void* A, const void* B, float* C,
-                                      const float* gamma, const float* beta, float eps, float* y, void* y_bf16, float* mean, float* rstd,
-                                      float* ws, size_t ws_bytes, void* stream) {
+                                        d->M, d->N, ln_ws, ln_ws_bytes, stream, pf);
+}
+
+extern "C" int unetr_gemm_bf16_ln_bwd(const unetr_gemm_bf16_desc* d, const void* A, const void* B, float* C,
+                                      const float* x, const float* gamma, const float* mean, const float* rstd,
+                                      float* dx, void* dx_bf16, const float* dres, float* dgamma, float* dbeta,
+                                      float* ln_ws, size_t ln_ws_bytes, float* ws, size_t ws_bytes, void* stream) {
+    return unetr_gemm_bf16_ln_bwd_pf(d, A, B, C, x, gamma, mean, rstd, dx, dx_bf16, dres, dgamma, dbeta, ln_ws, ln_ws_bytes, ws, ws_bytes, stream, nullptr);
+}
+
+extern "C" int unetr_gemm_bf16_ln_fwd_pf(const unetr_gemm_bf16_desc* d, const void* A, const void* B, float* C,
+                                         const float* gamma, const float* beta, float eps, float* y, void* y_bf16, float* mean, float* rstd,
+                                         float* ws, size_t ws_bytes, void* stream, const unetr_prefetch* pf) {
     if (!d || !C) return UNETR_ERR_ARG;
     if (d->pre || d->act || d->accumulate || d->alpha != 1.f || d->ldc != d->N) return UNETR_ERR_UNSUPPORTED;
     int splits = 1;
     if (int e = gemm_bf16_impl(d, A, B, C, nullptr, ws, ws_bytes, stream, &splits)) return e;
     if (splits > 1)
         return unetr_layernorm_fwd_partials(ws, splits, (long)d->M * d->N, d->bias, d->res, d->ldr, d->res_mod > 0 ? d->res_mod : d->M,
-                                            C, gamma, beta, y, y_bf16, mean, rstd, d->M, d->N, eps, stream);
-    return unetr_layernorm_fwd(C, gamma, beta, y, y_bf16, mean, rstd, d->M, d->N, eps, stream);
+                                            C, gamma, beta, y, y_bf16, mean, rstd, d->M, d->N, eps, stream, pf);
+    return unetr_layernorm_fwd_pf(C, gamma, beta, y, y_bf16, mean, rstd, d->M, d->N, eps, stream, pf);
+}
+
+extern "C" int unetr_gemm_bf16_ln_fwd(const unetr_gemm_bf16_desc* d, const void* A, const void* B, float* C,
+                                      const float* gamma, const float* beta, float eps, float* y, void* y_bf16, float* mean, float* rstd,
+                                      float* ws, size_t ws_bytes, void* stream) {
+    return unetr_gemm_bf16_ln_fwd_pf(d, A, B, C, gamma, beta, eps, y, y_bf16, mean, rstd, ws, ws_bytes, stream, nullptr);
 }
 
 extern "C" int unetr_cast_bf16(const float* src, void* dst, long n, void* stream) {
diff --git a/3dmedicalimagesegmentation_amd/csrc/norm_misc.hip b/3dmedicalimagesegmentation_amd/csrc/norm_misc.hip
--- a/3dmedicalimagesegmentation_amd/csrc/norm_misc.hip
+++ b/3dmedicalimagesegmentation_amd/csrc/norm_misc.hip
@@ -13,7 +13,9 @@
 __global__ void __launch_bounds__(256)
 layernorm_fwd_kernel(const float* __restrict__ x, const float* __restrict__ gamma, const float* __restrict__ beta,
                      float* __restrict__ y, uint16_t* __restrict__ yb, float* __restrict__ mean, float* __restrict__ rstd,
-                     int M, int H, float eps, LnFwdSrc src) {
+                     int M, int H, float eps, LnFwdSrc src, PrefetchRider pf) {
+    const int rider = (int)blockIdx.x - ((int)gridDim.x - pf.nblk);
+    if (rider >= 0) { prefetch_rider_block(pf, rider); return; }
     const int lane = threadIdx.x & 63, row = blockIdx.x * 4 + (threadIdx.x >> 6);
     if (row >= M) return;
     const int nv = H >> 2;
@@ -92,7 +94,9 @@
 __global__ void __launch_bounds__(256)
 layernorm_bwd_kernel(const float* __restrict__ dy, int splits, long slab, const float* __restrict__ x, const float* __restrict__ gamma,
                      const float* __restrict__ mean, const float* __restrict__ rstd, float* __restrict__ dx,
-                     uint16_t* __restrict__ dxb, const float* __restrict__ dres, float* __restrict__ part, int M, int H) {
+                     uint16_t* __restrict__ dxb, const float* __restrict__ dres, float* __restrict__ part, int M, int H, PrefetchRider pf) {
+    const int rider = (int)blockIdx.x - ((int)gridDim.x - pf.nblk);
+    if (rider >= 0) { prefetch_rider_block(pf, rider); return; }
     extern __shared__ __attribute__((aligned(16))) float lds[];
     const int lane = threadIdx.x & 63, wave = threadIdx.x >> 6;
     const int nv = H >> 2;
@@ -1566,27 +1570,36 @@
 
 }
 
-extern "C" int unetr_layernorm_fwd(const float* x, const float* gamma, const float* beta, float* y, void* y_bf16,
-                                   float* mean, float* rstd, int M, int H, float eps, void* stream) {
+constexpr long LN_PF_BLOCK_BYTES = 32 * 1024;
+
+extern "C" int unetr_layernorm_fwd_pf(const float* x, const float* gamma, const float* beta, float* y, void* y_bf16,
+                                      float* mean, float* rstd, int M, int H, float eps, void* stream, const unetr_prefetch* pf) {
     if (!x || !gamma || !beta || (!y && !y_bf16) || !mean || !rstd || M <= 0) return UNETR_ERR_ARG;
     if ((H & 3) || H > LN_MAXV_MAX * 256) return UNETR_ERR_UNSUPPORTED;
     const LnFwdSrc src{1, 0, nullptr, nullptr, 0, 1, nullptr};
-#define LN_FWD(V_) hipLaunchKernelGGL(layernorm_fwd_kernel<V_>, dim3(cdiv(M, 4)), dim3(256), 0, (hipStream_t)stream, x, gamma, beta, y, \
-                                      (uint16_t*)y_bf16, mean, rstd, M, H, eps, src)
+    const PrefetchRider rd = prefetch_rider(pf, LN_PF_BLOCK_BYTES);
+#define LN_FWD(V_) hipLaunchKernelGGL(layernorm_fwd_kernel<V_>, dim3(cdiv(M, 4) + rd.nblk), dim3(256), 0, (hipStream_t)stream, x, gamma, beta, y, \
+                                      (uint16_t*)y_bf16, mean, rstd, M, H, eps, src, rd)
     if (H <= 768) LN_FWD(3); else if (H <= 1024) LN_FWD(4); else LN_FWD(8);
 #undef LN_FWD
     return unetr_check_launch();
 }
 
+extern "C" int unetr_layernorm_fwd(const float* x, const float* gamma, const float* beta, float* y, void* y_bf16,
+                                   float* mean, float* rstd, int M, int H, float eps, void* stream) {
+    return unetr_layernorm_fwd_pf(x, gamma, beta, y, y_bf16, mean, rstd, M, H, eps, stream, nullptr);
+}
+
 int unetr_layernorm_fwd_partials(const float* partials, int splits, long slab, const float* bias, const float* res, long ldr, int res_mod,
                                  float* xout, const float* gamma, const float* beta, float* y, void* y_bf16, float* mean, float* rstd,
-                                 int M, int H, float eps, void* stream) {
+                                 int M, int H, float eps, void* stream, const unetr_prefetch* pf) {
     if (!partials || splits < 2 || !xout || !gamma || !beta || (!y && !y_bf16) || !mean || !rstd || M <= 0) return UNETR_ERR_ARG;
     if ((H & 3) || H > LN_MAXV_MAX * 256 || (res && (ldr & 3))) return UNETR_ERR_UNSUPPORTED;
     const LnFwdSrc src{splits, slab, bias, res, ldr, res_mod > 0 ? res_mod : M, xout};
     const float* x = partials;
-#define LN_FWD(V_) hipLaunchKernelGGL(layernorm_fwd_kernel<V_>, dim3(cdiv(M, 4)), dim3(256), 0, (hipStream_t)stream, x, gamma, beta, y, \
-                                      (uint16_t*)y_bf16, mean, rstd, M, H, eps, src)
+    const PrefetchRider rd = prefetch_rider(pf, LN_PF_BLOCK_BYTES);
+#define LN_FWD(V_) hipLaunchKernelGGL(layernorm_fwd_kernel<V_>, dim3(cdiv(M, 4) + rd.nblk), dim3(256), 0, (hipStream_t)stream, x, gamma, beta, y, \
+                                      (uint16_t*)y_bf16, mean, rstd, M, H, eps, src, rd)
     if (H <= 768) LN_FWD(3); else if (H <= 1024) LN_FWD(4); else LN_FWD(8);
 #undef LN_FWD
     return unetr_check_launch();
@@ -1594,23 +1607,30 @@
 
 int unetr_layernorm_bwd_partials(const float* dy, int splits, long slab, const float* x, const float* gamma, const float* mean,
                                  const float* rstd, float* dx, void* dx_bf16, const float* dres, float* dgamma,
-                                 float* dbeta, int M, int H, float* ws, size_t ws_bytes, void* stream) {
+                                 float* dbeta, int M, int H, float* ws, size_t ws_bytes, void* stream, const unetr_prefetch* pf) {
     if (!dy || !x || !gamma || !mean || !rstd || !dx || ((dgamma == nullptr) != (dbeta == nullptr)) || M <= 0) return UNETR_ERR_ARG;
     if ((H & 3) || H > LN_MAXV_MAX * 256) return UNETR_ERR_UNSUPPORTED;
     int nblk = cdiv(M, LN_RPB);
     if ((size_t)nblk * 2 * H * sizeof(float) > ws_bytes || !ws) return UNETR_ERR_WORKSPACE;
     hipStream_t st = (hipStream_t)stream;
-#define LN_BWD(V_) hipLaunchKernelGGL(layernorm_bwd_kernel<V_>, dim3(nblk), dim3(256), 4 * 2 * H * sizeof(float), st, dy, splits, slab, x, gamma, mean, \
-                                      rstd, dx, (uint16_t*)dx_bf16, dres, ws, M, H)
+    const PrefetchRider rd = prefetch_rider(pf, LN_PF_BLOCK_BYTES);
+#define LN_BWD(V_) hipLaunchKernelGGL(layernorm_bwd_kernel<V_>, dim3(nblk + rd.nblk), dim3(256), 4 * 2 * H * sizeof(float), st, dy, splits, slab, x, gamma, mean, \
+                                      rstd, dx, (uint16_t*)dx_bf16, dres, ws, M, H, rd)
     if (H <= 768) LN_BWD(3); else if (H <= 1024) LN_BWD(4); else LN_BWD(8);
     if (dgamma) hipLaunchKernelGGL(ln_finalize_kernel, dim3(cdiv(2 * H, 64)), dim3(256), 0, st, ws, nblk, H, dgamma, dbeta);
     return unetr_check_launch();
+}
+
+extern "C" int unetr_layernorm_bwd_pf(const float* dy, const float* x, const float* gamma, const float* mean,
+                                      const float* rstd, float* dx, void* dx_bf16, const float* dres, float* dgamma,
+                                      float* dbeta, int M, int H, float* ws, size_t ws_bytes, void* stream, const unetr_prefetch* pf) {
+    return unetr_layernorm_bwd_partials(dy, 1, 0, x, gamma, mean, rstd, dx, dx_bf16, dres, dgamma, dbeta, M, H, ws, ws_bytes, stream, pf);
 }
 
 extern "C" int unetr_layernorm_bwd(const float* dy, const float* x, const float* gamma, const float* mean,
                                    const float* rstd, float* dx, void* dx_bf16, const float* dres, float* dgamma,
                                    float* dbeta, int M, int H, float* ws, size_t ws_bytes, void* stream) {
-    return unetr_layernorm_bwd_partials(dy, 1, 0, x, gamma, mean, rstd, dx, dx_bf16, dres, dgamma, dbeta, M, H, ws, ws_bytes, stream);
+    return unetr_layernorm_bwd_pf(dy, x, gamma, mean, rstd, dx, dx_bf16, dres, dgamma, dbeta, M, H, ws, ws_bytes, stream, nullptr);
 }
 
 extern "C" int unetr_colsum(const float* x, long ld, int M, int N, float* out, int accumulate,
diff --git a/3dmedicalimagesegmentation_amd/functional.py b/3dmedicalimagesegmentation_amd/functional.py
--- a/3dmedicalimagesegmentation_amd/functional.py
+++ b/3dmedicalimagesegmentation_amd/functional.py
@@ -334,6 +334,7 @@
 
 
 _SHADOW = {}
+_SHADOW_AT = {}
 _WEIGHT_EPOCH = [0]
 
 
@@ -417,6 +418,7 @@
 
 def register_weight_shadow(w, shadow):
     _SHADOW[id(w)] = [shadow, w._version, _WEIGHT_EPOCH[0], True, weakref.ref(w), w.data_ptr()]
+    _SHADOW_AT[w.data_ptr()] = _SHADOW[id(w)]
 
 
 def weight_bf16(w):
@@ -424,6 +426,7 @@
     if ent is None or ent[4]() is not w or ent[0].shape != w.shape or ent[0].device != w.device:
         ent = [torch.empty(w.shape, dtype=torch.bfloat16, device=w.device), -1, -1, False, weakref.ref(w), 0]
         _SHADOW[id(w)] = ent
+        _SHADOW_AT[w.data_ptr()] = ent
     fresh = ent[1] == w._version and ent[5] == w.data_ptr() and (
         ent[3] or (ent[2] == _WEIGHT_EPOCH[0] and not torch.cuda.is_current_stream_capturing()))
     if not fresh:
@@ -489,6 +492,23 @@
     return ent[0].data_ptr()
 
 
+PREFETCH_RIDERS = True
+
+
+def _prefetch(host, *weights):
+    if not PREFETCH_RIDERS or (PREFETCH_RIDERS is not True and host not in PREFETCH_RIDERS):
+        return None
+    pf, n = _capi.Prefetch(), 0
+    for w in weights:
+        ent = _SHADOW_AT.get(w.data_ptr()) if w is not None else None
+        owner = ent[4]() if ent is not None else None
+        if owner is None or owner.data_ptr() != w.data_ptr() or ent[0].shape != w.shape or ent[0].device != w.device:
+            continue
+        pf.ptr[n], pf.bytes[n] = ent[0].data_ptr(), ent[0].numel() * 2
+        n += 1
+    return pf if n else None
+
+
 def _bf16_path(prec, *kdims):
     return prec == _capi.PREC_BF16 and all(k % 64 == 0 for k in kdims)
 
@@ -588,38 +608,38 @@
     return torch.empty(t.shape, dtype=torch.bfloat16, device=t.device)
 
 
-def layernorm_fwd(x, w, b, bf16_out=None, want_fp32=True):
+def layernorm_fwd(x, w, b, bf16_out=None, want_fp32=True, pf=None):
     M, H = x.shape
     y = torch.empty_like(x) if want_fp32 else None
     mean = torch.empty(M, dtype=torch.float32, device=x.device)
     rstd = torch.empty(M, dtype=torch.float32, device=x.device)
-    call("unetr_layernorm_fwd", x.data_ptr(), w.data_ptr(), b.data_ptr(), _p(y), _p(bf16_out), mean.data_ptr(),
-         rstd.data_ptr(), M, H, LN_EPS, _stream())
+    call("unetr_layernorm_fwd_pf", x.data_ptr(), w.data_ptr(), b.data_ptr(), _p(y), _p(bf16_out), mean.data_ptr(),
+         rstd.data_ptr(), M, H, LN_EPS, _stream(), pf)
     return y, mean, rstd
 
 
-def layernorm_bwd(dy, x, w, mean, rstd, dres=None, out_w=None, out_b=None, dx_bf16=None):
+def layernorm_bwd(dy, x, w, mean, rstd, dres=None, out_w=None, out_b=None, dx_bf16=None, pf=None):
     M, H = x.shape
     dx = torch.empty_like(x)
     dw = out_w if out_w is not None else torch.empty(H, dtype=torch.float32, device=x.device)
     db = out_b if out_b is not None else torch.empty(H, dtype=torch.float32, device=x.device)
     ws = workspace(x.device)
-    call("unetr_layernorm_bwd", dy.data_ptr(), x.data_ptr(), w.data_ptr(), mean.data_ptr(), rstd.data_ptr(), dx.data_ptr(),
-         _p(dx_bf16), dres.data_ptr() if dres is not None else None, dw.data_ptr(), db.data_ptr(), M, H, ws.data_ptr(), ws.numel() * 4, _stream())
+    call("unetr_layernorm_bwd_pf", dy.data_ptr(), x.data_ptr(), w.data_ptr(), mean.data_ptr(), rstd.data_ptr(), dx.data_ptr(),
+         _p(dx_bf16), dres.data_ptr() if dres is not None else None, dw.data_ptr(), db.data_ptr(), M, H, ws.data_ptr(), ws.numel() * 4, _stream(), pf)
     return dx, dw, db
 
 
-def layernorm_bwd_params(dy, x, w, b, mean, rstd, dres=None, dx_bf16=None):
+def layernorm_bwd_params(dy, x, w, b, mean, rstd, dres=None, dx_bf16=None, pf=None):
     ow, ob = _gout(w), _gout(b)
     if ow is None or ob is None:
-        dx, dw, db = layernorm_bwd(dy, x, w, mean, rstd, dres=dres, out_w=ow, out_b=ob, dx_bf16=dx_bf16)
+        dx, dw, db = layernorm_bwd(dy, x, w, mean, rstd, dres=dres, out_w=ow, out_b=ob, dx_bf16=dx_bf16, pf=pf)
         return dx, _ret(w, dw), _ret(b, db)
     M, H = x.shape
     nblk = (M + 3) // 4
     part = torch.empty(nblk * 2 * H, dtype=torch.float32, device=x.device)
     dx = torch.empty_like(x)
-    call("unetr_layernorm_bwd", dy.data_ptr(), x.data_ptr(), w.data_ptr(), mean.data_ptr(), rstd.data_ptr(), dx.data_ptr(),
-         _p(dx_bf16), _p(dres), None, None, M, H, part.data_ptr(), part.numel() * 4, _stream())
+    call("unetr_layernorm_bwd_pf", dy.data_ptr(), x.data_ptr(), w.data_ptr(), mean.data_ptr(), rstd.data_ptr(), dx.data_ptr(),
+         _p(dx_bf16), _p(dres), None, None, M, H, part.data_ptr(), part.numel() * 4, _stream(), pf)
     st = _GRAD_SINK[w.data_ptr()]
     st.defer["colsum"].append((part, ow, nblk, H, 2 * H))
     st.defer["colsum"].append((part[H:], ob, nblk, H, 2 * H))
@@ -631,7 +651,7 @@
     return M >= 32 and K % 32 == 0 and N % 4 == 0 and N >= 64 and os.environ.get("UNETR_X3_GEMM_DMA", "1") != "0"
 
 
-def gemm_bf16_ln_fwd(A, B, M, N, K, C, gamma, beta, y_bf16, bias=None, res=None, ldr=0, y=None, b_words=None):
+def gemm_bf16_ln_fwd(A, B, M, N, K, C, gamma, beta, y_bf16, bias=None, res=None, ldr=0, y=None, b_words=None, pf=None):
     x3 = A.dtype == torch.float32
     assert x3 or (A.dtype == torch.bfloat16 and B.dtype == torch.bfloat16)
     d = GemmBf16Desc()
@@ -646,8 +666,8 @@
     mean = torch.empty(M, dtype=torch.float32, device=C.device)
     rstd = torch.empty(M, dtype=torch.float32, device=C.device)
     ws = workspace(C.device)
-    call("unetr_gemm_bf16_ln_fwd", ctypes.byref(d), A.data_ptr(), B.data_ptr(), C.data_ptr(), gamma.data_ptr(), beta.data_ptr(), LN_EPS,
-         _p(y), _p(y_bf16), mean.data_ptr(), rstd.data_ptr(), ws.data_ptr(), ws.numel() * 4, _stream())
+    call("unetr_gemm_bf16_ln_fwd_pf", ctypes.byref(d), A.data_ptr(), B.data_ptr(), C.data_ptr(), gamma.data_ptr(), beta.data_ptr(), LN_EPS,
+         _p(y), _p(y_bf16), mean.data_ptr(), rstd.data_ptr(), ws.data_ptr(), ws.numel() * 4, _stream(), pf)
     return mean, rstd
 
 
@@ -666,7 +686,7 @@
     return st[0], st[1], st[2]
 
 
-def gemm_ln_bwd_params(A, Bw, M, N, K, x, w, b, mean, rstd, dres=None, dx_bf16=None, b_words=None):
+def gemm_ln_bwd_params(A, Bw, M, N, K, x, w, b, mean, rstd, dres=None, dx_bf16=None, b_words=None, pf=None):
     x3 = A.dtype == torch.float32
     assert x3 or (A.dtype == torch.bfloat16 and Bw.dtype == torch.bfloat16)
     d = GemmBf16Desc()
@@ -685,14 +705,14 @@
         dw = ow if ow is not None else torch.empty(N, dtype=torch.float32, device=x.device)
         db = ob if ob is not None else torch.empty(N, dtype=torch.float32, device=x.device)
         lnws = torch.empty(nblk * 2 * N, dtype=torch.float32, device=x.device)
-        call("unetr_gemm_bf16_ln_bwd", ctypes.byref(d), A.data_ptr(), Bw.data_ptr(), scratch.data_ptr(), x.data_ptr(), w.data_ptr(),
+        call("unetr_gemm_bf16_ln_bwd_pf", ctypes.byref(d), A.data_ptr(), Bw.data_ptr(), scratch.data_ptr(), x.data_ptr(), w.data_ptr(),
              mean.data_ptr(), rstd.data_ptr(), dx.data_ptr(), _p(dx_bf16), _p(dres), dw.data_ptr(), db.data_ptr(),
-             lnws.data_ptr(), lnws.numel() * 4, ws.data_ptr(), ws.numel() * 4, _stream())
+             lnws.data_ptr(), lnws.numel() * 4, ws.data_ptr(), ws.numel() * 4, _stream(), pf)
         return dx, _ret(w, dw), _ret(b, db)
     part = torch.empty(nblk * 2 * N, dtype=torch.float32, device=x.device)
-    call("unetr_gemm_bf16_ln_bwd", ctypes.byref(d), A.data_ptr(), Bw.data_ptr(), scratch.data_ptr(), x.data_ptr(), w.data_ptr(),
+    call("unetr_gemm_bf16_ln_bwd_pf", ctypes.byref(d), A.data_ptr(), Bw.data_ptr(), scratch.data_ptr(), x.data_ptr(), w.data_ptr(),
          mean.data_ptr(), rstd.data_ptr(), dx.data_ptr(), _p(dx_bf16), _p(dres), None, None,
-         part.data_ptr(), part.numel() * 4, ws.data_ptr(), ws.numel() * 4, _stream())
+         part.data_ptr(), part.numel() * 4, ws.data_ptr(), ws.numel() * 4, _stream(), pf)
     st = _GRAD_SINK[w.data_ptr()]
     st.defer["colsum"].append((part, ow, nblk, N, 2 * N))
     st.defer["colsum"].append((part[N:], ob, nblk, N, 2 * N))
@@ -716,17 +736,17 @@
     return dqkv
 
 
-def attention_bf16_fwd(qkvb, B, L, heads, dh, out_bf16, out=None):
+def attention_bf16_fwd(qkvb, B, L, heads, dh, out_bf16, out=None, pf=None):
     lse = torch.empty(B, heads, L, dtype=torch.float32, device=qkvb.device)
-    call("unetr_attention_bf16_fwd", qkvb.data_ptr(), _p(out), out_bf16.data_ptr(), lse.data_ptr(), B, L, heads, dh, float(dh) ** -0.5, _stream())
+    call("unetr_attention_bf16_fwd_pf", qkvb.data_ptr(), _p(out), out_bf16.data_ptr(), lse.data_ptr(), B, L, heads, dh, float(dh) ** -0.5, _stream(), pf)
     return lse
 
 
-def attention_bf16_bwd(qkvb, outb, doutb, lse, B, L, heads, dh, dqkv=None):
+def attention_bf16_bwd(qkvb, outb, doutb, lse, B, L, heads, dh, dqkv=None, pf=None):
     dqkvb = torch.empty_like(qkvb)
     delta = torch.empty_like(lse)
-    call("unetr_attention_bf16_bwd", qkvb.data_ptr(), outb.data_ptr(), doutb.data_ptr(), lse.data_ptr(), _p(dqkv), dqkvb.data_ptr(),
-         delta.data_ptr(), B, L, heads, dh, float(dh) ** -0.5, _stream())
+    call("unetr_attention_bf16_bwd_pf", qkvb.data_ptr(), outb.data_ptr(), doutb.data_ptr(), lse.data_ptr(), _p(dqkv), dqkvb.data_ptr(),
+         delta.data_ptr(), B, L, heads, dh, float(dh) ** -0.5, _stream(), pf)
     return dqkvb
 
 
@@ -1154,7 +1174,8 @@
         return None, dw, db, dpos, None, None
 
 
-def _tblock_forward(x, n1w, n1b, wqkv, wp, bp, n2w, n2b, w1, b1, w2, b2, B, L, heads, prec, train, next_ln=None, emit_twin=False):
+def _tblock_forward(x, n1w, n1b, wqkv, wp, bp, n2w, n2b, w1, b1, w2, b2, B, L, heads, prec, train, next_ln=None, emit_twin=False,
+                    next_wqkv=None):
     hid = x.shape[1]
     dh = hid // heads
     M, mlp = x.shape[0], w1.shape[0]
@@ -1168,12 +1189,12 @@
             y1b, m1, r1 = pre
         else:
             y1b = bf16_like(x)
-            _, m1, r1 = layernorm_fwd(x, n1w, n1b, bf16_out=y1b, want_fp32=False)
+            _, m1, r1 = layernorm_fwd(x, n1w, n1b, bf16_out=y1b, want_fp32=False, pf=_prefetch("ln1_fwd", wqkv))
         gemm_bf16(y1b, weight_bf16(wqkv), M, 3 * hid, hid, C=None if b16att else qkv, Cb=qkv if b16att else None)
         attb = bf16_like(x)
         if b16att:
             att = x.new_empty(0)
-            lse = attention_bf16_fwd(qkv, B, L, heads, dh, attb)
+            lse = attention_bf16_fwd(qkv, B, L, heads, dh, attb, pf=_prefetch("attn_fwd", wp, w1))
         else:
             att, lse = attention_fwd(qkv, B, L, heads, dh, prec, out_bf16=attb)
         x1 = torch.empty(M, hid, **f32)
@@ -1181,14 +1202,15 @@
         u = torch.empty(M, mlp, **f32) if train else None
         ab = torch.empty(M, mlp, dtype=torch.bfloat16, device=x.device)
         y2b = bf16_like(x)
-        _, m2, r2 = layernorm_fwd(x1, n2w, n2b, bf16_out=y2b, want_fp32=False)
+        _, m2, r2 = layernorm_fwd(x1, n2w, n2b, bf16_out=y2b, want_fp32=False, pf=_prefetch("ln2_fwd", w2))
         gemm_bf16(y2b, weight_bf16(w1), M, mlp, hid, Cb=ab, bias=b1, act=1, pre=u)
         if not train:
             u = m1 = r1 = m2 = r2 = y1b = y2b = x.new_empty(0)
         x2 = torch.empty(M, hid, **f32)
         if next_ln is not None and not emit_twin:
             xn = bf16_like(x)
-            mn, rn = gemm_bf16_ln_fwd(ab, weight_bf16(w2), M, hid, mlp, x2, next_ln[0], next_ln[1], xn, bias=b2, res=x1, ldr=hid)
+            mn, rn = gemm_bf16_ln_fwd(ab, weight_bf16(w2), M, hid, mlp, x2, next_ln[0], next_ln[1], xn, bias=b2, res=x1, ldr=hid,
+                                      pf=_prefetch("ln1_fwd", next_wqkv))
             _stash_ln(x2, next_ln[0], next_ln[1], xn, mn, rn)
         else:
             x2b = bf16_like(x) if emit_twin else None
@@ -1221,7 +1243,7 @@
 
     @staticmethod
     def forward(ctx, x, n1w, n1b, wqkv, wp, bp, n2w, n2b, w1, b1, w2, b2, B, L, heads, prec, ckpt=False, next_n1w=None, next_n1b=None,
-                emit_twin=False):
+                emit_twin=False, next_wqkv=None, below_w2=None, below_w1=None):
         _require_gpu(x)
         xc = x.contiguous()
         if xc is not x and hasattr(x, "_unetr_ln"):
@@ -1229,7 +1251,8 @@
         x = xc
         train = any(ctx.needs_input_grad[:12])
         x2, acts, twins = _tblock_forward(x, n1w, n1b, wqkv, wp, bp, n2w, n2b, w1, b1, w2, b2, B, L, heads, prec,
-                                          train and not ckpt, None if next_n1w is None else (next_n1w, next_n1b), bool(emit_twin))
+                                          train and not ckpt, None if next_n1w is None else (next_n1w, next_n1b), bool(emit_twin), next_wqkv)
+        ctx.below = (below_w2, below_w1)
         ctx.ckpt = bool(ckpt) and train
         if ctx.ckpt:
             acts, twins = (), None
@@ -1266,7 +1289,8 @@
         db1 = colsum_or_defer(dub if fast else du, M, mlp, mlp, b1)
         if fast:
             dx1b = bf16_like(x)
-            dx1, dn2w, dn2b = gemm_ln_bwd_params(dub, weight_bf16(w1), M, hid, mlp, x1, n2w, n2b, m2, r2, dres=dx2, dx_bf16=dx1b)
+            dx1, dn2w, dn2b = gemm_ln_bwd_params(dub, weight_bf16(w1), M, hid, mlp, x1, n2w, n2b, m2, r2, dres=dx2, dx_bf16=dx1b,
+                                                 pf=_prefetch("ln2_bwd", wp))
         else:
             dx1b = None
             if prec == _capi.PREC_BF16X3 and ln_ride_enabled() and x3_ride_ok(M, hid, mlp):
@@ -1287,14 +1311,15 @@
         dbp = colsum_or_defer(dx1, M, hid, hid, bp)
         if b16att:
             dqkv = None
-            dqkvb = attention_bf16_bwd(qkv, attb, dattb, lse, B, L, heads, dh)
+            dqkvb = attention_bf16_bwd(qkv, attb, dattb, lse, B, L, heads, dh, pf=_prefetch("attn_bwd", wqkv))
         else:
             dqkvb = torch.empty(M, 3 * hid, dtype=torch.bfloat16, device=x.device) if fast else None
             dqkv = attention_bwd(qkv, att, datt, lse, B, L, heads, dh, prec, dqkv_bf16=dqkvb)
         dwqkv = wgrad_or_defer(dqkv, y1, prec, wqkv, dqkvb, y1b)
         if fast:
             dxb = bf16_like(x)
-            dx, dn1w, dn1b = gemm_ln_bwd_params(dqkvb, weight_bf16(wqkv), M, hid, 3 * hid, x, n1w, n1b, m1, r1, dres=dx1, dx_bf16=dxb)
+            dx, dn1w, dn1b = gemm_ln_bwd_params(dqkvb, weight_bf16(wqkv), M, hid, 3 * hid, x, n1w, n1b, m1, r1, dres=dx1, dx_bf16=dxb,
+                                                pf=_prefetch("ln1_bwd", *ctx.below))
         else:
             dxb = None
             if prec == _capi.PREC_BF16X3 and ln_ride_enabled() and x3_ride_ok(M, hid, 3 * hid):
@@ -1304,12 +1329,12 @@
                 dx, dn1w, dn1b = layernorm_bwd_params(dy1, x, n1w, n1b, m1, r1, dres=dx1, dx_bf16=dxb)
         if fast:
             _attach_twin(dx, dxb)
-        return (dx, dn1w, dn1b, dwqkv, dwp, dbp, dn2w, dn2b, dw1, db1, dw2, db2, None, None, None, None, None, None, None, None)
+        return (dx, dn1w, dn1b, dwqkv, dwp, dbp, dn2w, dn2b, dw1, db1, dw2, db2) + (None,) * 11
 
 
 class LayerNormFn(torch.autograd.Function):
     @staticmethod
-    def forward(ctx, x, w, b, twin=False):
+    def forward(ctx, x, w, b, twin=False, below_w2=None, below_w1=None):
         _require_gpu(x)
         x = x.contiguous()
         yb = bf16_like(x) if twin else None
@@ -1318,16 +1343,17 @@
             _attach_twin(y, yb)
         ctx.save_for_backward(x, w, mean, rstd, b)
         ctx.twin = bool(twin)
+        ctx.below = (below_w2, below_w1) if twin else (None, None)
         return y
 
     @staticmethod
     def backward(ctx, dy):
         x, w, mean, rstd, b = ctx.saved_tensors
         dxb = bf16_like(x) if ctx.twin else None
-        dx, dw, db = layernorm_bwd_params(dy.contiguous(), x, w, b, mean, rstd, dx_bf16=dxb)
+        dx, dw, db = layernorm_bwd_params(dy.contiguous(), x, w, b, mean, rstd, dx_bf16=dxb, pf=_prefetch("ln1_bwd", *ctx.below))
         if dxb is not None:
             _attach_twin(dx, dxb)
-        return dx, dw, db, None
+        return dx, dw, db, None, None, None
 
 
 def skip_half(dims, C, prec, device):
diff --git a/3dmedicalimagesegmentation_amd/unetr.py b/3dmedicalimagesegmentation_amd/unetr.py
--- a/3dmedicalimagesegmentation_amd/unetr.py
+++ b/3dmedicalimagesegmentation_amd/unetr.py
@@ -300,7 +300,10 @@
                 blk.norm2.weight, blk.norm2.bias, blk.mlp.linear1.weight, blk.mlp.linear1.bias, blk.mlp.linear2.weight,
                 blk.mlp.linear2.bias, B, L, self.num_heads, prec, ckpt,
                 None if nxt is None else nxt.weight.detach(), None if nxt is None else nxt.bias.detach(),
-                i in taps)
+                i in taps,
+                self.vit.blocks[i + 1].attn.qkv.weight.detach() if b16 and i + 1 < nblk else None,
+                self.vit.blocks[i - 1].mlp.linear2.weight.detach() if b16 and i > 0 else None,
+                self.vit.blocks[i - 1].mlp.linear1.weight.detach() if b16 and i > 0 else None)
             k = self._pass_of_block(i) - 1
             if i in taps:
                 xa, xb = Fn.TapFn.apply(x, b16)
@@ -310,8 +313,9 @@
                 if (i + 1) in starts:
                     x = cut(x, k)
                 hidden_states_out.append(x)
-        x = Fn.LayerNormFn.apply(x, self.vit.norm.weight, self.vit.norm.bias,
-                                 Fn._bf16_path(prec, self.hidden_size, self.vit.blocks[0].mlp.linear1.weight.shape[0]))
+        x = Fn.LayerNormFn.apply(x, self.vit.norm.weight, self.vit.norm.bias, b16,
+                                 self.vit.blocks[-1].mlp.linear2.weight.detach() if b16 else None,
+                                 self.vit.blocks[-1].mlp.linear1.weight.detach() if b16 else None)
         x = cut(x, 0)
         enc1 = Fn.ResBlockFn.apply(Fn.to_channels_last(x_in), *self._res_w(self.encoder1.layer), prec, True)
         enc = []
diff --git a/include/unetr_hip.h b/include/unetr_hip.h
--- a/include/unetr_hip.h
+++ b/include/unetr_hip.h
@@ -90,6 +90,13 @@
 int unetr_attention_bf16_bwd(const void* qkv, const void* out_bf16, const void* dout_bf16, const float* lse, float* dqkv,
                              void* dqkv_bf16, float* delta, int B, int L, int heads, int dh, float scale, void* stream);
 
+typedef struct { const void* ptr[2]; size_t bytes[2]; } unetr_prefetch;
+int unetr_attention_bf16_fwd_pf(const void* qkv, float* out, void* out_bf16, float* lse, int B, int L, int heads, int dh,
+                                float scale, void* stream, const unetr_prefetch* pf);
+int unetr_attention_bf16_bwd_pf(const void* qkv, const void* out_bf16, const void* dout_bf16, const float* lse, float* dqkv,
+                                void* dqkv_bf16, float* delta, int B, int L, int heads, int dh, float scale, void* stream,
+                                const unetr_prefetch* pf);
+
 int unetr_pixel_shuffle2(const float* t, void* y, long ldy, int B, int D, int H, int W, int Cout, int act16, void* stream);
 int unetr_pixel_unshuffle2_bf16(const void* dy, long lddy, void* g_bf16, int B, int D, int H, int W, int Cout, int act16, void* stream);
 
@@ -103,6 +110,11 @@
                         const float* rstd, float* dx, void* dx_bf16 ,
                         const float* dres , float* dgamma, float* dbeta,
                         int M, int H, float* ws, size_t ws_bytes, void* stream);
+int unetr_layernorm_fwd_pf(const float* x, const float* gamma, const float* beta, float* y, void* y_bf16,
+                           float* mean, float* rstd, int M, int H, float eps, void* stream, const unetr_prefetch* pf);
+int unetr_layernorm_bwd_pf(const float* dy, const float* x, const float* gamma, const float* mean,
+                           const float* rstd, float* dx, void* dx_bf16, const float* dres, float* dgamma, float* dbeta,
+                           int M, int H, float* ws, size_t ws_bytes, void* stream, const unetr_prefetch* pf);
 
 int unetr_gemm_bf16_ln_bwd(const unetr_gemm_bf16_desc* d, const void* A, const void* B, float* C,
                            const float* x, const float* gamma, const float* mean, const float* rstd,
@@ -112,6 +124,13 @@
 int unetr_gemm_bf16_ln_fwd(const unetr_gemm_bf16_desc* d, const void* A, const void* B, float* C,
                            const float* gamma, const float* beta, float eps, float* y, void* y_bf16, float* mean, float* rstd,
                            float* ws, size_t ws_bytes, void* stream);
+int unetr_gemm_bf16_ln_bwd_pf(const unetr_gemm_bf16_desc* d, const void* A, const void* B, float* C,
+                              const float* x, const float* gamma, const float* mean, const float* rstd,
+                              float* dx, void* dx_bf16, const float* dres, float* dgamma, float* dbeta,
+                              float* ln_ws, size_t ln_ws_bytes, float* ws, size_t ws_bytes, void* stream, const unetr_prefetch* pf);
+int unetr_gemm_bf16_ln_fwd_pf(const unetr_gemm_bf16_desc* d, const void* A, const void* B, float* C,
+                              const float* gamma, const float* beta, float eps, float* y, void* y_bf16, float* mean, float* rstd,
+                              float* ws, size_t ws_bytes, void* stream, const unetr_prefetch* pf);
 
 int unetr_attention_fwd(const float* qkv, float* out, void* out_bf16 , float* lse,
                         int B, int L, int heads, int dh, float scale, int prec, void* stream);
```

New measurement: 476.0 volumes/s, median of 6. 2.3% higher.
